# Aman-4-Real/MMTG

Measured on AMD Instinct MI355X. Metric: train tokens/sec, full MMTG config (GPT-2-base-zh decoder, 5x(img+text) 2048-d WenLan embs), higher is better.
Workload: dtype bf16; 1 GPU; Full MMTG train step: S=5 experience steps, T=15+221=236 decoder positions, GPT-2 12L/768/12H V=13317, dropout 0.1 on, MyLoss stage 3 + 0.2*KL, clip 1.0, AdamW; rows_per_gpu=64, global_rows=64, seq_len=236, parallelism=single GPU, no collective

## Files before the change

include/mmtg_hip.h:

```cpp
#ifndef MMTG_HIP_H
#define MMTG_HIP_H

#ifdef __cplusplus
extern "C" {
#endif

#define MMTG_ABI_VERSION 12

#define MMTG_API __attribute__((visibility("default")))

enum { MMTG_OK = 0, MMTG_ERR_BAD_ARG = -1, MMTG_ERR_HIP = -2, MMTG_ERR_UNSUPPORTED = -3 };
enum { MMTG_F32 = 0, MMTG_BF16 = 1 };

enum {
    MMTG_EPI_NONE = 0,
    MMTG_EPI_GELU = 1,
    MMTG_EPI_TANH = 2,
    MMTG_EPI_RESID = 3,
    MMTG_EPI_DGELU = 4,
    MMTG_EPI_DTANH = 5,
    MMTG_EPI_ATOMIC = 6,
    MMTG_EPI_ROWDOT = 7,
    MMTG_EPI_SPLIT = 8,
    MMTG_EPI_TANH_ADD = 9
};
#define MMTG_GEMM_NO_TR 1
#define MMTG_GEMM_REGSTAGE 2
#define MMTG_GEMM_SKINNY 4
#define MMTG_GEMM_NO_SKINNY 8
#define MMTG_GEMM_WIDE 16
#define MMTG_GEMM_NO_WIDE 32
#define MMTG_GEMM_PERSIST 64
#define MMTG_GEMM_NO_PERSIST 128
#define MMTG_GEMM_ROW_ORDER 256
#define MMTG_GEMM_OCC4 512
#define MMTG_GEMM_NO_OCC4 1024
#define MMTG_GEMM_NO_P8 8192
#define MMTG_GEMM_GELU_GRAD 32768
#define MMTG_GEMM_P8 16384
#define MMTG_GEMM_AUX2_BF16 131072
#define MMTG_GEMM_P8_288 65536
#define MMTG_GEMM_P256 4096
#define MMTG_GEMM_COL_BLOCK 2048

enum {
    MMTG_PROF_GEMM_BF16 = 0, MMTG_PROF_GEMM_F32, MMTG_PROF_ATTN_FWD, MMTG_PROF_ATTN_BWD,
    MMTG_PROF_LAYERNORM, MMTG_PROF_EMBED, MMTG_PROF_LOSS, MMTG_PROF_OPTIM, MMTG_PROF_ENCODER,
    MMTG_PROF_DECODE, MMTG_PROF_MISC, MMTG_PROF_NCAT
};

MMTG_API int mmtg_abi_version(void);
MMTG_API const char* mmtg_build_flags(void);
MMTG_API const char* mmtg_last_error(void);

MMTG_API int mmtg_prof_enable(int on);
MMTG_API int mmtg_prof_read(int* launches, double* ms, double* flops, double* bytes);

MMTG_API int mmtg_gemm(int dtype, int transA, int transB, int M, int N, int K,
              const void* A, long lda, const void* B, long ldb, void* C, long ldc,
              const float* bias, int epi, const void* aux, long ldaux, void* aux2,
              int out_f32, float alpha, int splits, unsigned drop_thresh, unsigned drop_seed,
              int flags, void* stream);

MMTG_API int mmtg_gemm_x3(int M, int N, int K, const void* A, long lda, long planeA, const void* B, long ldb, long planeB,
                 float* C, long ldc, void* planes, long ldp, long plane_out, const float* bias, int epi,
                 const float* aux, long ldaux, void* aux2, unsigned drop_thresh, unsigned drop_seed, int flags, void* stream);
MMTG_API int mmtg_split_planes(const float* src, long lds, int rows, int cols, void* planes, long ldp, long plane, void* stream);
MMTG_API int mmtg_layernorm_fwd_x3(const float* x, void* planes, long ldp, long plane, const float* gamma, const float* beta,
                          float* mean, float* rstd, int rows, int cols, float eps, void* x_bf16, void* stream);

MMTG_API int mmtg_gemm_gather(int mode, int M, int N, int K, const void* A, long lda, const void* B, long ldb, void* C, long ldc,
                     const float* bias, int epi, const int* rows, int table_rows, const void* aux, long ldaux, const int* aux_rows,
                     int splits, void* stream);

MMTG_API int mmtg_gemm_trace(void* buf, int max_wgs);
MMTG_API int mmtg_gemm_cu_budget(int cus);
MMTG_API int mmtg_debug_occupy(int workgroups, int lds_bytes, double usec, void* stream);

MMTG_API int mmtg_splitk_finish(int dtype, const float* part, int splits, int M, int N, long ldp, const float* bias,
                       int epi, const void* aux, long ldaux, void* out, long ldo,
                       const float* ln_gamma, const float* ln_beta, void* ln_out, float eps, void* stream);

MMTG_API long mmtg_colsum_ws(int M, int N);
MMTG_API int mmtg_colsum(int dtype, const void* X, long ldx, int M, int N, float* out, float* ws, long ws_floats, void* stream);
typedef struct { const float* X; float* out; long ldx; int M; int N; } mmtg_colsum_item;
MMTG_API int mmtg_colsum_batch(const mmtg_colsum_item* items, int n, void* stream);

MMTG_API int mmtg_layernorm_fwd(int dtype, const void* x, void* y, const float* gamma, const float* beta,
                       float* mean, float* rstd, int rows, int cols, float eps, void* stream);
MMTG_API long mmtg_layernorm_bwd_ws(int rows, int cols);
MMTG_API int mmtg_layernorm_bwd(int dtype, const void* dy, const void* x, const float* gamma,
                       const float* mean, const float* rstd, const void* dres, void* dx,
                       float* dgamma, float* dbeta, int rows, int cols,
                       void* dx_masked, unsigned drop_thresh, unsigned drop_seed, float* dcolsum,
                       float* ws, long ws_floats, void* stream);
MMTG_API int mmtg_layernorm_bwd_partial(int dtype, const void* dy, const void* x, const float* gamma,
                       const float* mean, const float* rstd, const void* dres, void* dx, int rows, int cols,
                       void* dx_masked, unsigned drop_thresh, unsigned drop_seed, int want_colsum,
                       float* ws, long ws_floats, int* partial_rows, void* stream);
MMTG_API int mmtg_layernorm_bwd_x3(const float* dy, const float* x, const float* gamma, const float* mean, const float* rstd,
                          const float* dres, float* dx, float* dgamma, float* dbeta, int rows, int cols,
                          void* dx_planes, long plane, unsigned drop_thresh, unsigned drop_seed, float* dcolsum,
                          float* ws, long ws_floats, void* stream);
MMTG_API int mmtg_layernorm_bwd_x3_partial(const float* dy, const float* x, const float* gamma, const float* mean, const float* rstd,
                          const float* dres, float* dx, int rows, int cols, void* dx_planes, long plane,
                          unsigned drop_thresh, unsigned drop_seed, int want_colsum,
                          float* ws, long ws_floats, int* partial_rows, void* stream);

MMTG_API int mmtg_attn_fwd(int dtype, const void* qkv, const int* keep, void* out, float* lse,
                  int B, int T, int nH, int dh, unsigned drop_thresh, unsigned drop_seed, void* stream);
MMTG_API int mmtg_attn_fwd_x3(const void* qkv_planes, long qplane, const int* keep, float* out, void* out_planes, long plane, float* lse,
                     int B, int T, int nH, int dh, unsigned drop_thresh, unsigned drop_seed, void* stream);
MMTG_API int mmtg_attn_bwd_x3(const void* qkv_planes, long qplane, const int* keep, const float* out, const void* dout_planes, long doplane,
                     const float* lse, float* delta,
                     int delta_ready, float* dq32, long dq32_floats, void* dqkv_planes, long dplane, float* dbias, float* dbias_ws,
                     long dbias_ws_floats, int B, int T, int nH, int dh, unsigned drop_thresh, unsigned drop_seed, void* stream);
MMTG_API int mmtg_attn_trace(void* buf);
#define MMTG_ATTN_ELEM_MASK 1
#define MMTG_ATTN_DBIAS_ROWS 2
MMTG_API int mmtg_attn_bwd_dbias_rows(int dtype, int B, int T);
MMTG_API int mmtg_attn_bwd(int dtype, const void* qkv, const int* keep, const void* out, const void* dout,
                  const float* lse, float* delta, int delta_ready, float* dq32, void* dqkv, float* dbias, float* dbias_ws,
                  int B, int T, int nH, int dh, unsigned drop_thresh, unsigned drop_seed, int flags, void* stream);

MMTG_API int mmtg_embed_condition(int dtype, const void* table, const long long* topic_ids,
                         const long long* targets, const void* c, void* x,
                         int B, int P, int L, int S, int E, int two_sents, int V, void* stream);
MMTG_API int mmtg_segment_sum(int dtype, const void* g, void* out, int B, int P, int L, int S, int H,
                     int two_sents, void* stream);
MMTG_API int mmtg_embed_add(int dtype, const void* g, const void* wpe, const void* wte, const long long* type_ids,
                   void* h, int M, int T, int D, unsigned drop_thresh, unsigned drop_seed, void* stream);
MMTG_API long mmtg_embed_add_bwd_ws(int M, int D, int ntypes);
MMTG_API int mmtg_embed_add_bwd(int dtype, void* dh, const long long* type_ids, float* dwpe, float* dwte,
                       int M, int T, int D, int ntypes, unsigned drop_thresh, unsigned drop_seed, float* ws, long ws_floats,
                       void* stream);
MMTG_API int mmtg_dropout_apply(int dtype, const void* x, void* y, long n, int N, unsigned drop_thresh,
                       unsigned drop_seed, void* stream);

MMTG_API int mmtg_loss_fwd(int logits_dtype, const void* logits, long ldl, int V, const long long* topic_ids,
                  const long long* targets, const long long* ratings, int stage, int label_zero,
                  int B, int P, int L, float batch_den, float* nll, float* lse, float* sample_ce,
                  float* coef, float* scalars, void* stream);
MMTG_API int mmtg_loss_bwd(int dtype, int logits_dtype, const void* logits, long ldl, int V, const long long* topic_ids,
                  const long long* targets, const float* lse, const float* coef, float gscale, float lm_coef,
                  int B, int P, int L, void* dlogits, long ldd, int Vpad, void* stream);
MMTG_API int mmtg_loss_bwd_x3(const float* logits, long ldl, int V, const long long* topic_ids, const long long* targets, const float* lse,
                     const float* coef, float gscale, float lm_coef, int B, int P, int L, void* planes, long ldd, long plane,
                     int Vpad, void* stream);

MMTG_API int mmtg_gru_cell_fwd(int dtype, const void* gi, long ld_gi, const void* gh, long ld_gh, const void* h_prev, long ld_hp,
                      void* h, long ld_h, float* save, int B, int H, void* stream);
MMTG_API int mmtg_gru_cell_bwd(int dtype, const float* dh, const float* save, const void* h_prev, long ld_hp,
                      void* dgi, long ld_dgi, void* dgh, float* dh_prev, int B, int H, void* stream);
MMTG_API int mmtg_gru_cell_bwd_fused(int dtype, const void* rows, long ld_rows, const float* carry, const float* part, int splits,
                            const float* save, const void* h_prev, long ld_hp, void* dgi, long ld_dgi, void* dgh,
                            float* dh_prev, int B, int H, void* stream);
#define MMTG_RNN_RELU 0
#define MMTG_RNN_LSTM 1
MMTG_API int mmtg_rnn_cell_fwd(int dtype, int kind, const void* gi, long ld_gi, const void* gh, long ld_gh, const float* c_prev,
                      void* h, long ld_h, float* c, float* save, int B, int H, void* stream);
MMTG_API int mmtg_rnn_cell_bwd(int dtype, int kind, const void* rows, long ld_rows, const float* part, const float* save,
                      const float* c_prev, const void* h, long ld_h, float* dc, int dc_in, void* da, long ld_da,
                      int B, int H, void* stream);
MMTG_API int mmtg_alpha_attn_fwd(int dtype, const void* qkv, const float* prior, void* ctx, float* probs,
                        float* kl, int B, int S, int H, int heads, void* stream);
MMTG_API int mmtg_alpha_attn_bwd(int dtype, const void* qkv, const float* prior, const float* probs,
                        const void* dctx, float dkl, void* dqkv, int B, int S, int H, int heads,
                        void* stream);
MMTG_API int mmtg_beta_fuse_fwd(int dtype, const void* topic, const void* img, const void* txt,
                       const float* att_w, const float* att_b, void* o, float* a,
                       int B, int S, int H, void* stream);
MMTG_API long mmtg_beta_fuse_bwd_ws(int B, int S, int H);
// ... 110 lines not shown
```

mmtg_amd/csrc/attention.hip:

```cpp
#include <stdlib.h>

#include "attn_common.h"

namespace {

#ifndef ATTN_FWD_WAVES
#define ATTN_FWD_WAVES 4
#endif
template <typename T>
__global__ __launch_bounds__(256, ATTN_FWD_WAVES) void attn_fwd_kernel(const T* __restrict__ qkv, const int* __restrict__ keep,
        T* __restrict__ out, float* __restrict__ lse, int Tn, int nH,
        uint32_t drop_thresh, uint32_t drop_seed, float inv_keep) {
    typedef typename Vec16<T>::type V;
    typedef AT<T> A;
    __shared__ __attribute__((aligned(16))) char sK[64 * A::ROWB];
    __shared__ __attribute__((aligned(16))) char sV[64 * A::ROWB];
    __shared__ int sKeep[64];

    const int tid = threadIdx.x, lane = tid & 63, wave = tid >> 6, g = lane >> 4, l15 = lane & 15;
    const int qb = gridDim.x - 1 - blockIdx.x, h = blockIdx.y, b = blockIdx.z;
    const int D = nH * DH;
    const long ld = 3L * D;
    const T* base = qkv + (long)b * Tn * ld + h * DH;
    const int qi = qb * 64 + wave * 16 + l15;
// ... 422 lines not shown
}
template <int MT = 256>
__device__ __forceinline__ void dma_issue_scalars(void* dst, const void* src, int stride, int nvalid, int wave, int lane) {
    const __amdgpu_buffer_rsrc_t r = __builtin_amdgcn_make_buffer_rsrc(const_cast<void*>(src), 0, (int)(((long)(nvalid - 1) * stride + 1) * 4), 0x00020000);
    const int ws = wave % (MT / 64), i = 64 * ws + lane;
    __builtin_amdgcn_raw_ptr_buffer_load_lds(r, LDS_PTR(void, (char*)dst + 256 * ws), 4, i * stride * 4, 0, 0, 0);
}
template <int NW = 8, int MT = 256>
__device__ __forceinline__ void dma_wait_chunk(int c) {
    if (c >= 3) asm volatile("s_waitcnt vmcnt(0)" ::: "memory");
    else if ((MT / 32) / NW == 1) asm volatile("s_waitcnt vmcnt(2)" ::: "memory");
    else asm volatile("s_waitcnt vmcnt(4)" ::: "memory");
}
__device__ __forceinline__ void raw_barrier() { asm volatile("s_waitcnt lgkmcnt(0)\n\ts_barrier" ::: "memory"); }

constexpr int MASK_BITS = 12;
template <int NTHR = 512, int MT = 256>
__device__ __forceinline__ void gen_keep_mask(uint32_t* sMask, uint32_t bh, int Tn, uint32_t seed, uint32_t keepq, int tid) {
    const int nband = (Tn + 31) >> 5, total = 16 * nband * (nband + 1);
#pragma unroll 1
    for (int i = tid; i < total; i += NTHR) {
        int k = 0;
        while (16 * (k + 1) * (k + 2) <= i) ++k;
        const int j = i - 16 * k * (k + 1), row = 32 * k + j / (k + 1), w = j % (k + 1);
        if (keepq > 4096u) {
            const uint32_t base = (bh * (uint32_t)Tn + (uint32_t)row) * (uint32_t)Tn + 32u * (uint32_t)w;
            uint32_t bits = 0;
#pragma unroll 8
            for (int bit = 0; bit < 32; ++bit) bits |= (hash_u32(seed, base + (uint32_t)bit) >= keepq ? 1u : 0u) << bit;
            sMask[mask_row_base<MT>(row) + w] = bits;
            continue;
        }
        uint32_t x = hash_u32(seed, (bh * (uint32_t)Tn + (uint32_t)row) * (uint32_t)(MT / 32) + (uint32_t)w) | 1u;
        uint32_t acc = 0;
#pragma unroll
        for (int bit = 0; bit < MASK_BITS; ++bit) {
            x ^= x << 13; x ^= x >> 17; x ^= x << 5;
            acc = ((keepq >> bit) & 1u) ? (acc | x) : (acc & x);
        }
        sMask[mask_row_base<MT>(row) + w] = acc;
    }
}
__device__ __forceinline__ float mask_keep(float p, uint32_t w, int pos) {
    const int m = __builtin_amdgcn_sbfe(w, pos, 1);
    return __builtin_bit_cast(float, __builtin_bit_cast(int, p) & m);
}

__device__ __forceinline__ float mask_keep_u(float p, uint32_t w, int pos) {
    int m;
    asm("v_bfe_i32 %0, %1, %2, 1" : "=v"(m) : "v"(w), "s"(pos));
    return __builtin_bit_cast(float, __builtin_bit_cast(int, p) & m);
}

struct FwdTile {
    f32x4 o[4];
    float m, l;
};

__device__ __forceinline__ float max3f(float a, float b, float c) {
    float d;
    asm("v_max3_f32 %0, %1, %2, %3" : "=v"(d) : "v"(a), "v"(b), "v"(c));
    return d;
}

template <bool DROP, int MT = 256, bool DIAG = true>
__device__ __forceinline__ void fwd_small_chunk(FwdTile& st, const char* sK, const char* sV, const float* sBias, const uint32_t* sMask,
                                                const bf16x8 (&qf)[2], int t, int j0, int lane) {
    const int g = lane >> 4, l15 = lane & 15;
    const int qi = 16 * t + l15, qlast = 16 * t + 15;
    f32x4 s_acc[4];
    float mloc = -INFINITY;
#pragma unroll
    for (int kt = 0; kt < 4; ++kt) {
        s_acc[kt] = f32x4{0.f, 0.f, 0.f, 0.f};
        if (!DIAG || j0 + 16 * kt <= qlast) {
#pragma unroll
            for (int ks = 0; ks < 2; ++ks) mma16(ld_row(sK, j0 + kt * 16 + l15, ks, g), qf[ks], s_acc[kt]);
            const int k0 = j0 + kt * 16 + 4 * g;
            const f32x4 kb = *reinterpret_cast<const f32x4*>(sBias + k0);
            if (DIAG && j0 + 16 * kt + 15 > 16 * t) {
#pragma unroll
                for (int r = 0; r < 4; ++r) s_acc[kt][r] = (k0 + r <= qi) ? s_acc[kt][r] * LOG2E + kb[r] : -INFINITY;
            } else {
#pragma unroll
                for (int r = 0; r < 4; ++r) s_acc[kt][r] = s_acc[kt][r] * LOG2E + kb[r];
            }
            mloc = max3f(max3f(mloc, s_acc[kt][0], s_acc[kt][1]), s_acc[kt][2], s_acc[kt][3]);
        }
    }
    mloc = fmaxf(mloc, __shfl_xor(mloc, 16, 64));
    mloc = fmaxf(mloc, __shfl_xor(mloc, 32, 64));
    const float m_new = fmaxf(st.m, mloc);
    const float m_use = (m_new == -INFINITY) ? 0.f : m_new;
    const float alpha = __builtin_amdgcn_exp2f(st.m - m_use);
    float rs = 0.f;
    uint32_t w0 = 0, w1 = 0;
    if constexpr (DROP) {
        if constexpr (MT == 256) {
            const u32x2 w = *reinterpret_cast<const u32x2*>(sMask + qi * 8 + (j0 >> 5));
            w0 = w[0] >> (4 * g);
            w1 = w[1] >> (4 * g);
        } else {
            const uint32_t* wp = sMask + mask_row_base<MT>(qi) + (j0 >> 5);
            w0 = wp[0] >> (4 * g);
            w1 = wp[1] >> (4 * g);
        }
    }
#pragma unroll
    for (int kt = 0; kt < 4; ++kt) {
        if (!DIAG || j0 + 16 * kt <= qlast) {
#pragma unroll
            for (int r = 0; r < 4; ++r) {
                float p = __builtin_amdgcn_exp2f(s_acc[kt][r] - m_use);
                rs += p;
                if constexpr (DROP) p = mask_keep_u(p, kt < 2 ? w0 : w1, 16 * (kt & 1) + r);
                s_acc[kt][r] = p;
            }
        }
    }
    rs += __shfl_xor(rs, 16, 64);
    rs += __shfl_xor(rs, 32, 64);
    st.l = st.l * alpha + rs;
    st.m = m_new;
#pragma unroll
    for (int dt = 0; dt < 4; ++dt) {
        st.o[dt][0] *= alpha; st.o[dt][1] *= alpha; st.o[dt][2] *= alpha; st.o[dt][3] *= alpha;
    }
#pragma unroll
    for (int s2 = 0; s2 < 2; ++s2) {
        if (!DIAG || j0 + 32 * s2 <= qlast) {
            const bf16x8 pb = acc_as_operand(s_acc[2 * s2], s_acc[2 * s2 + 1], bf16());
#pragma unroll
            for (int dt = 0; dt < 4; ++dt)
                mma16(ld_ks(sV, j0 + 32 * s2 + 4 * g, j0 + 32 * s2 + 16 + 4 * g, dt * 16, lane, bf16()), pb, st.o[dt]);
        }
    }
}
template <bool DROP, int MT = 256>
__device__ __forceinline__ void fwd_small_chunk_any(FwdTile& st, const char* sK, const char* sV, const float* sBias, const uint32_t* sMask,
                                                    const bf16x8 (&qf)[2], int t, int j0, int lane) {
    if (j0 + 63 <= 16 * t) fwd_small_chunk<DROP, MT, false>(st, sK, sV, sBias, sMask, qf, t, j0, lane);
    else fwd_small_chunk<DROP, MT, true>(st, sK, sV, sBias, sMask, qf, t, j0, lane);
}

__device__ __forceinline__ void fwd_small_store(const FwdTile& st, int t, int lane, int b, int h, int Tn, int nH, float inv_keep,
                                                bf16* __restrict__ out, float* __restrict__ lse) {
    const int g = lane >> 4, l15 = lane & 15, qi = 16 * t + l15, D = nH * DH;
    if (qi < Tn) {
        const float inv = st.l > 0.f ? inv_keep / st.l : 0.f;
        bf16* dst = out + ((long)b * Tn + qi) * D + h * DH;
#pragma unroll
        for (int dt = 0; dt < 4; ++dt) {
            bf16x4 o = {(bf16)(st.o[dt][0] * inv), (bf16)(st.o[dt][1] * inv), (bf16)(st.o[dt][2] * inv), (bf16)(st.o[dt][3] * inv)};
            *reinterpret_cast<bf16x4*>(dst + dt * 16 + 4 * g) = o;
        }
        if (g == 0) lse[((long)b * nH + h) * Tn + qi] = st.l > 0.f ? st.m * (1.0f / LOG2E) + logf(st.l) : -INFINITY;
    }
}

template <bool DROP, int MT = 256>
__global__ __launch_bounds__(2 * MT, 4) void attn_fwd_small_kernel(const bf16* __restrict__ qkv, const int* __restrict__ keep,
        bf16* __restrict__ out, float* __restrict__ lse, int Tn, int nH,
        uint32_t keep16, uint32_t drop_seed, float inv_keep, unsigned long long* __restrict__ trace) {
    extern __shared__ __attribute__((aligned(16))) char smem[];
    unsigned long long ts[6] = {0, 0, 0, 0, 0, 0};
    ts[0] = __builtin_amdgcn_s_memrealtime();
    constexpr int NW = MT / 32, CROWS = MT / 4;
    const int nchunk = (Tn + CROWS - 1) / CROWS, rows_pad = nchunk * CROWS;
    char* sK = smem;
    char* sV = sK + rows_pad * 128;
    int* sKeep = reinterpret_cast<int*>(sV + rows_pad * 128);
    float* sBias = reinterpret_cast<float*>(sKeep + MT);
    uint32_t* sMask = reinterpret_cast<uint32_t*>(sBias + MT + MT);
    const int tid = threadIdx.x, lane = tid & 63, g = lane >> 4, l15 = lane & 15;
    const int wave = __builtin_amdgcn_readfirstlane(tid >> 6);
    const int h = blockIdx.x % nH, b = blockIdx.x / nH;
    const int D = nH * DH;
    const long ld = 3L * D;
    const bf16* base = qkv + (long)b * Tn * ld + h * DH;
    const int ntile = (Tn + 15) >> 4, npair = (ntile + 1) >> 1;
    const int tA = wave, tB = ntile - 1 - wave;
    const bool work = wave < npair;
    bf16x8 qfA[2], qfB[2];
#pragma unroll
    for (int ks = 0; ks < 2; ++ks) {
        qfA[ks] = zero16<bf16>();
        qfB[ks] = zero16<bf16>();
        if (work) {
            const int qa = 16 * tA + l15, qb = 16 * tB + l15;
            if (qa < Tn) qfA[ks] = *reinterpret_cast<const bf16x8*>(base + (long)qa * ld + ks * 32 + g * 8);
            if (qb < Tn) qfB[ks] = *reinterpret_cast<const bf16x8*>(base + (long)qb * ld + ks * 32 + g * 8);
        }
    }
    const __amdgpu_buffer_rsrc_t rk = rows_rsrc(base + D, ld, Tn), rv = rows_rsrc(base + 2 * D, ld, Tn);
    dma_issue_scalars<MT>(sKeep, keep + (long)b * Tn, 1, Tn, wave, lane);
    dma_issue_chunk<NW, MT>(sK, rk, ld, sV, rv, ld, 0, nchunk, wave, lane);
    dma_issue_chunk<NW, MT>(sK, rk, ld, sV, rv, ld, 1, nchunk, wave, lane);
    if (trace) ts[1] = __builtin_amdgcn_s_memrealtime();
    if constexpr (DROP) gen_keep_mask<2 * MT, MT>(sMask, (uint32_t)(b * nH + h), Tn, drop_seed, keep16, tid);
#pragma unroll
    for (int ks = 0; ks < 2; ++ks)
#pragma unroll
        for (int e = 0; e < 8; ++e) {
            qfA[ks][e] = (bf16)((float)qfA[ks][e] * 0.125f);
            qfB[ks][e] = (bf16)((float)qfB[ks][e] * 0.125f);
        }
    FwdTile st;
#pragma unroll
    for (int i = 0; i < 4; ++i) st.o[i] = f32x4{0.f, 0.f, 0.f, 0.f};
    st.m = -INFINITY;
    st.l = 0.f;
#pragma unroll 1
    for (int jb = 0; jb < nchunk; ++jb) {
        dma_wait_chunk<NW, MT>(jb);
        raw_barrier();
        if (jb < 2) dma_issue_chunk<NW, MT>(sK, rk, ld, sV, rv, ld, jb + 2, nchunk, wave, lane);
        if (jb == 0) {
            if (tid < MT) sBias[tid] = sKeep[tid] != 0 ? 0.f : -INFINITY;
            raw_barrier();
            if (trace) ts[2] = __builtin_amdgcn_s_memrealtime();
        }
#pragma unroll 1
        for (int j0 = jb * CROWS; j0 < (jb + 1) * CROWS; j0 += 64)
            if (work && j0 <= 16 * tB + 15) fwd_small_chunk_any<DROP, MT>(st, sK, sV, sBias, sMask, qfB, tB, j0, lane);
    }
    if (trace) ts[3] = __builtin_amdgcn_s_memrealtime();
    if (work) fwd_small_store(st, tB, lane, b, h, Tn, nH, inv_keep, out, lse);
    if (trace) ts[4] = __builtin_amdgcn_s_memrealtime();
    if (work && tA != tB) {
#pragma unroll
        for (int i = 0; i < 4; ++i) st.o[i] = f32x4{0.f, 0.f, 0.f, 0.f};
        st.m = -INFINITY;
        st.l = 0.f;
#pragma unroll 1
        for (int j0 = 0; j0 <= 16 * tA + 15; j0 += 64) fwd_small_chunk_any<DROP, MT>(st, sK, sV, sBias, sMask, qfA, tA, j0, lane);
        fwd_small_store(st, tA, lane, b, h, Tn, nH, inv_keep, out, lse);
    }
    if (trace && lane == 0) {
        ts[5] = __builtin_amdgcn_s_memrealtime();
        unsigned long long* r = trace + ((long)blockIdx.x * NW + wave) * 8;
        r[0] = ts[0]; r[1] = ts[1]; r[2] = ts[2]; r[3] = ts[3]; r[4] = ts[4]; r[5] = ts[5];
        r[6] = __builtin_amdgcn_s_getreg((4 << 11) | 20);
        r[7] = 1;
    }
}

struct BwdKeys {
// ... 305 lines not shown
#pragma unroll
    for (int dt = 0; dt < 4; ++dt) {
        const bf16x8 ao = ld_ks(sO, q0 + 4 * g, q0 + 16 + 4 * g, dt * 16, lane, bf16());
        const bf16x8 aq = ld_ks(sQ, q0 + 4 * g, q0 + 16 + 4 * g, dt * 16, lane, bf16());
#pragma unroll
        for (int j = 0; j < 2; ++j) {
            mma16(ao, pb[j], st[j].dv[dt]);
            mma16(aq, db[j], st[j].dk[dt]);
        }
    }
}
__device__ __forceinline__ void bwd_small_keys2_store(const BwdKeys (&st)[2], int u, int lane, int b, int h, int Tn, int nH, float inv_keep,
                                                      const int* sKeep, int mt_mask, bf16* __restrict__ dqkv, bool bias, float& ck, float& cv) {
    const int g = lane >> 4, l15 = lane & 15, D = nH * DH;
    const long ld = 3L * D;
    f32x4 fk[4], fv[4];
#pragma unroll
    for (int dt = 0; dt < 4; ++dt) fk[dt] = fv[dt] = f32x4{0.f, 0.f, 0.f, 0.f};
#pragma unroll
    for (int j = 0; j < 2; ++j) {
        const int key = 32 * u + 16 * j + l15;
        const bool kin = key < Tn, kpok = sKeep[key & mt_mask] != 0;
        const float kz = kpok ? 1.f : 0.f, vz = kpok ? inv_keep : 0.f;
        bf16x4 kk[4], vv[4];
#pragma unroll
        for (int dt = 0; dt < 4; ++dt) {
            kk[dt] = bf16x4{(bf16)(st[j].dk[dt][0] * kz), (bf16)(st[j].dk[dt][1] * kz), (bf16)(st[j].dk[dt][2] * kz), (bf16)(st[j].dk[dt][3] * kz)};
            vv[dt] = bf16x4{(bf16)(st[j].dv[dt][0] * vz), (bf16)(st[j].dv[dt][1] * vz), (bf16)(st[j].dv[dt][2] * vz), (bf16)(st[j].dv[dt][3] * vz)};
        }
        if (kin) {
            bf16* dst = dqkv + ((long)b * Tn + key) * ld + h * DH;
#pragma unroll
            for (int dt = 0; dt < 4; ++dt) {
                *reinterpret_cast<bf16x4*>(dst + D + dt * 16 + 4 * g) = kk[dt];
                *reinterpret_cast<bf16x4*>(dst + 2 * D + dt * 16 + 4 * g) = vv[dt];
            }
        }
        if (bias) {
#pragma unroll
            for (int dt = 0; dt < 4; ++dt)
#pragma unroll
                for (int r = 0; r < 4; ++r) {
                    fk[dt][r] += kin ? (float)kk[dt][r] : 0.f;
                    fv[dt][r] += kin ? (float)vv[dt][r] : 0.f;
                }
        }
    }
    if (bias) {
        ck += bias_fold16(fk, l15);
        cv += bias_fold16(fv, l15);
    }
}

template <bool DROP, int MT = 256>
__global__ __launch_bounds__(MT, (MT == 256 ? 2 : 1)) void attn_bwd_small_kv2_kernel(const bf16* __restrict__ qkv, const int* __restrict__ keep,
        const bf16* __restrict__ d_out, const float* __restrict__ lse, const float* __restrict__ delta,
        bf16* __restrict__ dqkv, float* __restrict__ dbias, int bias_rows, int Tn, int nH,
        uint32_t keep16, uint32_t drop_seed, float inv_keep, unsigned long long* __restrict__ trace) {
    extern __shared__ __attribute__((aligned(16))) char smem[];
    unsigned long long ts[6] = {0, 0, 0, 0, 0, 0};
    ts[0] = __builtin_amdgcn_s_memrealtime();
    constexpr int NW = MT / 64, CROWS = MT / 4;
    const int nchunk = (Tn + CROWS - 1) / CROWS, rows_pad = nchunk * CROWS;
    char* sQ = smem;
    char* sO = sQ + rows_pad * 128;
    float* sLse = reinterpret_cast<float*>(sO + rows_pad * 128);
    float* sDel = sLse + MT;
    int* sKeep = reinterpret_cast<int*>(sDel + MT);
    uint32_t* sMask = reinterpret_cast<uint32_t*>(sKeep + 2 * MT);
    const int tid = threadIdx.x, lane = tid & 63, g = lane >> 4, l15 = lane & 15;
    const int wave = __builtin_amdgcn_readfirstlane(tid >> 6);
    const int h = blockIdx.x % nH, b = blockIdx.x / nH;
    const int D = nH * DH;
    const long ld = 3L * D;
    const bf16* base = qkv + (long)b * Tn * ld + h * DH;
    const bf16* dob = d_out + (long)b * Tn * D + h * DH;
    const int nunit = (Tn + 31) >> 5, nupair = (nunit + 1) >> 1;
    const int uA = wave, uB = nunit - 1 - wave;
    const bool work = wave < nupair;
    bf16x8 kf[2][2], vf[2][2];
    auto load_frags = [&](int u) {
#pragma unroll
        for (int j = 0; j < 2; ++j) {
            const int key = 32 * u + 16 * j + l15;
#pragma unroll
            for (int ks = 0; ks < 2; ++ks) {
                kf[j][ks] = vf[j][ks] = zero16<bf16>();
                if (key < Tn) {
                    kf[j][ks] = *reinterpret_cast<const bf16x8*>(base + (long)key * ld + D + ks * 32 + g * 8);
                    vf[j][ks] = *reinterpret_cast<const bf16x8*>(base + (long)key * ld + 2 * D + ks * 32 + g * 8);
                }
            }
        }
    };
    if (work) load_frags(uA);
    else {
#pragma unroll
        for (int j = 0; j < 2; ++j) kf[j][0] = kf[j][1] = vf[j][0] = vf[j][1] = zero16<bf16>();
    }
    const __amdgpu_buffer_rsrc_t rq = rows_rsrc(base, ld, Tn), ro = rows_rsrc(dob, D, Tn);
    dma_issue_scalars<MT>(sKeep, keep + (long)b * Tn, 1, Tn, wave, lane);
    dma_issue_scalars<MT>(sLse, lse + ((long)b * nH + h) * Tn, 1, Tn, wave, lane);
    dma_issue_scalars<MT>(sDel, delta + (long)b * Tn * nH + h, nH, Tn, wave, lane);
    dma_issue_chunk<NW, MT>(sQ, rq, ld, sO, ro, D, 0, nchunk, wave, lane);
    dma_issue_chunk<NW, MT>(sQ, rq, ld, sO, ro, D, 1, nchunk, wave, lane);
    if (trace) ts[1] = __builtin_amdgcn_s_memrealtime();
    if constexpr (DROP) gen_keep_mask<64 * NW, MT>(sMask, (uint32_t)(b * nH + h), Tn, drop_seed, keep16, tid);
    asm volatile("" :: "v"(kf[0][0]), "v"(kf[0][1]), "v"(vf[0][0]), "v"(vf[0][1]), "v"(kf[1][0]), "v"(kf[1][1]), "v"(vf[1][0]), "v"(vf[1][1]));
    BwdKeys st[2];
#pragma unroll
    for (int j = 0; j < 2; ++j)
#pragma unroll
        for (int i = 0; i < 4; ++i) st[j].dk[i] = st[j].dv[i] = f32x4{0.f, 0.f, 0.f, 0.f};
    float ck = 0.f, cv = 0.f;
    const float ik_scale = inv_keep * 0.125f;
#pragma unroll 1
    for (int c = 0; c < nchunk; ++c) {
        dma_wait_chunk<NW, MT>(c);
        raw_barrier();
        if (c < 2) dma_issue_chunk<NW, MT>(sQ, rq, ld, sO, ro, D, c + 2, nchunk, wave, lane);
        if (c == 0) {
            for (int i = tid; i < MT; i += 64 * NW) { sLse[i] *= LOG2E; sDel[i] *= 0.125f; }
            raw_barrier();
            if (trace) ts[2] = __builtin_amdgcn_s_memrealtime();
        }
#pragma unroll 1
        for (int qb = c * (CROWS / 32); qb < (c + 1) * (CROWS / 32) && qb < nunit; ++qb)
            if (work && qb >= uA) {
                if (qb == uA) bwd_small_keys2_block<DROP, MT, true>(st, sQ, sO, sLse, sDel, sMask, kf, vf, uA, 32 * qb, lane, ik_scale);
                else bwd_small_keys2_block<DROP, MT, false>(st, sQ, sO, sLse, sDel, sMask, kf, vf, uA, 32 * qb, lane, ik_scale);
            }
    }
    if (trace) ts[3] = __builtin_amdgcn_s_memrealtime();
    if (work) {
        if (uB != uA) load_frags(uB);
        bwd_small_keys2_store(st, uA, lane, b, h, Tn, nH, inv_keep, sKeep, MT - 1, dqkv, dbias != nullptr, ck, cv);
        if (uB != uA) {
#pragma unroll
            for (int j = 0; j < 2; ++j)
#pragma unroll
                for (int i = 0; i < 4; ++i) st[j].dk[i] = st[j].dv[i] = f32x4{0.f, 0.f, 0.f, 0.f};
            bwd_small_keys2_block<DROP, MT, true>(st, sQ, sO, sLse, sDel, sMask, kf, vf, uB, 32 * uB, lane, ik_scale);
#pragma unroll 1
// ... 39 lines not shown
    uint32_t wq = 0;
    if constexpr (DROP) wq = sMask[mask_row_base<MT>(qi) + (j0 >> 5)] >> (4 * g);
#pragma unroll
    for (int kt = 0; kt < 2; ++kt) {
        dsT[kt] = f32x4{0.f, 0.f, 0.f, 0.f};
        if (!DIAG || j0 + 16 * kt <= qlast) {
            f32x4 s_acc = {0.f, 0.f, 0.f, 0.f}, dp_acc = {0.f, 0.f, 0.f, 0.f};
#pragma unroll
            for (int ks = 0; ks < 2; ++ks) {
                mma16(ld_row(sK, j0 + kt * 16 + l15, ks, g), qf[ks], s_acc);
                mma16(ld_row(sV, j0 + kt * 16 + l15, ks, g), of[ks], dp_acc);
            }
            const int k0 = j0 + kt * 16 + 4 * g;
            const f32x4 kb = *reinterpret_cast<const f32x4*>(sBias + k0);
#pragma unroll
            for (int r = 0; r < 4; ++r) {
                float x = s_acc[r] * c1 - lse2_q + kb[r];
                if constexpr (DIAG) x = k0 + r <= qi ? x : -INFINITY;
                const float p = __builtin_amdgcn_exp2f(x);
                float dp = dp_acc[r];
                if constexpr (DROP) dp = mask_keep_u(dp, wq, 16 * kt + r);
                dsT[kt][r] = p * (dp * ik_scale - dels_q);
            }
        }
    }
    const bf16x8 db = acc_as_operand(dsT[0], dsT[1], bf16());
#pragma unroll
    for (int dt = 0; dt < 4; ++dt)
        mma16(ld_ks(sK, j0 + 4 * g, j0 + 16 + 4 * g, dt * 16, lane, bf16()), db, dq[dt]);
}
__device__ __forceinline__ void bwd_small_queries_store(const f32x4 (&dq)[4], int t, int lane, int b, int h, int Tn, int nH,
                                                        bf16* __restrict__ dqkv, bool bias, float& cq) {
    const int g = lane >> 4, l15 = lane & 15, qi = 16 * t + l15, D = nH * DH;
    const long ld = 3L * D;
    const bool qok = qi < Tn;
    if (qok) {
        bf16* dst = dqkv + ((long)b * Tn + qi) * ld + h * DH;
#pragma unroll
        for (int dt = 0; dt < 4; ++dt) {
            bf16x4 qq = {(bf16)dq[dt][0], (bf16)dq[dt][1], (bf16)dq[dt][2], (bf16)dq[dt][3]};
            *reinterpret_cast<bf16x4*>(dst + dt * 16 + 4 * g) = qq;
        }
    }
    if (bias) {
        f32x4 fq[4];
#pragma unroll
        for (int dt = 0; dt < 4; ++dt)
#pragma unroll
            for (int r = 0; r < 4; ++r) fq[dt][r] = qok ? (float)(bf16)dq[dt][r] : 0.f;
        cq += bias_fold16(fq, l15);
    }
}

template <bool DROP, int MT = 256>
__global__ __launch_bounds__(2 * MT, 4) void attn_bwd_small_q_kernel(const bf16* __restrict__ qkv, const int* __restrict__ keep,
        const bf16* __restrict__ d_out, const float* __restrict__ lse, const float* __restrict__ delta,
        bf16* __restrict__ dqkv, float* __restrict__ dbias, int bias_rows, int Tn, int nH,
        uint32_t keep16, uint32_t drop_seed, float inv_keep, unsigned long long* __restrict__ trace) {
    extern __shared__ __attribute__((aligned(16))) char smem[];
    unsigned long long ts[6] = {0, 0, 0, 0, 0, 0};
    ts[0] = __builtin_amdgcn_s_memrealtime();
    constexpr int NW = MT / 32, CROWS = MT / 4;
    const int nchunk = (Tn + CROWS - 1) / CROWS, rows_pad = nchunk * CROWS;
    char* sK = smem;
    char* sV = sK + rows_pad * 128;
    int* sKeep = reinterpret_cast<int*>(sV + rows_pad * 128);
    float* sBias = reinterpret_cast<float*>(sKeep);
    float* sLse = sBias + MT;
    float* sDel = sLse + MT;
    uint32_t* sMask = reinterpret_cast<uint32_t*>(sDel + 2 * MT);
    const int tid = threadIdx.x, lane = tid & 63, g = lane >> 4, l15 = lane & 15;
    const int wave = __builtin_amdgcn_readfirstlane(tid >> 6);
    const int h = blockIdx.x % nH, b = blockIdx.x / nH;
    const int D = nH * DH;
    const long ld = 3L * D;
    const bf16* base = qkv + (long)b * Tn * ld + h * DH;
    const bf16* dob = d_out + (long)b * Tn * D + h * DH;
    const int ntile = (Tn + 15) >> 4, npair = (ntile + 1) >> 1;
    const int tA = wave, tB = ntile - 1 - wave;
    const bool work = wave < npair;
    const __amdgpu_buffer_rsrc_t rk = rows_rsrc(base + D, ld, Tn), rv = rows_rsrc(base + 2 * D, ld, Tn);
    dma_issue_scalars<MT>(sKeep, keep + (long)b * Tn, 1, Tn, wave, lane);
    dma_issue_scalars<MT>(sLse, lse + ((long)b * nH + h) * Tn, 1, Tn, wave, lane);
    dma_issue_scalars<MT>(sDel, delta + (long)b * Tn * nH + h, nH, Tn, wave, lane);
    dma_issue_chunk<NW, MT>(sK, rk, ld, sV, rv, ld, 0, nchunk, wave, lane);
    const int qa = 16 * tA + l15, qb_ = 16 * tB + l15;
    bf16x8 qfB[2], ofB[2];
    {
        const int qc = work ? (qb_ < Tn ? qb_ : Tn - 1) : 0;
#pragma unroll
        for (int ks = 0; ks < 2; ++ks) {
            qfB[ks] = *reinterpret_cast<const bf16x8*>(base + (long)qc * ld + ks * 32 + g * 8);
            ofB[ks] = *reinterpret_cast<const bf16x8*>(dob + (long)qc * D + ks * 32 + g * 8);
        }
    }
    dma_issue_chunk<NW, MT>(sK, rk, ld, sV, rv, ld, 1, nchunk, wave, lane);
    if (trace) ts[1] = __builtin_amdgcn_s_memrealtime();
    if constexpr (DROP) gen_keep_mask<2 * MT, MT>(sMask, (uint32_t)(b * nH + h), Tn, drop_seed, keep16, tid);
    asm volatile("" :: "v"(qfB[0]), "v"(qfB[1]), "v"(ofB[0]), "v"(ofB[1]));
    if (!(work && qb_ < Tn)) { qfB[0] = qfB[1] = ofB[0] = ofB[1] = zero16<bf16>(); }
    float lseB = 0.f, delB = 0.f;
    f32x4 dq[4];
#pragma unroll
    for (int i = 0; i < 4; ++i) dq[i] = f32x4{0.f, 0.f, 0.f, 0.f};
    const float ik_scale = inv_keep * 0.125f;
    bf16x8 qfA[2], ofA[2];
#pragma unroll 1
    for (int c = 0; c < nchunk; ++c) {
        dma_wait_chunk<NW, MT>(c);
        raw_barrier();
        if (c < 2) dma_issue_chunk<NW, MT>(sK, rk, ld, sV, rv, ld, c + 2, nchunk, wave, lane);
        if (c == 0) {
            if (tid < MT) sBias[tid] = sKeep[tid] != 0 ? 0.f : -INFINITY;
            lseB = sLse[qb_ & (MT - 1)] * LOG2E;
            delB = sDel[qb_ & (MT - 1)] * 0.125f;
            raw_barrier();
            if (trace) ts[2] = __builtin_amdgcn_s_memrealtime();
        }
#pragma unroll 1
        for (int kb = c * (CROWS / 32); kb < (c + 1) * (CROWS / 32); ++kb)
            if (work && 32 * kb <= 16 * tB + 15) {
                if (32 * kb + 31 <= 16 * tB) bwd_small_queries_block<DROP, MT, false>(dq, sK, sV, sBias, sMask, qfB, ofB, lseB, delB, tB, 32 * kb, lane, ik_scale);
                else bwd_small_queries_block<DROP, MT, true>(dq, sK, sV, sBias, sMask, qfB, ofB, lseB, delB, tB, 32 * kb, lane, ik_scale);
            }
    }
    if (trace) ts[3] = __builtin_amdgcn_s_memrealtime();
    float cq = 0.f;
    if (work) {
        if (tA != tB) {
            const int qc = qa < Tn ? qa : Tn - 1;
#pragma unroll
            for (int ks = 0; ks < 2; ++ks) {
                qfA[ks] = *reinterpret_cast<const bf16x8*>(base + (long)qc * ld + ks * 32 + g * 8);
                ofA[ks] = *reinterpret_cast<const bf16x8*>(dob + (long)qc * D + ks * 32 + g * 8);
// ... 16 lines not shown
    if (trace) ts[4] = __builtin_amdgcn_s_memrealtime();
    if (dbias) {
        __syncthreads();
        float* sBw = reinterpret_cast<float*>(smem);
        sBw[wave * DH + (l15 >> 2) * 16 + 4 * g + (l15 & 3)] = cq;
        __syncthreads();
        if (tid < DH) {
            float sm = 0.f;
#pragma unroll
            for (int w = 0; w < NW; ++w) sm += sBw[w * DH + tid];
            const int col = h * DH + tid;
            if (bias_rows) dbias[(long)b * 3 * D + col] = sm;
            else atomicAdd(dbias + col, sm);
        }
    }
    if (trace && lane == 0) {
        ts[5] = __builtin_amdgcn_s_memrealtime();
        unsigned long long* r = trace + ((long)(gridDim.x + blockIdx.x) * 16 + wave) * 8;
        r[0] = ts[0]; r[1] = ts[1]; r[2] = ts[2]; r[3] = ts[3]; r[4] = ts[4]; r[5] = ts[5];
        r[6] = __builtin_amdgcn_s_getreg((4 << 11) | 20);
        r[7] = 1;
    }
}

template <int MT = 256> inline size_t small_smem(int T) {
    const int cr = MT / 4, rp = ((T + cr - 1) / cr) * cr;
    return (size_t)rp * 256 + 4 * MT * 4 + (size_t)mask_words<MT>() * 4;
}
inline unsigned small_keep16(unsigned thresh32) { return 4096u - ((thresh32 + 0x80000u) >> 20); }
inline float small_inv_keep(unsigned keepq) { return (float)(4096.0 / (double)keepq); }


template <typename T> size_t bwd_smem_bytes() {
    typedef AT<T> A;
    const int KB = 4 * A::KPW;
    return (size_t)3 * KB * A::ROWB + 4 * 32 * A::ROWB + 32 * KB * sizeof(T) + 64 * sizeof(float) + KB * sizeof(int);
}

inline float inv_keep_of(unsigned thresh) {
    return thresh ? (float)(4294967296.0 / (4294967296.0 - (double)thresh)) : 1.0f;
}

}

static unsigned long long* g_attn_trace = nullptr;
extern "C" int mmtg_attn_trace(void* buf) {
    g_attn_trace = reinterpret_cast<unsigned long long*>(buf);
    return MMTG_OK;
}

static bool attn_route_tiled() { static const bool v = getenv("MMTG_ATTN_TILED") != nullptr; return v; }
static bool attn_route_no512() { static const bool v = getenv("MMTG_ATTN_NO512") != nullptr; return v; }

extern "C" int mmtg_attn_fwd(int dtype, const void* qkv, const int* keep, void* out, float* lse,
                             int B, int T, int nH, int dh, unsigned drop_thresh, unsigned drop_seed, void* stream) {
    MMTG_REQUIRE(dh == DH, "attn_fwd: head dim %d unsupported (built for 64)", dh);
    MMTG_REQUIRE(B > 0 && T > 0 && nH > 0, "attn_fwd: bad sizes");
    MMTG_REQUIRE(qkv && keep && out && lse, "attn_fwd: null pointer");
    MMTG_REQUIRE(MMTG_ALIGNED16(qkv) && MMTG_ALIGNED16(out), "attn_fwd: 16-byte alignment");
    hipStream_t s = (hipStream_t)stream;
    const double esz = dtype == MMTG_F32 ? 4 : 2;
    ProfScope prof(MMTG_PROF_ATTN_FWD, s, 2.0 * B * nH * (double)T * T * dh, esz * 4.0 * B * T * nH * dh);
    dim3 grid(cdiv(T, 64), nH, B), block(256);
    const float ik = inv_keep_of(drop_thresh);
    const bool legacy = attn_route_tiled(), no512 = attn_route_no512();
    if (dtype == MMTG_BF16 && T <= (no512 ? 256 : SM_MAXT) && !legacy) {
        static bool attr_set = false;
        if (!attr_set) {
            if (hipFuncSetAttribute((const void*)attn_fwd_small_kernel<false, 256>, hipFuncAttributeMaxDynamicSharedMemorySize, (int)small_smem<256>(256)) != hipSuccess ||
                hipFuncSetAttribute((const void*)attn_fwd_small_kernel<true, 256>, hipFuncAttributeMaxDynamicSharedMemorySize, (int)small_smem<256>(256)) != hipSuccess ||
                hipFuncSetAttribute((const void*)attn_fwd_small_kernel<false, 512>, hipFuncAttributeMaxDynamicSharedMemorySize, (int)small_smem<512>(512)) != hipSuccess ||
                hipFuncSetAttribute((const void*)attn_fwd_small_kernel<true, 512>, hipFuncAttributeMaxDynamicSharedMemorySize, (int)small_smem<512>(512)) != hipSuccess)
                MMTG_FAIL(MMTG_ERR_HIP, "attn_fwd: cannot raise dynamic LDS");
            attr_set = true;
        }
        const unsigned k16 = small_keep16(drop_thresh);
        const bool drop = k16 < 4096u;
        const unsigned kq = drop ? k16 : 0u;
        const float ikq = drop ? small_inv_keep(k16) : 1.0f;
#define FWD_SMALL(DROP_, MT_) hipLaunchKernelGGL((attn_fwd_small_kernel<DROP_, MT_>), dim3(B * nH), dim3(2 * MT_), small_smem<MT_>(T), s, \
                                                 (const bf16*)qkv, keep, (bf16*)out, lse, T, nH, kq, drop_seed, ikq, g_attn_trace)
        if (T <= 256) { if (drop) FWD_SMALL(true, 256); else FWD_SMALL(false, 256); }
        else { if (drop) FWD_SMALL(true, 512); else FWD_SMALL(false, 512); }
#undef FWD_SMALL
        MMTG_LAUNCH_CHECK("attn_fwd");
        return MMTG_OK;
    }
    if (dtype == MMTG_F32)
        hipLaunchKernelGGL(attn_fwd_kernel<float>, grid, block, 0, s, (const float*)qkv, keep, (float*)out, lse, T, nH, drop_thresh, drop_seed, ik);
    else if (dtype == MMTG_BF16)
        hipLaunchKernelGGL(attn_fwd_kernel<bf16>, grid, block, 0, s, (const bf16*)qkv, keep, (bf16*)out, lse, T, nH, drop_thresh, drop_seed, ik);
    else MMTG_FAIL(MMTG_ERR_BAD_ARG, "attn_fwd: bad dtype");
    MMTG_LAUNCH_CHECK("attn_fwd");
    return MMTG_OK;
}

extern "C" int mmtg_colsum(int dtype, const void* X, long ldx, int M, int N, float* out, float* ws, long ws_floats, void* stream);

extern "C" int mmtg_attn_bwd_dbias_rows(int dtype, int B, int T) {
    return (dtype == MMTG_BF16 && T <= (attn_route_no512() ? 256 : SM_MAXT) && !attn_route_tiled()) ? B : 0;
}

extern "C" int mmtg_attn_bwd(int dtype, const void* qkv, const int* keep, const void* out, const void* dout,
                             const float* lse, float* delta, int delta_ready, float* dq32, void* dqkv, float* dbias, float* dbias_ws,
                             int B, int T, int nH, int dh, unsigned drop_thresh, unsigned drop_seed, int flags, void* stream) {
    MMTG_REQUIRE(dh == DH, "attn_bwd: head dim %d unsupported (built for 64)", dh);
    MMTG_REQUIRE(B > 0 && T > 0 && nH > 0, "attn_bwd: bad sizes");
    MMTG_REQUIRE(qkv && keep && out && dout && lse && delta && dq32 && dqkv, "attn_bwd: null pointer");
    MMTG_REQUIRE(MMTG_ALIGNED16(qkv) && MMTG_ALIGNED16(dout) && MMTG_ALIGNED16(dqkv), "attn_bwd: 16-byte alignment");
    hipStream_t s = (hipStream_t)stream;
    const double esz = dtype == MMTG_F32 ? 4 : 2;
    ProfScope prof(MMTG_PROF_ATTN_BWD, s, 5.0 * B * nH * (double)T * T * dh, esz * 8.0 * B * T * nH * dh);
    const long rows = (long)B * T;
    const int D = nH * dh;
    const float ik = inv_keep_of(drop_thresh);
    float* const bias_dst = dbias && dbias_ws ? dbias_ws : dbias;
    const int bias_rows = dbias && dbias_ws ? 1 : 0;
    static bool attr_set[2] = {false, false};
    bool small_path = false;
    static const int ablate = getenv("MMTG_ATTN_ABLATE") ? atoi(getenv("MMTG_ATTN_ABLATE")) : 0;
    if (dtype == MMTG_F32) {
        const int KB = 4 * AT<float>::KPW;
        const int nkb = cdiv(T, KB);
        const size_t shm = bwd_smem_bytes<float>();
        if (!attr_set[0]) {
            if (hipFuncSetAttribute((const void*)attn_bwd_kernel<float, 4>, hipFuncAttributeMaxDynamicSharedMemorySize, (int)shm) != hipSuccess)
                MMTG_FAIL(MMTG_ERR_HIP, "attn_bwd: cannot raise dynamic LDS to %zu", shm);
            attr_set[0] = true;
        }
        if (!delta_ready) hipLaunchKernelGGL(attn_delta_kernel<float>, dim3(cdiv(rows * nH, 4)), dim3(256), 0, s, (const float*)out, (const float*)dout, delta, T, nH, rows);
        if (nkb > 1) { if (hipMemsetAsync(dq32, 0, rows * D * sizeof(float), s) != hipSuccess) MMTG_FAIL(MMTG_ERR_HIP, "attn_bwd: memset failed"); }
        hipLaunchKernelGGL((attn_bwd_kernel<float, 4>), dim3(nkb, nH, B), dim3(256), shm, s, (const float*)qkv, keep, (const float*)dout, lse, delta, dq32, (float*)dqkv, bias_dst, bias_rows, T, nH, nkb == 1, drop_thresh, drop_seed, ik, ablate);
        if (nkb > 1) hipLaunchKernelGGL(attn_dq_finish_kernel<float>, dim3(2048), dim3(256), 0, s, dq32, (float*)dqkv, rows, D);
    } else if (dtype == MMTG_BF16 && T <= (attn_route_no512() ? 256 : SM_MAXT) && !attn_route_tiled()) {
        small_path = true;
        static bool attr_small = false;
        if (!attr_small) {
            const int shm2 = (int)small_smem<256>(256), shm5 = (int)small_smem<512>(512);
            bool ok = true;
#define SET_LDS(K_, B_) ok = ok && hipFuncSetAttribute((const void*)K_, hipFuncAttributeMaxDynamicSharedMemorySize, B_) == hipSuccess
            SET_LDS((attn_bwd_small_kv_kernel<false, 8, 256>), shm2); SET_LDS((attn_bwd_small_kv_kernel<true, 8, 256>), shm2);
            SET_LDS((attn_bwd_small_kv_kernel<false, 4, 256>), shm2); SET_LDS((attn_bwd_small_kv_kernel<true, 4, 256>), shm2);
            SET_LDS((attn_bwd_small_q_kernel<false, 256>), shm2); SET_LDS((attn_bwd_small_q_kernel<true, 256>), shm2);
            SET_LDS((attn_bwd_small_kv_kernel<false, 16, 512>), shm5); SET_LDS((attn_bwd_small_kv_kernel<true, 16, 512>), shm5);
            SET_LDS((attn_bwd_small_kv_kernel<false, 8, 512>), shm5); SET_LDS((attn_bwd_small_kv_kernel<true, 8, 512>), shm5);
            SET_LDS((attn_bwd_small_q_kernel<false, 512>), shm5); SET_LDS((attn_bwd_small_q_kernel<true, 512>), shm5);
            SET_LDS((attn_bwd_small_kv2_kernel<false, 256>), shm2); SET_LDS((attn_bwd_small_kv2_kernel<true, 256>), shm2);
            SET_LDS((attn_bwd_small_kv2_kernel<false, 512>), shm5); SET_LDS((attn_bwd_small_kv2_kernel<true, 512>), shm5);
#undef SET_LDS
            if (!ok) MMTG_FAIL(MMTG_ERR_HIP, "attn_bwd: cannot raise dynamic LDS");
            attr_small = true;
        }
        if (!delta_ready) hipLaunchKernelGGL(attn_delta_kernel<bf16>, dim3(cdiv(rows * nH, 4)), dim3(256), 0, s, (const bf16*)out, (const bf16*)dout, delta, T, nH, rows);
        const unsigned th16 = small_keep16(drop_thresh);
        const bool elem = (flags & MMTG_ATTN_ELEM_MASK) && drop_thresh > 4096u;
        const bool drop = elem || th16 < 4096u;
        const unsigned kq = elem ? drop_thresh : drop ? th16 : 0u;
        const float ik16 = elem ? ik : drop ? small_inv_keep(th16) : 1.0f;
        static const int kv_nw = getenv("MMTG_ATTN_KV_NW") ? atoi(getenv("MMTG_ATTN_KV_NW")) : 0;
#define KV_SMALL(DROP_, NW_, MT_) hipLaunchKernelGGL((attn_bwd_small_kv_kernel<DROP_, NW_, MT_>), dim3(B * nH), dim3(64 * NW_), small_smem<MT_>(T), s, \
                                   (const bf16*)qkv, keep, (const bf16*)dout, lse, delta, (bf16*)dqkv, bias_dst, bias_rows, T, nH, kq, drop_seed, ik16, g_attn_trace)
#define Q_SMALL(DROP_, MT_) hipLaunchKernelGGL((attn_bwd_small_q_kernel<DROP_, MT_>), dim3(B * nH), dim3(2 * MT_), small_smem<MT_>(T), sq, \
                                   (const bf16*)qkv, keep, (const bf16*)dout, lse, delta, (bf16*)dqkv, bias_dst, bias_rows, T, nH, kq, drop_seed, ik16, g_attn_trace)
        static const bool kv2 = !(getenv("MMTG_ATTN_KV2") && atoi(getenv("MMTG_ATTN_KV2")) == 0);
#define KV2_SMALL(DROP_, MT_) hipLaunchKernelGGL((attn_bwd_small_kv2_kernel<DROP_, MT_>), dim3(B * nH), dim3(MT_), small_smem<MT_>(T), s, \
                                   (const bf16*)qkv, keep, (const bf16*)dout, lse, delta, (bf16*)dqkv, bias_dst, bias_rows, T, nH, kq, drop_seed, ik16, g_attn_trace)
        static const bool fork = getenv("MMTG_ATTN_BWD_FORK") && atoi(getenv("MMTG_ATTN_BWD_FORK")) == 1;
        static hipStream_t s2 = nullptr;
        static hipEvent_t ev_fork = nullptr, ev_join = nullptr;
        if (fork && !s2) {
            if (hipStreamCreateWithFlags(&s2, hipStreamNonBlocking) != hipSuccess || hipEventCreateWithFlags(&ev_fork, hipEventDisableTiming) != hipSuccess ||
                hipEventCreateWithFlags(&ev_join, hipEventDisableTiming) != hipSuccess)
                MMTG_FAIL(MMTG_ERR_HIP, "attn_bwd: cannot create the side stream");
        }
        hipStream_t sq = s;
        if (fork && kv2 && !kv_nw) {
            sq = s2;
            if (hipEventRecord(ev_fork, s) != hipSuccess || hipStreamWaitEvent(s2, ev_fork, 0) != hipSuccess) MMTG_FAIL(MMTG_ERR_HIP, "attn_bwd: fork failed");
        }
        if (kv2 && !kv_nw) {
            if (T <= 256) { if (drop) KV2_SMALL(true, 256); else KV2_SMALL(false, 256); }
            else { if (drop) KV2_SMALL(true, 512); else KV2_SMALL(false, 512); }
            if (T <= 256) { if (drop) Q_SMALL(true, 256); else Q_SMALL(false, 256); }
            else { if (drop) Q_SMALL(true, 512); else Q_SMALL(false, 512); }
            if (sq != s) {
                if (hipEventRecord(ev_join, s2) != hipSuccess || hipStreamWaitEvent(s, ev_join, 0) != hipSuccess) MMTG_FAIL(MMTG_ERR_HIP, "attn_bwd: join failed");
            }
        } else if (T <= 256) {
            const bool half = kv_nw ? kv_nw == 4 : drop;
            if (drop) { if (half) KV_SMALL(true, 4, 256); else KV_SMALL(true, 8, 256); Q_SMALL(true, 256); }
            else { if (half) KV_SMALL(false, 4, 256); else KV_SMALL(false, 8, 256); Q_SMALL(false, 256); }
        } else {
            const bool half = kv_nw ? kv_nw == 8 : drop;
            if (drop) { if (half) KV_SMALL(true, 8, 512); else KV_SMALL(true, 16, 512); Q_SMALL(true, 512); }
            else { if (half) KV_SMALL(false, 8, 512); else KV_SMALL(false, 16, 512); Q_SMALL(false, 512); }
        }
#undef KV_SMALL
#undef KV2_SMALL
#undef Q_SMALL
    } else if (dtype == MMTG_BF16) {
        const int KB = 4 * AT<bf16>::KPW;
        const int nkb = cdiv(T, KB);
        const size_t shm = bwd_smem_bytes<bf16>();
        if (!attr_set[1]) {
            if (hipFuncSetAttribute((const void*)attn_bwd_kernel<bf16, 8>, hipFuncAttributeMaxDynamicSharedMemorySize, (int)shm) != hipSuccess)
                MMTG_FAIL(MMTG_ERR_HIP, "attn_bwd: cannot raise dynamic LDS to %zu", shm);
            attr_set[1] = true;
        }
        if (!delta_ready) hipLaunchKernelGGL(attn_delta_kernel<bf16>, dim3(cdiv(rows * nH, 4)), dim3(256), 0, s, (const bf16*)out, (const bf16*)dout, delta, T, nH, rows);
        if (nkb > 1) { if (hipMemsetAsync(dq32, 0, rows * D * sizeof(float), s) != hipSuccess) MMTG_FAIL(MMTG_ERR_HIP, "attn_bwd: memset failed"); }
        hipLaunchKernelGGL((attn_bwd_kernel<bf16, 8>), dim3(nkb, nH, B), dim3(512), shm, s, (const bf16*)qkv, keep, (const bf16*)dout, lse, delta, dq32, (bf16*)dqkv, bias_dst, bias_rows, T, nH, nkb == 1, drop_thresh, drop_seed, ik, ablate);
        if (nkb > 1) hipLaunchKernelGGL(attn_dq_finish_kernel<bf16>, dim3(2048), dim3(256), 0, s, dq32, (bf16*)dqkv, rows, D);
    } else MMTG_FAIL(MMTG_ERR_BAD_ARG, "attn_bwd: bad dtype");
    MMTG_LAUNCH_CHECK("attn_bwd");
    const int nkb_ = small_path ? 1 : cdiv(T, dtype == MMTG_F32 ? 4 * AT<float>::KPW : 4 * AT<bf16>::KPW);
    if (bias_rows && !((flags & MMTG_ATTN_DBIAS_ROWS) && small_path)) {
        int rc = mmtg_colsum(MMTG_F32, dbias_ws, 3L * D, B * nkb_, 3 * D, dbias, nullptr, 0, stream);
        if (rc) return rc;
    }
    if (dbias && nkb_ > 1)
        return mmtg_colsum(dtype, dqkv, 3L * D, (int)rows, D, dbias, dbias_ws ? dbias_ws + (long)B * nkb_ * 3 * D : nullptr, dbias_ws ? 44L * 3 * D : 0, stream);
    return MMTG_OK;
}
```

mmtg_amd/csrc/gemm.hip:

```cpp
#include "gemm_common.h"
#include <stdlib.h>

namespace {

template <typename T, bool AKS, bool BKS, bool USE_TR>
__global__ __launch_bounds__(NTHR, 2) void gemm_kernel(GemmArgs p) {
    typedef typename Vec16<T>::type V;
    __shared__ __attribute__((aligned(16))) char smem[4 * TILE_BYTES];
    const int tid = threadIdx.x, lane = tid & 63, wave = tid >> 6;
    const int g = lane >> 4, l15 = lane & 15;
    const int wm = wave >> 1, wn = wave & 1;
    int m0, n0;
    int split;
    tile_origin(p, blockIdx.x, gridDim.x, m0, n0, split);
    const int kbeg = split * p.kper;
    const int kend = min(p.K, kbeg + p.kper);
    const int nk = (kend - kbeg + GT<T>::BK - 1) / GT<T>::BK;
    const T* A = reinterpret_cast<const T*>(p.A);
    const T* B = reinterpret_cast<const T*>(p.B);

    f32x4 acc[4][4];
#pragma unroll
    for (int i = 0; i < 4; ++i)
#pragma unroll
// ... 574 lines not shown
    constexpr int NW = TBM / 32;
    const size_t shm = 2 * (TBM + 128) * 128 + NW * epi_scratch_bytes<4, 4>();
    static_assert(TBM == 256 || 2 * (128 + 128) * 128 + 4 * epi_scratch_bytes<4, 4>() <= 80 * 1024, "two workgroups per CU");
    if (!attr_done) {
        int rc = set_lds(gemm_pp_kernel<AKS, BKS, TBM>, shm, 64 * NW, TBM == 256 ? "persistent 256x128" : "persistent 128x128");
        if (rc) return rc;
        attr_done = true;
    }
    GemmArgs b = a;
    b.tiles_n = cdiv(a.N, 128);
    b.ntiles = cdiv(a.M, TBM) * b.tiles_n;
    b.nitems = b.ntiles * splits;
    if (TBM == 256 && !(AKS && BKS) && splits == 1 && !(a.dbg_flags & 1)) b.cbw = column_block(a, TBM, 128, num_cus());
    const int slots = ((TBM == 256 ? 1 : 2) * num_cus()) & ~7;
    dim3 grid(b.nitems < slots ? b.nitems : slots), block(64 * NW);
    hipLaunchKernelGGL((gemm_pp_kernel<AKS, BKS, TBM>), grid, block, shm, stream, b);
    return MMTG_OK;
}

__device__ __forceinline__ void p8_issue(__amdgpu_buffer_rsrc_t r, char* d0, char* d1, int v0, int v1, int soff) {
    soff = __builtin_amdgcn_readfirstlane(soff);
    __builtin_amdgcn_raw_ptr_buffer_load_lds(r, LDS_PTR(void, d0), 16, v0, soff, 0, 0);
    __builtin_amdgcn_raw_ptr_buffer_load_lds(r, LDS_PTR(void, d1), 16, v1, soff, 0, 0);
}
__device__ __forceinline__ void p8_issue1(__amdgpu_buffer_rsrc_t r, char* d0, int v0, int soff) {
    soff = __builtin_amdgcn_readfirstlane(soff);
    __builtin_amdgcn_raw_ptr_buffer_load_lds(r, LDS_PTR(void, d0), 16, v0, soff, 0, 0);
}

template <int AH, int BH, int NA, int TMW, int FAN>
__device__ __forceinline__ void p8_mfma(const bf16x8 (&fa)[FAN][2], const bf16x8 (&fb)[2][2], f32x4 (&acc)[TMW][4], const bool prio = true) {
    if (prio) __builtin_amdgcn_s_setprio(1);
#pragma unroll
    for (int kk = 0; kk < 2; ++kk)
#pragma unroll
        for (int i = 0; i < NA; ++i)
#pragma unroll
            for (int j = 0; j < 2; ++j) mma16(fb[j][kk], fa[i][kk], acc[4 * AH + i][2 * BH + j]);
    if (prio) __builtin_amdgcn_s_setprio(0);
}

__device__ __forceinline__ bf16x8 p8_ld(const char* q) { return *reinterpret_cast<const bf16x8*>(q); }

#define P8_SYNC_IN()  do { asm volatile("s_barrier\n\ts_waitcnt lgkmcnt(0)" ::: "memory"); __builtin_amdgcn_sched_barrier(0); } while (0)
#define P8_SYNC_OUT() do { __builtin_amdgcn_sched_barrier(0); asm volatile("s_barrier" ::: "memory"); } while (0)

template <int GRPCH>
__device__ __forceinline__ int p8_ks_voff(long ld, int col0, int ncols, int h, int blk, int lane) {
    const int k = blk * 4 + (lane >> 4), pc = lane & 15, c = pc ^ ks_swz(k);
    const int col = (c / GRPCH) * (2 * GRPCH * 8) + h * (GRPCH * 8) + (c % GRPCH) * 8;
    return (col0 + col < ncols) ? (int)(((long)k * ld + col) * 2) : OOB;
}

template <int TBM, bool KS = false, bool X3 = false>
__global__ __launch_bounds__(512, 1) void gemm_p8_kernel(GemmArgs p) {
    typedef typename std::conditional<X3, float, bf16>::type TE;
    static_assert(!(X3 && (KS || TBM == 288)), "x3: K-contiguous operands, 256- or 192-row tiles");
    static_assert(TBM == 256 || ((TBM == 192 || TBM == 288) && !KS), "row tiles of 256 or (K-contiguous operands) 192 / 288");
    constexpr int WTM = TBM / 2, TMW = WTM / 16, NA1 = TMW - 4;
    constexpr int NBG = TBM / 16;
    constexpr int TA = TBM * 128, STAGE = TA + 256 * 128;
    extern __shared__ __attribute__((aligned(16))) char smem[];
    const int tid = threadIdx.x, lane = tid & 63;
    const int wave = __builtin_amdgcn_readfirstlane(tid >> 6);
    const int g = lane >> 4, l15 = lane & 15;
    const int wr = wave >> 2, wc = wave & 3;
    asm volatile("" :: "s"(p.A), "s"(p.B), "s"(p.M), "s"(p.N), "s"(p.K), "s"(p.lda), "s"(p.ldb), "s"(p.ntiles), "s"(p.tiles_n),
                 "s"(p.tiles_m_fast), "s"(p.cbw), "s"(p.trace), "s"(p.dbg_flags), "s"(p.bytesA), "s"(p.bytesB), "s"(p.kper));
    const bool tr = p.trace != nullptr;
    unsigned long long ts0 = 0, ts1 = 0, ts2 = 0, tc1 = 0, tc2 = 0;
    ts0 = __builtin_amdgcn_s_memrealtime();
    int m0, n0, split;
    tile_origin(p, blockIdx.x, gridDim.x, m0, n0, split, TBM, 256);
    const int kbeg = KS ? split * p.kper : 0;
    const int nk1 = max(0, (KS ? min(p.K, kbeg + p.kper) : p.K) - kbeg) >> 6;
    const int nk = X3 ? 3 * nk1 : nk1;

    const __amdgpu_buffer_rsrc_t ra = __builtin_amdgcn_make_buffer_rsrc(const_cast<void*>(p.A), 0, p.bytesA, 0x00020000);
    const __amdgpu_buffer_rsrc_t rb = __builtin_amdgcn_make_buffer_rsrc(const_cast<void*>(p.B), 0, p.bytesB, 0x00020000);
    const int sa0 = (int)((KS ? (long)kbeg * p.lda + m0 : (long)m0 * p.lda) * 2), sb0 = (int)((KS ? (long)kbeg * p.ldb + n0 : (long)n0 * p.ldb) * 2);
    const int stepa = KS ? (int)(64 * p.lda * 2) : 128, stepb = KS ? (int)(64 * p.ldb * 2) : 128;
    int lA00, lA01, lA10, lA11, lB00, lB01, lB10, lB11, vA00, vA01, vA10, vA11, vB00, vB01, vB10, vB11;
    int lA12 = 0, vA12 = OOB;
    if constexpr (!KS) {
        const int bA0 = wave, bA1 = bA0 + NBG;
        const int bA2 = TBM != 192 ? 8 + wave : (wave >> 2) * NBG + 8 + (wave & 3), bA3 = NBG + 8 + wave;
        const int bA4 = wave < 2 ? 16 + wave : NBG + 16 + ((wave - 2) & 1);
        lA12 = bA4 * 1024;
        vA12 = (TBM == 288 && wave < 4) ? dma_voff<false, TBM>(p.lda, m0, p.M, 64, bA4, lane) : OOB;
        const int bB = 8 * (wave >> 2) + (wave & 3);
        lA00 = bA0 * 1024; lA01 = bA1 * 1024; lA10 = bA2 * 1024; lA11 = bA3 * 1024;
        lB00 = TA + bB * 1024; lB01 = TA + (bB + 16) * 1024; lB10 = TA + (bB + 4) * 1024; lB11 = TA + (bB + 20) * 1024;
        vA00 = dma_voff<false, TBM>(p.lda, m0, p.M, 64, bA0, lane); vA01 = dma_voff<false, TBM>(p.lda, m0, p.M, 64, bA1, lane);
        vA10 = dma_voff<false, TBM>(p.lda, m0, p.M, 64, bA2, lane);
        vA11 = TBM != 192 ? dma_voff<false, TBM>(p.lda, m0, p.M, 64, bA3, lane) : OOB;
        vB00 = dma_voff<false, 256>(p.ldb, n0, p.N, 64, bB, lane); vB01 = dma_voff<false, 256>(p.ldb, n0, p.N, 64, bB + 16, lane);
        vB10 = dma_voff<false, 256>(p.ldb, n0, p.N, 64, bB + 4, lane); vB11 = dma_voff<false, 256>(p.ldb, n0, p.N, 64, bB + 20, lane);
    } else {
        lA00 = wave * 1024; lA01 = (wave + 8) * 1024; lA10 = 16384 + lA00; lA11 = 16384 + lA01;
        lB00 = TA + lA00; lB01 = TA + lA01; lB10 = TA + lA10; lB11 = TA + lA11;
        vA00 = p8_ks_voff<8>(p.lda, m0, p.M, 0, wave, lane); vA01 = p8_ks_voff<8>(p.lda, m0, p.M, 0, wave + 8, lane);
        vA10 = p8_ks_voff<8>(p.lda, m0, p.M, 1, wave, lane); vA11 = p8_ks_voff<8>(p.lda, m0, p.M, 1, wave + 8, lane);
        vB00 = p8_ks_voff<4>(p.ldb, n0, p.N, 0, wave, lane); vB01 = p8_ks_voff<4>(p.ldb, n0, p.N, 0, wave + 8, lane);
        vB10 = p8_ks_voff<4>(p.ldb, n0, p.N, 1, wave, lane); vB11 = p8_ks_voff<4>(p.ldb, n0, p.N, 1, wave + 8, lane);
    }
#define P8_PASS(t) (((t) >= nk1 ? 1 : 0) + ((t) >= 2 * nk1 ? 1 : 0))
#define P8_SA(t) (X3 ? sa0 + ((t) - P8_PASS(t) * nk1) * stepa + (P8_PASS(t) == 1 ? p.planeA : 0) : sa0 + (t) * stepa)
// ... 54 lines not shown
#ifdef MMTG_P8_PHASE_TRACE
    unsigned pst[20];
#pragma unroll
    for (int i_ = 0; i_ < 20; ++i_) pst[i_] = 0;
#define P8_STAMP(kt_, i_) do { if (tr && (kt_) == 8 && blockIdx.x == 0) pst[i_] = (unsigned)__builtin_amdgcn_s_memtime(); } while (0)
#else
#define P8_STAMP(kt_, i_) do { } while (0)
#endif
#define P8_TILE(ST, kt)                                                                                    \
    do {                                                                                                   \
        P8_STAMP(kt, 0);                                                                                   \
        P8_RD_B(ST, 0, fb0);                                                                               \
        __builtin_amdgcn_sched_barrier(0);                                                                 \
        P8_RD_A(ST, 0, 4);                                                                                 \
        P8_A1((kt) + 1);                                                                                   \
         \
        if constexpr (!KS) asm volatile("s_waitcnt lgkmcnt(8)" ::: "memory");                               \
        else asm volatile("s_waitcnt lgkmcnt(15)" ::: "memory");                                           \
        P8_STAMP(kt, 1);                                                                                   \
        P8_SYNC_IN(); P8_STAMP(kt, 2); p8_mfma<0, 0, 4, TMW>(fa, fb0, acc, mprio); P8_STAMP(kt, 3); P8_SYNC_OUT(); P8_STAMP(kt, 4);  \
        P8_RD_B(ST, 1, fb1);                                                                               \
        P8_B0((kt) + 2);                                                                                   \
        P8_STAMP(kt, 5);                                                                                   \
        P8_SYNC_IN(); P8_STAMP(kt, 6); p8_mfma<0, 1, 4, TMW>(fa, fb1, acc, mprio); P8_STAMP(kt, 7); P8_SYNC_OUT(); P8_STAMP(kt, 8);  \
        P8_RD_A(ST, 1, NA1);                                                                               \
        P8_A0((kt) + 2);                                                                                   \
        P8_STAMP(kt, 9);                                                                                   \
        P8_SYNC_IN(); P8_STAMP(kt, 10); p8_mfma<1, 1, NA1, TMW>(fa, fb1, acc, mprio); P8_STAMP(kt, 11); P8_SYNC_OUT(); P8_STAMP(kt, 12); \
        P8_B1((kt) + 2);                                                                                   \
        wait_vmcnt<6>();                                                      \
        P8_STAMP(kt, 13);                                                                                  \
        P8_SYNC_IN(); P8_STAMP(kt, 14); p8_mfma<1, 0, NA1, TMW>(fa, fb0, acc, mprio); P8_STAMP(kt, 15); P8_SYNC_OUT(); P8_STAMP(kt, 16); \
    } while (0)
    for (int kt = 0; kt < nk; kt += 2) {
        P8_TILE(0, kt);
        P8_TILE(1, kt + 1);
    }
#undef P8_TILE
#undef P8_STAMP
#undef P8_RD_A
#undef P8_RD_B
#undef P8_A0
#undef P8_A1
#undef P8_B0
#undef P8_B1
#undef P8_SA
#undef P8_SB
#undef P8_PASS
    wait_vmcnt<0>();
    if (tr) { ts2 = __builtin_amdgcn_s_memrealtime(); tc2 = __builtin_amdgcn_s_memtime(); }
    if (wr == 0) asm volatile("s_barrier" ::: "memory");
    asm volatile("s_barrier" ::: "memory");
    if constexpr (KS) p.C = reinterpret_cast<char*>(p.C) + (long)split * p.split_stride;
    gemm_epilogue<TE, false, TMW, 4, (TBM == 256 ? 2 : TBM == 288 ? -1 : -2), X3>(p, acc, m0 + wr * WTM, n0 + wc * 64, g, l15, smem + wave * epi_scratch_bytes<TMW, 4>(), lane);
#ifdef MMTG_P8_PHASE_TRACE
    if (tr && blockIdx.x == 0 && lane == 0 && (int)(gridDim.x + 4 * wave + 4) <= p.trace_n) {
        unsigned long long* r = p.trace + 6 * (size_t)(gridDim.x + 4 * wave);
#pragma unroll
        for (int i_ = 0; i_ < 20; ++i_) r[i_] = pst[i_];
    }
#endif
    if (tr && wave == 0 && (int)blockIdx.x < p.trace_n) {
        wait_vmcnt<0>();
        const unsigned long long ts3 = __builtin_amdgcn_s_memrealtime();
        if (lane == 0) {
            unsigned long long* r = p.trace + 6 * (size_t)blockIdx.x;
            r[0] = ts0; r[1] = ts1; r[2] = ts2; r[3] = ts3; r[4] = (unsigned long long)nk | ((tc2 - tc1) << 20);
            r[5] = ((unsigned long long)__builtin_amdgcn_s_getreg((3 << 11) | 20) << 32) | __builtin_amdgcn_s_getreg((31 << 11) | 4);
        }
    }
}

template <int TBM>
__global__ __launch_bounds__(512, 1) void gemm_p8p_kernel(GemmArgs p) {
    typedef bf16 T;
    static_assert(TBM == 256 || TBM == 192, "row tiles of 256 or 192");
    constexpr int WTM = TBM / 2, TMW = WTM / 16, NA1 = TMW - 4;
    constexpr int NBG = TBM / 16;
    constexpr int TA = TBM * 128, STAGE = TA + 256 * 128;
    extern __shared__ __attribute__((aligned(16))) char smem[];
    const int tid = threadIdx.x, lane = tid & 63;
    const int wave = __builtin_amdgcn_readfirstlane(tid >> 6);
    const int g = lane >> 4, l15 = lane & 15, l8 = lane >> 3;
    const int wr = wave >> 2, wc = wave & 3;
    const int nk = p.K >> 6;
    const __amdgpu_buffer_rsrc_t ra = __builtin_amdgcn_make_buffer_rsrc(const_cast<void*>(p.A), 0, p.bytesA, 0x00020000);
    const __amdgpu_buffer_rsrc_t rb = __builtin_amdgcn_make_buffer_rsrc(const_cast<void*>(p.B), 0, p.bytesB, 0x00020000);
    const int bA0 = wave, bA1 = bA0 + NBG;
    const int bA2 = TBM == 256 ? 8 + wave : (wave >> 2) * NBG + 8 + (wave & 3), bA3 = NBG + 8 + wave;
    const int bB0 = 8 * (wave >> 2) + (wave & 3), bB1 = bB0 + 16, bB2 = bB0 + 4, bB3 = bB0 + 20;
    const int c8 = ((lane & 7) ^ l8) * 16;
    const int vrA = (int)((long)l8 * p.lda * 2) + c8, vrB = (int)((long)l8 * p.ldb * 2) + c8;
    const int vA00 = vrA + (int)((long)bA0 * 8 * p.lda * 2), vA01 = vrA + (int)((long)bA1 * 8 * p.lda * 2);
    const int vA10 = vrA + (int)((long)bA2 * 8 * p.lda * 2), vA11 = vrA + (int)((long)bA3 * 8 * p.lda * 2);
    const int vB00 = vrB + (int)((long)bB0 * 8 * p.ldb * 2), vB01 = vrB + (int)((long)bB1 * 8 * p.ldb * 2);
    const int vB10 = vrB + (int)((long)bB2 * 8 * p.ldb * 2), vB11 = vrB + (int)((long)bB3 * 8 * p.ldb * 2);

    int item = blockIdx.x, m0, n0, split, m0n = 0, n0n = 0;
    tile_origin(p, item, p.nitems, m0, n0, split, TBM, 256);
    bool has_next = false;
#define P8P_SEL(t)                                                                                          \
    const bool cur_ = (t) < nk;                                                                             \
    const bool live_ = cur_ || has_next;                                                                    \
    const int tt_ = cur_ ? (t) : (t) - nk;                                                                  \
    const int mm_ = cur_ ? m0 : m0n, nn_ = cur_ ? n0 : n0n;                                                 \
    const int sa_ = (int)(((long)mm_ * p.lda + (long)tt_ * 64) * 2), sb_ = (int)(((long)nn_ * p.ldb + (long)tt_ * 64) * 2); \
    const int la_ = live_ ? p.M - mm_ : 0, lb_ = live_ ? p.N - nn_ : 0;                                     \
// ... 50 lines not shown
        P8P_A0((kt) + 2);                                                                                  \
        P8_SYNC_IN(); p8_mfma<1, 1, NA1, TMW>(fa, fb1, acc); P8_SYNC_OUT();                                 \
        P8P_B1((kt) + 2);                                                                                  \
        wait_vmcnt<6>();                                                                                   \
        P8_SYNC_IN(); p8_mfma<1, 0, NA1, TMW>(fa, fb0, acc); P8_SYNC_OUT();                                 \
    } while (0)
    for (;;) {
        const int nxt = item + (int)gridDim.x;
        has_next = nxt < p.nitems;
        if (has_next) tile_origin(p, nxt, p.nitems, m0n, n0n, split, TBM, 256);
        for (int kt = 0; kt < nk; kt += 2) {
            P8P_TILE(0, kt);
            P8P_TILE(1, kt + 1);
        }
        gemm_epilogue<T, false, TMW, 4, (TBM == 256 ? 2 : -2)>(p, acc, m0 + wr * WTM, n0 + wc * 64, g, l15,
                                                               smem + 2 * STAGE + wave * epi_scratch_bytes<TMW, 4>(), lane);
        if (!has_next) break;
        for (int i = 0; i < TMW; ++i)
            for (int j = 0; j < 4; ++j) acc[i][j] = f32x4{0.f, 0.f, 0.f, 0.f};
        item = nxt; m0 = m0n; n0 = n0n;
    }
#undef P8P_TILE
#undef P8_RD_A
#undef P8_RD_B
#undef P8P_A0
#undef P8P_A1
#undef P8P_B0
#undef P8P_B1
#undef P8P_SEL
    if (wr == 0) asm volatile("s_barrier" ::: "memory");
}

template <int TBM>
int launch_p8p(const GemmArgs& a, hipStream_t stream) {
    static bool attr_done = false;
    const size_t shm = 2 * (TBM + 256) * 128 + 8 * epi_scratch_bytes<TBM / 32, 4>();
    if (!attr_done) {
        int rc = set_lds(gemm_p8p_kernel<TBM>, shm, 512, TBM == 256 ? "persistent eight-phase 256x256" : "persistent eight-phase 192x256");
        if (rc) return rc;
        attr_done = true;
    }
    GemmArgs b = a;
    b.tiles_n = cdiv(a.N, 256);
    b.ntiles = cdiv(a.M, TBM) * b.tiles_n;
    b.nitems = b.ntiles;
    b.tiles_m_fast = 0;
    b.cbw = 0;
    if (!(a.dbg_flags & 1)) b.cbw = column_block(a, TBM, 256, num_cus());
    const int grid = b.nitems < num_cus() ? b.nitems : num_cus();
    hipLaunchKernelGGL(gemm_p8p_kernel<TBM>, dim3(grid), dim3(512), shm, stream, b);
    return MMTG_OK;
}

template <int TBM, bool KS = false, bool X3 = false>
int launch_p8(const GemmArgs& a, int splits, hipStream_t stream) {
    static bool attr_done = false;
    const size_t shm = 2 * (TBM + 256) * 128;
    if (!attr_done) {
        int rc = set_lds(gemm_p8_kernel<TBM, KS, X3>, shm, 512, KS ? "eight-phase 256x256 K-strided" : TBM == 256 ? "eight-phase 256x256" : TBM == 288 ? "eight-phase 288x256" : "eight-phase 192x256");
        if (rc) return rc;
        attr_done = true;
    }
    GemmArgs b = a;
    b.tiles_n = cdiv(a.N, 256);
    b.ntiles = cdiv(a.M, TBM) * b.tiles_n;
    b.nitems = b.ntiles * splits;
    b.tiles_m_fast = KS && b.tiles_n > cdiv(a.M, TBM) && !(a.dbg_flags & 1);
    b.cbw = 0;
    if (!KS && !(a.dbg_flags & 1)) b.cbw = column_block(a, TBM, 256, num_cus());
    hipLaunchKernelGGL((gemm_p8_kernel<TBM, KS, X3>), dim3(b.nitems), dim3(512), shm, stream, b);
    return MMTG_OK;
}

template <bool AKS, bool BKS, bool SLAB = false>
int launch_occ4(const GemmArgs& a, int splits, hipStream_t stream) {
    static bool attr_done = false;
    constexpr int TBM = 128;
    const size_t shm = (TBM + 128) * 128;
    if (!attr_done) {
        int rc = set_lds(gemm_occ4_kernel<AKS, BKS, SLAB>, shm, 256, "single-stage 128x128, 4 per CU");
        if (rc) return rc;
        attr_done = true;
    }
    GemmArgs b = a;
    b.tiles_n = cdiv(a.N, 128);
    b.ntiles = cdiv(a.M, TBM) * b.tiles_n;
    b.nitems = b.ntiles * splits;
    b.tiles_m_fast = AKS && BKS && b.tiles_n > cdiv(a.M, TBM);
    if (!(AKS && BKS) && splits == 1 && !(a.dbg_flags & 1)) b.cbw = column_block(a, TBM, 128, 3 * num_cus());
    hipLaunchKernelGGL((gemm_occ4_kernel<AKS, BKS, SLAB>), dim3(b.nitems), dim3(256), shm, stream, b);
    return MMTG_OK;
}

int launch_dma(const GemmArgs& a, int transA, int transB, int splits, int skinny, int wide, int persist, hipStream_t stream) {
    if (a.dbg_flags & 2) {
        if (!transA && transB) return launch_occ4<false, false>(a, splits, stream);
        if (!transA && !transB) return launch_occ4<false, true>(a, splits, stream);
        if (a.epi == MMTG_EPI_SPLIT) return launch_occ4<true, true, true>(a, splits, stream);
        return launch_occ4<true, true>(a, splits, stream);
    }
    if (persist && !wide && !skinny && (a.dbg_flags & 32)) {
        if (!transA && transB) return launch_pp<false, false, 256>(a, splits, stream);
        if (!transA && !transB) return launch_pp<false, true, 256>(a, splits, stream);
    }
    if (persist && !wide && !skinny) {
        if (!transA && transB) return launch_pp<false, false>(a, splits, stream);
        if (!transA && !transB) return launch_pp<false, true>(a, splits, stream);
        return launch_pp<true, true>(a, splits, stream);
    }
    if (wide) {
        if (!transA && transB) return launch_dma_cfg<false, false, 192, 128, 3, 2, 2>(a, splits, stream);
        if (!transA && !transB) return launch_dma_cfg<false, true, 192, 128, 3, 2, 2>(a, splits, stream);
    }
    if (!transA && transB && !skinny && (a.dbg_flags & 64)) {
        return launch_dma_cfg<false, false, 256, 256, 2, 2, 2>(a, splits, stream);
    }
    if (!transA && transB) {
        if (skinny) {
            const char* e = getenv("MMTG_SKINNY_CFG");
            const int cfg = e ? atoi(e) : 1;
            switch (cfg) {
                case 1: return launch_dma_cfg<false, false, 64, 64, 2, 2, 4>(a, splits, stream);
                case 2: return launch_dma_cfg<false, false, 128, 64, 2, 2, 4>(a, splits, stream);
// ... 72 lines not shown
        const long bytesA = ((long)(K - 1) * lda + M) * 2, bytesB = ((long)(table_rows - 1) * ldb + N) * 2;
        MMTG_REQUIRE(bytesA < 0x7FFFFF00L && bytesB < 0x7FFFFF00L, "gemm_gather: operands must stay below 2 GiB");
        a.bytesA = (int)bytesA; a.bytesB = (int)bytesB;
        a.out_f32 = 1;
        a.kper = cdiv(cdiv(K, splits), 64) * 64;
        a.split_stride = (long)M * ldc * 4;
        a.tiles_n = cdiv(N, 128);
        a.ntiles = cdiv(M, 128) * a.tiles_n;
        a.nitems = a.ntiles * splits;
        a.tiles_m_fast = a.tiles_n > cdiv(M, 128);
        ProfScope prof(MMTG_PROF_GEMM_BF16, s, 2.0 * M * N * (double)K, 2.0 * ((double)M * K + (double)N * K) + 4.0 * (double)M * N);
        static bool attr_done = false;
        const size_t shm = (128 + 128) * 128;
        if (!attr_done) {
            int rc = set_lds(gemm_occ4_kernel<true, true, true, true>, shm, 256, "gather weight gradient");
            if (rc) return rc;
            attr_done = true;
        }
        hipLaunchKernelGGL((gemm_occ4_kernel<true, true, true, true>), dim3(a.nitems), dim3(256), shm, s, a);
    }
    MMTG_LAUNCH_CHECK("gemm_gather");
    return MMTG_OK;
}

extern "C" int mmtg_gemm(int dtype, int transA, int transB, int M, int N, int K,
                         const void* A, long lda, const void* B, long ldb, void* C, long ldc,
                         const float* bias, int epi, const void* aux, long ldaux, void* aux2,
                         int out_f32, float alpha, int splits, unsigned drop_thresh, unsigned drop_seed,
                         int flags, void* stream) {
    MMTG_REQUIRE(dtype == MMTG_F32 || dtype == MMTG_BF16, "gemm: bad dtype %d", dtype);
    MMTG_REQUIRE(M > 0 && N > 0 && K > 0, "gemm: empty problem %d %d %d", M, N, K);
    MMTG_REQUIRE(A && B && C, "gemm: null operand");
    MMTG_REQUIRE(!(transA && transB), "gemm: layout transA=1,transB=1 is not built");
    const int epc = dtype == MMTG_F32 ? 4 : 8;
    MMTG_REQUIRE(MMTG_ALIGNED16(A) && MMTG_ALIGNED16(B) && MMTG_ALIGNED16(C), "gemm: operands must be 16-byte aligned");
    MMTG_REQUIRE(lda % epc == 0 && ldb % epc == 0, "gemm: lda/ldb must be multiples of %d elements", epc);
    MMTG_REQUIRE((transA ? M : K) % epc == 0, "gemm: contiguous extent of A (%d) must be a multiple of %d", transA ? M : K, epc);
    MMTG_REQUIRE((transB ? K : N) % epc == 0, "gemm: contiguous extent of B (%d) must be a multiple of %d", transB ? K : N, epc);
    const bool wgrad = transA && !transB;
    MMTG_REQUIRE(epi != MMTG_EPI_ATOMIC || wgrad, "gemm: the atomic epilogue belongs to the transA=1,transB=0 (weight-gradient) layout");
    MMTG_REQUIRE(!wgrad || epi == MMTG_EPI_ATOMIC || epi == MMTG_EPI_SPLIT,
                 "gemm: the weight-gradient layout has the atomic and the split (slab) epilogues only");
    if (epi != MMTG_EPI_ATOMIC) {
        MMTG_REQUIRE(N % 8 == 0 && ldc % 8 == 0, "gemm: N and ldc must be multiples of 8 (N=%d ldc=%ld)", N, ldc);
        MMTG_REQUIRE(!bias || MMTG_ALIGNED16(bias), "gemm: bias must be 16-byte aligned");
        MMTG_REQUIRE(splits <= 1 || epi == MMTG_EPI_SPLIT, "gemm: split-K needs the atomic or the split epilogue");
        if (epi == MMTG_EPI_SPLIT)
            MMTG_REQUIRE(out_f32 && !bias && (dtype == MMTG_BF16 ? !(flags & (MMTG_GEMM_REGSTAGE | MMTG_GEMM_NO_TR | MMTG_GEMM_PERSIST)) : true),
                         "gemm: the split epilogue stores raw fp32 partial products (out_f32, no bias) from the bf16 LDS-DMA kernels "
                         "or the fp32 kernel");
    } else {
        MMTG_REQUIRE(!bias, "gemm: atomic epilogue takes no bias");
    }
    if (epi == MMTG_EPI_ROWDOT)
        MMTG_REQUIRE(aux2 && !bias && N % 64 == 0 && dtype == MMTG_BF16 && !transA && M > 256 && !(flags & (MMTG_GEMM_REGSTAGE | MMTG_GEMM_NO_TR | MMTG_GEMM_SKINNY)),
                     "gemm: ROWDOT epilogue needs aux2 (f32 [M, N/64]), no bias, N %% 64 == 0, the bf16 128x128 LDS-DMA configuration");
    if (epi == MMTG_EPI_RESID || epi == MMTG_EPI_DGELU || epi == MMTG_EPI_DTANH || epi == MMTG_EPI_ROWDOT)
        MMTG_REQUIRE(aux && ldaux % 8 == 0 && MMTG_ALIGNED16(aux), "gemm: epilogue %d needs a 16-byte aligned aux operand with ldaux %% 8 == 0", epi);
    if (epi == MMTG_EPI_GELU) MMTG_REQUIRE(aux2 && MMTG_ALIGNED16(aux2), "gemm: GELU epilogue needs a 16-byte aligned aux2 for the pre-activation");
    GemmArgs a;
    memset(&a, 0, sizeof(a));
    a.A = A; a.B = B; a.C = C; a.bias = bias; a.aux = aux; a.aux2 = aux2;
    a.M = M; a.N = N; a.K = K; a.lda = lda; a.ldb = ldb; a.ldc = ldc; a.ldaux = ldaux;
    a.epi = epi; a.out_f32 = out_f32; a.use_tr = !(flags & MMTG_GEMM_NO_TR);
    a.trace = g_trace; a.trace_n = g_trace_n;
    a.gelu_grad = (flags & MMTG_GEMM_GELU_GRAD) ? 1 : 0;
    a.dbg_flags = ((flags & MMTG_GEMM_ROW_ORDER) ? 1 : 0) | ((flags & MMTG_GEMM_COL_BLOCK) ? 16 : 0) | ((flags & MMTG_GEMM_P256) ? 32 : 0);
    static const int p8_noprio = getenv("MMTG_P8_NOPRIO") ? atoi(getenv("MMTG_P8_NOPRIO")) : 0;
    if (p8_noprio) a.dbg_flags |= 128;
    a.tiles_n = cdiv(N, BN); a.alpha = alpha;
    const long esz = dtype == MMTG_F32 ? 4 : 2;
    const long bytesA = ((long)((transA ? K : M) - 1) * lda + (transA ? M : K)) * esz;
    const long bytesB = ((long)((transB ? N : K) - 1) * ldb + (transB ? K : N)) * esz;
    const bool small = bytesA < 0x7FFFFF00L && bytesB < 0x7FFFFF00L;
    MMTG_REQUIRE(!(wgrad && epi == MMTG_EPI_SPLIT) || small, "gemm: the weight-gradient slab epilogue needs operands below 2 GiB");
    a.bytesA = (int)(small ? bytesA : 0); a.bytesB = (int)(small ? bytesB : 0);
    const int bk = dtype == MMTG_F32 ? 32 : 64;
    if (splits < 1) splits = 1;
    int kper = cdiv(cdiv(K, splits), bk) * bk;
    if (epi != MMTG_EPI_SPLIT) splits = cdiv(K, kper);
    a.kper = kper;
    a.split_stride = epi == MMTG_EPI_SPLIT ? (long)M * ldc * 4 : 0;
    a.drop_thresh = drop_thresh; a.drop_seed = drop_seed;
    a.drop_inv_keep = drop_thresh ? (float)(4294967296.0 / (4294967296.0 - (double)drop_thresh)) : 1.0f;
    hipStream_t s = (hipStream_t)stream;
    const double esz_ = dtype == MMTG_F32 ? 4 : 2;
    double alg_bytes = esz_ * ((double)M * K + (double)N * K) + (double)M * N * (out_f32 ? 4 : esz_);
    if (epi == MMTG_EPI_RESID || epi == MMTG_EPI_DGELU || epi == MMTG_EPI_DTANH || epi == MMTG_EPI_ROWDOT) alg_bytes += esz_ * (double)M * N;
    if (epi == MMTG_EPI_GELU) alg_bytes += esz_ * (double)M * N;
    ProfScope prof(dtype == MMTG_F32 ? MMTG_PROF_GEMM_F32 : MMTG_PROF_GEMM_BF16, s, 2.0 * M * N * (double)K, alg_bytes);
    a.ntiles = cdiv(M, BM) * cdiv(N, BN);
    a.nitems = a.ntiles * splits;
    MMTG_REQUIRE((long)cdiv(M, BM) * cdiv(N, BN) * splits < (1L << 20), "gemm: %ld work items exceed the tile-order arithmetic's 2^20", (long)cdiv(M, BM) * cdiv(N, BN) * splits);
    dim3 grid(a.nitems);
    const int skinny = (flags & MMTG_GEMM_SKINNY) || (!transA && transB && M <= 256 && !(flags & MMTG_GEMM_NO_SKINNY));
    int rc;
    if (dtype == MMTG_F32) rc = launch_regstage<float>(a, transA, transB, grid, s);
    else if ((flags & (MMTG_GEMM_REGSTAGE | MMTG_GEMM_NO_TR)) || !small) rc = launch_regstage<bf16>(a, transA, transB, grid, s);
    else {
        bool wide = (flags & MMTG_GEMM_WIDE) != 0;
        static const int wide_rule = getenv("MMTG_GEMM_WIDE_RULE") ? atoi(getenv("MMTG_GEMM_WIDE_RULE")) : 1;
        if (!wide && !(flags & MMTG_GEMM_NO_WIDE) && !transA && !skinny && M >= 1024 && wide_rule) {
            const long t128 = (long)cdiv(M, 128) * cdiv(N, 128), t192 = (long)cdiv(M, 192) * cdiv(N, 128);
            wide = (t128 > 512 && t192 <= 512) || (wide_rule >= 2 && N >= 4096);
        }
        if (epi == MMTG_EPI_DGELU && aux2) {
            MMTG_REQUIRE(!(flags & MMTG_GEMM_WIDE), "gemm: DGELU with column sums (aux2) has no 192x128 configuration");
            wide = false;
        }
        bool persist = (flags & (MMTG_GEMM_PERSIST | MMTG_GEMM_P256)) != 0;
        static const int p256_rule = getenv("MMTG_GEMM_P256_RULE") ? atoi(getenv("MMTG_GEMM_P256_RULE")) : 0;
        if (p256_rule && !persist && !transA && !skinny && !(flags & (MMTG_GEMM_WIDE | MMTG_GEMM_OCC4 | MMTG_GEMM_NO_PERSIST)) && M >= 4096 && N <= 1024 &&
            K >= (p256_rule >= 2 ? 512 : 2048) && epi != MMTG_EPI_SPLIT && epi != MMTG_EPI_ROWDOT && epi != MMTG_EPI_DGELU) {
            persist = true;
            wide = false;
            a.dbg_flags |= 32;
        }
        static const bool env_no_occ4 = getenv("MMTG_GEMM_NO_OCC4") != nullptr;
        if (!(flags & MMTG_GEMM_NO_OCC4) && !env_no_occ4 && !persist && !skinny && !(flags & MMTG_GEMM_WIDE)) {
            const long t128 = (long)cdiv(M, 128) * cdiv(N, 128);
            if (transA || (flags & MMTG_GEMM_OCC4) || (!wide && t128 > 2L * num_cus())) a.dbg_flags |= 2;
        }
        if (wgrad && epi == MMTG_EPI_SPLIT) a.dbg_flags |= 2;
        static const int big = getenv("MMTG_GEMM_BIG") ? atoi(getenv("MMTG_GEMM_BIG")) : 0;
        static const int p8 = getenv("MMTG_GEMM_P8") ? atoi(getenv("MMTG_GEMM_P8")) : 1;
        static const int p8_rows_env = getenv("MMTG_GEMM_P8_ROWS") ? atoi(getenv("MMTG_GEMM_P8_ROWS")) : 0;
        const bool nt_big = !transA && transB && !skinny && !wgrad && M >= 1024 && N >= 256 && splits == 1 && epi != MMTG_EPI_SPLIT &&
                            epi != MMTG_EPI_ATOMIC && !(flags & (MMTG_GEMM_WIDE | MMTG_GEMM_OCC4 | MMTG_GEMM_P256 | MMTG_GEMM_NO_P8)) &&
                            (!(flags & MMTG_GEMM_PERSIST) || (flags & MMTG_GEMM_P8));
        if (big == 1 && nt_big && epi != MMTG_EPI_ROWDOT && !(epi == MMTG_EPI_DGELU && aux2)) {
            wide = false; persist = false; a.dbg_flags &= ~(2 | 32); a.dbg_flags |= 64;
        } else if (p8 && nt_big && K % 128 == 0 && (epi != MMTG_EPI_DGELU || p8 >= 2 || (flags & MMTG_GEMM_P8))) {
            const long t256 = (long)cdiv(M, 256) * cdiv(N, 256), t192 = (long)cdiv(M, 192) * cdiv(N, 256), t288 = (long)cdiv(M, 288) * cdiv(N, 256);
            const long ncu = p8_cus();
            static const int p8_288 = getenv("MMTG_GEMM_P8_288") ? atoi(getenv("MMTG_GEMM_P8_288")) : 1;
            const double nkt = (double)K / 64.0;
            auto cost = [&](long tiles, double r) { const double tk = 1.41 * r / 256.0; return (double)cdiv(tiles, ncu) * (5.6 + nkt * (tk < 1.15 ? 1.15 : tk)); };
            const double c192 = cost(t192, 192), c256 = cost(t256, 256), c288 = cost(t288, 288);
            int rows = c192 < 0.97 * c256 ? 192 : 256;
            if (p8_288 && c288 < 0.95 * (rows == 192 ? c192 : c256)) rows = 288;
            if (flags & MMTG_GEMM_P8_288) rows = 288;
            if (p8_rows_env) rows = p8_rows_env;
            if (epi == MMTG_EPI_DGELU && aux2) rows = 256;
            static const int p8_persist = getenv("MMTG_GEMM_P8_PERSIST") ? atoi(getenv("MMTG_GEMM_P8_PERSIST")) : 0;
            const bool want_persist = p8_persist || ((flags & MMTG_GEMM_P8) && (flags & MMTG_GEMM_PERSIST));
            if (want_persist && rows == 288) rows = 256;
            const long tiles = rows == 192 ? t192 : rows == 288 ? t288 : t256;
            if (want_persist && tiles > num_cus() && num_cus() % 8 == 0) rc = rows == 192 ? launch_p8p<192>(a, s) : launch_p8p<256>(a, s);
            else rc = rows == 192 ? launch_p8<192>(a, 1, s) : rows == 288 ? launch_p8<288>(a, 1, s) : launch_p8<256>(a, 1, s);
            if (rc) return rc;
            MMTG_LAUNCH_CHECK("gemm");
            return MMTG_OK;
        }
        static const int p8t = getenv("MMTG_GEMM_P8T") ? atoi(getenv("MMTG_GEMM_P8T")) : 0;
        if ((p8t || (flags & MMTG_GEMM_P8)) && wgrad && epi == MMTG_EPI_SPLIT && K % 128 == 0 && M >= 256 && N >= 256 && !(flags & (MMTG_GEMM_NO_P8 | MMTG_GEMM_PERSIST))) {
            a.kper = cdiv(cdiv(K, splits), 128) * 128;
            rc = launch_p8<256, true>(a, splits, s);
            if (rc) return rc;
            MMTG_LAUNCH_CHECK("gemm");
            return MMTG_OK;
        }
        rc = launch_dma(a, transA, transB, splits, skinny && !transA && transB, wide, persist, s);
    }
    if (rc) return rc;
    MMTG_LAUNCH_CHECK("gemm");
    return MMTG_OK;
}

extern "C" int mmtg_gemm_x3(int M, int N, int K, const void* A, long lda, long planeA, const void* B, long ldb, long planeB,
                            float* C, long ldc, void* planes, long ldp, long plane_out, const float* bias, int epi,
                            const float* aux, long ldaux, void* aux2, unsigned drop_thresh, unsigned drop_seed, int flags, void* stream) {
    MMTG_REQUIRE(M > 0 && N > 0 && K > 0 && A && B, "gemm_x3: empty problem or null operand");
    MMTG_REQUIRE(C || planes, "gemm_x3: needs an fp32 output, a plane-pair output, or both");
    MMTG_REQUIRE(K % 128 == 0 && N % 8 == 0 && lda % 8 == 0 && ldb % 8 == 0, "gemm_x3: K %% 128 == 0, N, lda, ldb %% 8 == 0 (K=%d N=%d)", K, N);
    MMTG_REQUIRE(MMTG_ALIGNED16(A) && MMTG_ALIGNED16(B) && MMTG_ALIGNED16(C) && MMTG_ALIGNED16(planes) && planeA % 8 == 0 && planeB % 8 == 0,
                 "gemm_x3: operands and plane distances must be 16-byte aligned");
    MMTG_REQUIRE(!C || ldc % 8 == 0, "gemm_x3: ldc %% 8 == 0");
    MMTG_REQUIRE(!planes || (ldp % 8 == 0 && plane_out % 8 == 0 && plane_out >= (long)(M - 1) * ldp + N), "gemm_x3: plane output: ldp, plane distance %% 8 == 0, planes disjoint");
    MMTG_REQUIRE(planeA >= (long)(M - 1) * lda + K && planeB >= (long)(N - 1) * ldb + K, "gemm_x3: an operand's lo plane must lie behind its hi plane");
    MMTG_REQUIRE(epi == MMTG_EPI_NONE || epi == MMTG_EPI_GELU || epi == MMTG_EPI_TANH || epi == MMTG_EPI_RESID || epi == MMTG_EPI_DGELU ||
                 epi == MMTG_EPI_DTANH || epi == MMTG_EPI_ROWDOT, "gemm_x3: epilogue %d is not built for the split-precision product", epi);
    if (epi == MMTG_EPI_RESID || epi == MMTG_EPI_DGELU || epi == MMTG_EPI_DTANH || epi == MMTG_EPI_ROWDOT)
        MMTG_REQUIRE(aux && ldaux % 8 == 0 && MMTG_ALIGNED16(aux), "gemm_x3: epilogue %d needs a 16-byte aligned fp32 aux with ldaux %% 8 == 0", epi);
    if (epi == MMTG_EPI_GELU) MMTG_REQUIRE(aux2 && MMTG_ALIGNED16(aux2) && ldc % 8 == 0 && ldc >= N, "gemm_x3: GELU needs aux2 (fp32 pre-activation, ld = ldc)");
    if (epi == MMTG_EPI_ROWDOT) MMTG_REQUIRE(aux2 && !bias && N % 64 == 0, "gemm_x3: ROWDOT needs aux2 (f32 [M, N/64]), no bias, N %% 64 == 0");
    MMTG_REQUIRE(!bias || MMTG_ALIGNED16(bias), "gemm_x3: bias must be 16-byte aligned");
    const long bytesA = (planeA + (long)(M - 1) * lda + K) * 2, bytesB = (planeB + (long)(N - 1) * ldb + K) * 2;
    MMTG_REQUIRE(bytesA < 0x7FFFFF00L && bytesB < 0x7FFFFF00L, "gemm_x3: an operand's plane pair must stay below 2 GiB");
    GemmArgs a;
    memset(&a, 0, sizeof(a));
    a.A = A; a.B = B; a.C = C; a.bias = bias; a.aux = aux; a.aux2 = aux2;
    a.M = M; a.N = N; a.K = K; a.lda = lda; a.ldb = ldb; a.ldc = ldc; a.ldaux = ldaux;
    a.epi = epi; a.out_f32 = 1; a.use_tr = 1; a.alpha = 1.0f;
    a.trace = g_trace; a.trace_n = g_trace_n;
    a.gelu_grad = (flags & MMTG_GEMM_GELU_GRAD) ? 1 : 0;
    a.dbg_flags = (flags & MMTG_GEMM_ROW_ORDER) ? 1 : 0;
    a.bytesA = (int)bytesA; a.bytesB = (int)bytesB;
    a.planeA = (int)(planeA * 2); a.planeB = (int)(planeB * 2);
    a.planes = planes; a.ldp = ldp; a.plane_out = plane_out;
    a.aux2_bf16 = (flags & MMTG_GEMM_AUX2_BF16) ? 1 : 0;
    a.x3 = 1;
// ... 23 lines not shown
```

mmtg_amd/csrc/gemm_common.h:

```cpp
#pragma once
#include "mma.h"
#include <type_traits>

namespace {

enum { BM = 128, BN = 128, TILE_BYTES = 16384, NTHR = 256 };
constexpr int DG_NP = 32;

struct GemmArgs {
    const void* A; const void* B; void* C;
    const float* bias;
    const void* aux;
    void* aux2;
    int M, N, K;
    long lda, ldb, ldc, ldaux;
    int epi;
    int out_f32;
    int use_tr;
    int tiles_n;
    int tiles_m_fast;
    int cbw;
    int ntiles;
    int kper;
    long split_stride;
// ... 196 lines not shown
template <typename T, bool AKS, bool BKS, bool std_orient, bool use_tr>
__device__ __forceinline__ void compute_tile(const char* tA, const char* tB, f32x4 (&acc)[4][4],
                                             int wm, int wn, int lane,
                                             const int (&oa)[4], const int (&ob)[4]) {
    typedef typename Vec16<T>::type V;
    const int g = lane >> 4, l15 = lane & 15;
    constexpr bool hoist = sizeof(T) == 2;
#pragma unroll
    for (int kk = 0; kk < 2; ++kk) {
        V fa[4], fb[4];
#pragma unroll
        for (int i = 0; i < 4; ++i) {
            if constexpr (!AKS) fa[i] = ld_frag_kc<T>(tA, wm * 64 + i * 16 + l15, kk, g);
            else if constexpr (hoist && use_tr) fa[i] = tr_read_pair(tA, oa[i] + kk * 8192, oa[i] + kk * 8192 + 1024);
            else fa[i] = ld_frag_ks(tA, wm * 64 + i * 16, kk, lane, 0, T());
            if constexpr (!BKS) fb[i] = ld_frag_kc<T>(tB, wn * 64 + i * 16 + l15, kk, g);
            else if constexpr (hoist && use_tr) fb[i] = tr_read_pair(tB, ob[i] + kk * 8192, ob[i] + kk * 8192 + 1024);
            else fb[i] = ld_frag_ks(tB, wn * 64 + i * 16, kk, lane, 0, T());
        }
        if (std_orient) {
#pragma unroll
            for (int i = 0; i < 4; ++i)
#pragma unroll
                for (int j = 0; j < 4; ++j) mma16(fa[i], fb[j], acc[i][j]);
        } else {
#pragma unroll
            for (int i = 0; i < 4; ++i)
#pragma unroll
                for (int j = 0; j < 4; ++j) mma16(fb[j], fa[i], acc[i][j]);
        }
    }
}

template <typename T> __device__ __forceinline__ void load8(const T* p, float (&v)[8]);
template <> __device__ __forceinline__ void load8<float>(const float* p, float (&v)[8]) {
    f32x4 a = *reinterpret_cast<const f32x4*>(p), b = *reinterpret_cast<const f32x4*>(p + 4);
#pragma unroll
    for (int e = 0; e < 4; ++e) { v[e] = a[e]; v[4 + e] = b[e]; }
}
template <> __device__ __forceinline__ void load8<bf16>(const bf16* p, float (&v)[8]) {
    bf16x8 a = *reinterpret_cast<const bf16x8*>(p);
#pragma unroll
    for (int e = 0; e < 8; ++e) v[e] = (float)a[e];
}
template <typename TO> __device__ __forceinline__ void store8(TO* p, const float (&v)[8]);
template <> __device__ __forceinline__ void store8<float>(float* p, const float (&v)[8]) {
    *reinterpret_cast<f32x4*>(p) = f32x4{v[0], v[1], v[2], v[3]};
    *reinterpret_cast<f32x4*>(p + 4) = f32x4{v[4], v[5], v[6], v[7]};
}
template <> __device__ __forceinline__ void store8<bf16>(bf16* p, const float (&v)[8]) {
    bf16x8 o = {(bf16)v[0], (bf16)v[1], (bf16)v[2], (bf16)v[3], (bf16)v[4], (bf16)v[5], (bf16)v[6], (bf16)v[7]};
    *reinterpret_cast<bf16x8*>(p) = o;
}
template <typename T, int EPI, int TM, int TN, int PFD, bool X3 = false>
__device__ __forceinline__ void epi_tiles(const GemmArgs& p, f32x4 (&acc)[TM][TN], int mw0, int nw0, int g, int l15,
                                          char* lds, int lane) {
    constexpr int WTN = TN * 16;
    constexpr int NCH = WTN / 4;
    constexpr int LPR = WTN / 8;
    constexpr int RPI = 64 / LPR;
    constexpr int NQ = 16 / RPI;
    constexpr bool HAS_AUX = EPI == MMTG_EPI_RESID || EPI == MMTG_EPI_DGELU || EPI == MMTG_EPI_DTANH || EPI == MMTG_EPI_ROWDOT ||
                             EPI == MMTG_EPI_TANH_ADD;
    const T* aux = reinterpret_cast<const T*>(p.aux);
    typedef typename std::conditional<X3, bf16, T>::type TF;
    const int col = (lane % LPR) * 8, n = nw0 + col, r0 = lane / LPR;
    const bool nok = n < p.N;
    float b8[8];
#pragma unroll
    for (int e = 0; e < 8; ++e) b8[e] = 0.f;
    if (p.bias && nok) load8<float>(p.bias + n, b8);
    typedef typename Vec16<T>::type V;
    constexpr int VPA = 8 / Vec16<T>::N;
    constexpr int DEPTH = PFD < 0 ? -PFD : PFD;
    constexpr int RING = DEPTH + 1 < TM ? DEPTH + 1 : TM;
    V ax[HAS_AUX ? RING * NQ * VPA : 1];
#define EPI_LOAD_BAND(hb)                                                                                   \
    _Pragma("unroll") for (int q_ = 0; q_ < NQ; ++q_) {                                                     \
        const int m_ = mw0 + (hb) * 16 + q_ * RPI + r0;                                                     \
        const int mc_ = m_ < p.M ? m_ : p.M - 1;                                                            \
        const V* src_ = reinterpret_cast<const V*>(aux + (long)(p.aux_rows ? p.aux_rows[mc_] : mc_) * p.ldaux + (nok ? n : 0)); \
        _Pragma("unroll") for (int u_ = 0; u_ < VPA; ++u_) ax[(((hb) % RING) * NQ + q_) * VPA + u_] = src_[u_]; \
    }
    if constexpr (HAS_AUX) {
#pragma unroll
        for (int hb = 0; hb < RING - 1; ++hb) { EPI_LOAD_BAND(hb) }
    }
    constexpr bool COLSUM = EPI == MMTG_EPI_DGELU && PFD > 0;
    float cs[8] = {0.f, 0.f, 0.f, 0.f, 0.f, 0.f, 0.f, 0.f};
#pragma unroll
    for (int h = 0; h < TM; ++h) {
        if constexpr (HAS_AUX) {
            if (h + RING - 1 < TM) { EPI_LOAD_BAND(h + RING - 1) }
        }
#pragma unroll
        for (int j = 0; j < TN; ++j)
            *reinterpret_cast<f32x4*>(lds + l15 * (WTN * 4) + (((j * 4 + g) ^ (l15 & (NCH - 1))) << 4)) = acc[h][j];
#pragma unroll
        for (int q = 0; q < NQ; ++q) {
            const int row = q * RPI + r0;
            const int m = mw0 + h * 16 + row;
            float v[8];
            {
                const int c0 = 2 * (lane % LPR), sw = row & (NCH - 1);
                const f32x4 lo = *reinterpret_cast<const f32x4*>(lds + row * (WTN * 4) + ((c0 ^ sw) << 4));
                const f32x4 hi = *reinterpret_cast<const f32x4*>(lds + row * (WTN * 4) + (((c0 + 1) ^ sw) << 4));
#pragma unroll
// ... 12 lines not shown
                    for (int e = 0; e < 8; ++e) gd[e] = gelu_new_grad_t<TF>(v[e]);
                    if (X3 && p.aux2_bf16) store8<bf16>(reinterpret_cast<bf16*>(p.aux2) + (long)m * p.ldc + n, gd);
                    else store8<T>(reinterpret_cast<T*>(p.aux2) + (long)m * p.ldc + n, gd);
                } else if (X3 && p.aux2_bf16) {
                    store8<bf16>(reinterpret_cast<bf16*>(p.aux2) + (long)m * p.ldc + n, v);
                } else {
                    store8<T>(reinterpret_cast<T*>(p.aux2) + (long)m * p.ldc + n, v);
                }
#pragma unroll
                for (int e = 0; e < 8; ++e) v[e] = gelu_new_t<TF>(v[e]);
            } else if constexpr (EPI == MMTG_EPI_TANH) {
#pragma unroll
                for (int e = 0; e < 8; ++e) v[e] = tanh_t<TF>(v[e]);
            } else if constexpr (EPI == MMTG_EPI_TANH_ADD) {
#pragma unroll
                for (int e = 0; e < 8; ++e) v[e] = tanh_t<TF>(v[e] + a8[e]);
            } else if constexpr (EPI == MMTG_EPI_RESID) {
                if (p.drop_thresh) {
#pragma unroll
                    for (int e = 0; e < 8; ++e)
                        v[e] *= dropout_scale(p.drop_seed, (uint32_t)((long)m * p.N + n + e), p.drop_thresh, p.drop_inv_keep);
                }
#pragma unroll
                for (int e = 0; e < 8; ++e) v[e] += a8[e];
            } else if constexpr (EPI == MMTG_EPI_DGELU) {
#pragma unroll
                for (int e = 0; e < 8; ++e) {
                    v[e] *= p.gelu_grad ? a8[e] : gelu_new_grad_t<TF>(a8[e]);
                    if constexpr (COLSUM) cs[e] += (float)(T)v[e];
                }
            } else if constexpr (EPI == MMTG_EPI_DTANH) {
#pragma unroll
                for (int e = 0; e < 8; ++e) v[e] *= (1.0f - a8[e] * a8[e]);
            } else if constexpr (EPI == MMTG_EPI_ROWDOT) {
                static_assert(WTN == 64, "ROWDOT needs 64-column wave tiles (one attention head)");
                float dot = 0.f;
#pragma unroll
                for (int e = 0; e < 8; ++e) dot += (float)(T)v[e] * a8[e];
                dot += __shfl_xor(dot, 1, 64);
                dot += __shfl_xor(dot, 2, 64);
                dot += __shfl_xor(dot, 4, 64);
                if ((lane & 7) == 0) reinterpret_cast<float*>(p.aux2)[(long)m * (p.N >> 6) + (n >> 6)] = dot;
            }
            if constexpr (X3) {
                if (p.C) store8<float>(reinterpret_cast<float*>(p.C) + (long)m * p.ldc + n, v);
                if (p.planes) {
                    bf16x8 hi, lo;
#pragma unroll
                    for (int e = 0; e < 8; ++e) { hi[e] = (bf16)v[e]; lo[e] = (bf16)(v[e] - (float)hi[e]); }
                    bf16* dst = reinterpret_cast<bf16*>(p.planes) + (long)m * p.ldp + n;
                    *reinterpret_cast<bf16x8*>(dst) = hi;
                    *reinterpret_cast<bf16x8*>(dst + p.plane_out) = lo;
                }
            } else {
                if (p.out_f32) store8<float>(reinterpret_cast<float*>(p.C) + (long)m * p.ldc + n, v);
                else store8<T>(reinterpret_cast<T*>(p.C) + (long)m * p.ldc + n, v);
            }
        }
        if constexpr (COLSUM) {
            static_assert(!COLSUM || TM % 4 == 0, "column-sum bands are 64 rows: wave tiles of 64 or 128 rows");
            if (h % 4 == 3) {
                if (p.aux2) {
#pragma unroll
                    for (int e = 0; e < 8; ++e) {
#pragma unroll
                        for (int o = LPR; o < 64; o <<= 1) cs[e] += __shfl_xor(cs[e], o, 64);
                    }
                    if (lane < LPR && nok && mw0 + (h - 3) * 16 < p.M)
                        store8<float>(reinterpret_cast<float*>(p.aux2) + (long)((mw0 >> 6) + (h >> 2)) * p.N + n, cs);
                }
#pragma unroll
                for (int e = 0; e < 8; ++e) cs[e] = 0.f;
            }
        }
    }
}

#undef EPI_LOAD_BAND

template <int TM, int TN> constexpr int epi_scratch_bytes() { return 16 * (TN * 16) * 4; }

template <typename T, bool std_orient, int TM, int TN, int PFD = TM, bool X3 = false>
__device__ __forceinline__ void gemm_epilogue(const GemmArgs& p, f32x4 (&acc)[TM][TN], int mw0, int nw0, int g, int l15,
                                              char* lds, int lane) {
    if constexpr (std_orient) {
        float* C = reinterpret_cast<float*>(p.C);
        const bool slab = p.epi == MMTG_EPI_SPLIT;
#pragma unroll
        for (int i = 0; i < TM; ++i)
#pragma unroll
            for (int j = 0; j < TN; ++j) {
                const int n = nw0 + j * 16 + l15;
#pragma unroll
                for (int r = 0; r < 4; ++r) {
                    const int m = mw0 + i * 16 + 4 * g + r;
                    if (m < p.M && n < p.N) {
                        if (slab) C[(long)m * p.ldc + n] = acc[i][j][r];
                        else atomicAdd(C + (long)m * p.ldc + n, acc[i][j][r] * p.alpha);
                    }
                }
            }
    } else {
        switch (p.epi) {
            case MMTG_EPI_GELU: epi_tiles<T, MMTG_EPI_GELU, TM, TN, PFD, X3>(p, acc, mw0, nw0, g, l15, lds, lane); break;
            case MMTG_EPI_TANH: epi_tiles<T, MMTG_EPI_TANH, TM, TN, PFD, X3>(p, acc, mw0, nw0, g, l15, lds, lane); break;
            case MMTG_EPI_TANH_ADD: epi_tiles<T, MMTG_EPI_TANH_ADD, TM, TN, PFD, X3>(p, acc, mw0, nw0, g, l15, lds, lane); break;
            case MMTG_EPI_RESID: epi_tiles<T, MMTG_EPI_RESID, TM, TN, PFD, X3>(p, acc, mw0, nw0, g, l15, lds, lane); break;
            case MMTG_EPI_DGELU: epi_tiles<T, MMTG_EPI_DGELU, TM, TN, PFD, X3>(p, acc, mw0, nw0, g, l15, lds, lane); break;
            case MMTG_EPI_DTANH: epi_tiles<T, MMTG_EPI_DTANH, TM, TN, PFD, X3>(p, acc, mw0, nw0, g, l15, lds, lane); break;
            case MMTG_EPI_ROWDOT:
                if constexpr (TN == 4) epi_tiles<T, MMTG_EPI_ROWDOT, TM, TN, PFD, X3>(p, acc, mw0, nw0, g, l15, lds, lane);
                break;
            default: epi_tiles<T, MMTG_EPI_NONE, TM, TN, PFD, X3>(p, acc, mw0, nw0, g, l15, lds, lane); break;
        }
    }
}

}
```

mmtg_amd/engine.py:

```python
from __future__ import annotations

import contextlib
import math

import numpy as np
import torch

from . import hip
from .configs import rnn_param_shapes

ALIGN = 64


class ParamLayout:

    def __init__(self, model_cfgs, gpt2_cfg):
        S = model_cfgs["seq_len"]
        E = model_cfgs["topic"]["input_dim"]
        H = model_cfgs["topic"]["hidden_dim"]
        D = gpt2_cfg["n_embd"]
        V = gpt2_cfg["vocab_size"]
        NP = gpt2_cfg["n_positions"]
        L = gpt2_cfg["n_layer"]
        self.Vpad = (V + 127) // 128 * 128
# ... 112 lines not shown
        rows.append((v32 / v32.sum()).astype(np.float32))
    return np.stack(rows)


import os as _os


def _dist_rank():
    import torch.distributed as dist
    return dist.get_rank() if dist.is_available() and dist.is_initialized() else int(_os.environ.get("RANK", "0"))


_NO_OCC4 = bool(_os.environ.get("MMTG_GEMM_NO_OCC4"))
_WG_NUM = float(_os.environ.get("MMTG_WGRAD_NUM", "760"))
_WG_CAP = int(_os.environ.get("MMTG_WGRAD_CAP", "12"))
_NO_FEW_ROWS = bool(_os.environ.get("MMTG_NO_FEW_ROWS"))
_WGRAD_SLAB = not _os.environ.get("MMTG_WGRAD_ATOMIC")
_NO_GATHER = bool(_os.environ.get("MMTG_NO_GATHER"))
_PREFETCH = int(_os.environ.get("MMTG_PREFETCH", "0"))


def _wgrad_splits(M, N, K, occ4=False, slots=512, t_iter=1.1, t_fixed=6.0):
    tiles = ((M + 127) // 128) * ((N + 127) // 128)
    if occ4 and not _NO_OCC4:
        smax = max(1, K // 256)
        s = round(_WG_NUM / tiles) if tiles < 512 else round(2520.0 / tiles)
        return int(max(1, min(smax, s, _WG_CAP)))
    best, best_t = 1, None
    for s in range(1, 33):
        if s > 1 and K // s < 256:
            break
        rounds = -(-tiles * s // slots)
        t = rounds * (K / (64.0 * s) * t_iter + t_fixed) + tiles * s * 65536 / 1.3e6
        if best_t is None or t < best_t * 0.97:
            best, best_t = s, t
    return best


_LAZY_ZERO = _os.environ.get("MMTG_FULL_ZERO_GRAD") is None
_WTE_T = _os.environ.get("MMTG_NO_WTE_T") is None
_P8T = _os.environ.get("MMTG_GEMM_P8T", "0") != "0"
_WGRAD_GROUP = _os.environ.get("MMTG_WGRAD_GROUP", "1") != "0"
_WGRAD_GROUP_SPLITS = int(_os.environ.get("MMTG_WGRAD_GROUP_SPLITS", "0"))
_GELU_GRAD = _os.environ.get("MMTG_GELU_GRAD", "0") != "0"
_DEFER_SUMS = _os.environ.get("MMTG_DEFER_SUMS", "1") != "0"
_WGRAD_TAIL = int(_os.environ.get("MMTG_WGRAD_TAIL", "8"))
_TAIL_FORK_EARLY = _os.environ.get("MMTG_WGRAD_TAIL_FORK", "loop") == "loop"
_LMHEAD_GROUP = _os.environ.get("MMTG_LMHEAD_GROUP", "1") != "0"
_LMHEAD_GROUP_SPLITS = int(_os.environ.get("MMTG_LMHEAD_GROUP_SPLITS", "0"))
_WGRAD_STREAM = _os.environ.get("MMTG_WGRAD_STREAM", "0") != "0"
_ENC_STREAMS = _os.environ.get("MMTG_ENC_STREAMS", "0") != "0"
_HYBRID_ENC_BF16 = _os.environ.get("MMTG_HYBRID_ENC_BF16", "1") != "0"
_X3_WG_CFG = 6 if _os.environ.get("MMTG_WGRAD_X3_COMBINED", "1") != "0" else 2
_WGRAD_GROUP_CFG = int(_os.environ.get("MMTG_WGRAD_GROUP_CFG", "0"))


def _group_splits(tiles, K, slots=1024):
    if _WGRAD_GROUP_SPLITS > 0:
        return _WGRAD_GROUP_SPLITS
    return int(max(1, min(slots // max(1, tiles), K // 1024, 16)))


def _group_splits_x3(tiles, K):
    if _X3_WG_CFG != 6:
        return _group_splits(tiles, K)
    if _WGRAD_GROUP_SPLITS > 0:
        return _WGRAD_GROUP_SPLITS
    s = 512 // max(1, tiles)
    if s == 0:
        s = 2048 // tiles
    return int(max(1, min(s, K // 1024, 16)))


def _wgrad_splits_p8(M, N, K, cus=256):
    if not _P8T or K % 128 or M < 256 or N < 256:
        return None
    tiles = ((M + 255) // 256) * ((N + 255) // 256)
    if tiles > cus // 2:
        return None
    units = K // 128
    s0 = max(1, min(cus // tiles, units // 4))
    per = -(-units // s0)
    return -(-units // per)


def _round_capacity(n):
    if n <= 1024:
        return 1024
    k = 1 << (int(n - 1).bit_length() - 1)
    for q in (4, 5, 6, 7, 8):
        if k * q // 4 >= n:
            return k * q // 4
    return 2 * k


def mix_seed(seed, site):
    x = (seed ^ (0x9E3779B9 * (site + 1))) & 0xFFFFFFFF
    x = ((x ^ (x >> 16)) * 0x7FEB352D) & 0xFFFFFFFF
    x = ((x ^ (x >> 15)) * 0x846CA68B) & 0xFFFFFFFF
    return (x ^ (x >> 16)) & 0xFFFFFFFF


def initial_drop_seed(rank=0):
    return mix_seed(torch.initial_seed() & 0xFFFFFFFF, 0x5EED + 7919 * rank)


# ... 417 lines not shown
        else:
            type_ids, keep = self._infer_types_mask(batch, targets, per_row_infer)
        type_ids = type_ids.contiguous().view(-1)
        keep = (keep != 0).to(torch.int32).contiguous()
        h1 = self.buf("h1", (M, H))
        px3 = (self.x3 and E % 128 == 0 and H % 128 == 0 and D % 8 == 0 and "decoder.projector_layer2.weight" in self.wt_entries
               and _os.environ.get("MMTG_X3_PROJECTOR", "1") != "0")
        a["px3"] = px3
        gather = self.dtype == hip.BF16 and M > 256 and not _NO_GATHER
        if gather:
            ids32 = torch.cat([topic_ids, targets], 1).to(torch.int32).contiguous().view(-1)
            rowmap = self._rowmaps.get((B, T))
            if rowmap is None:
                lp = torch.arange(T, device=self.dev) - P
                seg = torch.div(lp, sh.two_sents, rounding_mode="floor")
                seg = torch.where((lp >= 0) & (seg < S), seg, torch.full_like(seg, -1))
                rowmap = torch.where(seg >= 0, torch.arange(B, device=self.dev)[:, None] * S + seg[None, :],
                                     torch.full((B, T), B * S, device=self.dev)).to(torch.int32).contiguous().view(-1)
                if len(self._rowmaps) > 256:
                    self._rowmaps.clear()
                self._rowmaps[(B, T)] = rowmap
            cW = self.buf("c_w1", (B * S + 1, H))
            self._fwd(c, "decoder.projector_layer1.weight", cW[:B * S], B * S, "linear")
            cW[B * S:].zero_()
            hip.gemm_gather(0, self.table, self.W("decoder.projector_layer1.weight"), h1, M, H, E, ids32, self.table.shape[0],
                            lda=E, ldb=E, bias=self.P("decoder.projector_layer1.bias"), epi=hip.EPI_TANH_ADD, aux=cW, ldaux=H,
                            aux_rows=rowmap)
            x = None
        else:
            ids32 = None
            x = self.buf("x_cond", (M, E))
            hip.embed_condition(self.table, topic_ids, targets, c, x, B, P, L, S, E, sh.two_sents, self.table.shape[0])
            if px3:
                xp = hip.split_planes(x, M, E, self.pbuf("x_cond_p", M, E))
                h1p = self.pbuf("h1_p", M, H)
                hip.gemm_x3(xp, self.Wx("decoder.projector_layer1.weight"), h1, M, H, E, planes=h1p,
                            bias=self.P("decoder.projector_layer1.bias"), epi=hip.EPI_TANH)
                a.update(xp=xp, h1p=h1p)
            else:
                self._fwd(x, "decoder.projector_layer1.weight", h1, M, "linear", bias=self.P("decoder.projector_layer1.bias"),
                          epi=hip.EPI_TANH)
        hcur = self.buf("resid_0", (M, D))
        if px3:
            hip.gemm_x3(a["h1p"], self.Wx("decoder.projector_layer2.weight"), hcur, M, D, H, bias=self.P("decoder.projector_layer2.bias"))
        else:
            self._fwd(h1, "decoder.projector_layer2.weight", hcur, M, "linear", bias=self.P("decoder.projector_layer2.bias"))
        pre = "decoder.gpt2.transformer."
        hip.embed_add(hcur, self.W(pre + "wpe.weight"), self.W(pre + "wte.weight"), type_ids, hcur, M, T, D,
                      drop_p=pe, drop_seed=seed)

        layers = []
        x3 = self.x3 and D % 128 == 0
        a["x3"] = x3
        for l in range(sh.L):
            p = f"{pre}h.{l}."
            s = (mix_seed(seed, 3 * l + 1), mix_seed(seed, 3 * l + 2), mix_seed(seed, 3 * l + 3))
            mu1 = self.buf(f"l{l}_mu1", (M,), torch.float32)
            rs1 = self.buf(f"l{l}_rs1", (M,), torch.float32)
            mu2 = self.buf(f"l{l}_mu2", (M,), torch.float32)
            rs2 = self.buf(f"l{l}_rs2", (M,), torch.float32)
            if x3:
                a1 = self.pbuf(f"l{l}_a", M, D)
                hyb = self.hybrid
                xb1 = self.buf(f"l{l}_xin_b", (M, D), torch.bfloat16) if hyb else None
                xb2 = self.buf(f"l{l}_xmid_b", (M, D), torch.bfloat16) if hyb else None
                hip.layernorm_fwd_x3(hcur, a1, self.P(p + "ln_1.weight"), self.P(p + "ln_1.bias"), mu1, rs1, M, D, sh.eps, xb=xb1)
                qkv = self.pbuf(f"l{l}_qkvp", M, 3 * D)
                self._fwd_x3(a1, p + "attn.c_attn.weight", None, M, bias=self.P(p + "attn.c_attn.bias"), planes=qkv, ldc=3 * D)
                if not need_logits and l == sh.L - 1:
                    layers.append((hcur, mu1, rs1, a1, qkv))
                    break
                ctx = self.buf(f"l{l}_ctx", (M, D))
                lse = self.buf(f"l{l}_lse", (B, sh.nH, T), torch.float32)
                ctxp = self.pbuf(f"l{l}_ctxp", M, D)
                hip.attn_fwd_x3(qkv, keep, ctx, ctxp, lse, B, T, sh.nH, D // sh.nH, drop_p=pa, drop_seed=s[0])
                xmid = self.buf(f"l{l}_xmid", (M, D))
                self._fwd_x3(ctxp, p + "attn.c_proj.weight", xmid, M, bias=self.P(p + "attn.c_proj.bias"),
                             epi=hip.EPI_RESID, aux=hcur, ldaux=D, drop_p=pr, drop_seed=s[1])
                m2 = self.pbuf(f"l{l}_m", M, D)
                hip.layernorm_fwd_x3(xmid, m2, self.P(p + "ln_2.weight"), self.P(p + "ln_2.bias"), mu2, rs2, M, D, sh.eps, xb=xb2)
                u = self.buf(f"l{l}_u_b" if hyb else f"l{l}_u", (M, 4 * D), torch.bfloat16 if hyb else None)
                gact = self.pbuf(f"l{l}_g", M, 4 * D)
                self._fwd_x3(m2, p + "mlp.c_fc.weight", None, M, bias=self.P(p + "mlp.c_fc.bias"), planes=gact, ldc=4 * D,
                             epi=hip.EPI_GELU, aux2=u, flags=hip.GEMM_AUX2_BF16 if hyb else 0)
                xout = self.buf(f"resid_{l + 1}", (M, D))
                self._fwd_x3(gact, p + "mlp.c_proj.weight", xout, M, bias=self.P(p + "mlp.c_proj.bias"),
                             epi=hip.EPI_RESID, aux=xmid, ldaux=D, drop_p=pr, drop_seed=s[2])
                layers.append((hcur, mu1, rs1, a1, qkv, ctx, lse, xmid, mu2, rs2, m2, u, gact, s, ctxp))
                if hyb:
                    a.setdefault("hyb_rows", []).append((xb1, xb2))
                hcur = xout
                continue
            a1 = self.buf(f"l{l}_a", (M, D))
            hip.layernorm_fwd(hcur, a1, self.P(p + "ln_1.weight"), self.P(p + "ln_1.bias"), mu1, rs1, M, D, sh.eps)
            qkv = self.buf(f"l{l}_qkv", (M, 3 * D))
            self._fwd(a1, p + "attn.c_attn.weight", qkv, M, "conv1d", bias=self.P(p + "attn.c_attn.bias"))
            if not need_logits and l == sh.L - 1:
                layers.append((hcur, mu1, rs1, a1, qkv))
                break
            ctx = self.buf(f"l{l}_ctx", (M, D))
            lse = self.buf(f"l{l}_lse", (B, sh.nH, T), torch.float32)
            hip.attn_fwd(qkv, keep, ctx, lse, B, T, sh.nH, D // sh.nH, drop_p=pa, drop_seed=s[0])
            xmid = self.buf(f"l{l}_xmid", (M, D))
            self._fwd(ctx, p + "attn.c_proj.weight", xmid, M, "conv1d", bias=self.P(p + "attn.c_proj.bias"),
                      epi=hip.EPI_RESID, aux=hcur, ldaux=D, drop_p=pr, drop_seed=s[1])
            m2 = self.buf(f"l{l}_m", (M, D))
            hip.layernorm_fwd(xmid, m2, self.P(p + "ln_2.weight"), self.P(p + "ln_2.bias"), mu2, rs2, M, D, sh.eps)
            u = self.buf(f"l{l}_u", (M, 4 * D))
            gact = self.buf(f"l{l}_g", (M, 4 * D))
            self._fwd(m2, p + "mlp.c_fc.weight", gact, M, "conv1d", bias=self.P(p + "mlp.c_fc.bias"),
                      epi=hip.EPI_GELU, aux2=u, flags=hip.GEMM_GELU_GRAD if _GELU_GRAD else 0)
            xout = self.buf(f"resid_{l + 1}", (M, D))
            self._fwd(gact, p + "mlp.c_proj.weight", xout, M, "conv1d", bias=self.P(p + "mlp.c_proj.bias"),
                      epi=hip.EPI_RESID, aux=xmid, ldaux=D, drop_p=pr, drop_seed=s[2])
            layers.append((hcur, mu1, rs1, a1, qkv, ctx, lse, xmid, mu2, rs2, m2, u, gact, s, None))
            hcur = xout
        if not need_logits:
            a.update(c=c, kl=kl, type_ids=type_ids, keep=keep, layers=layers, x_last=hcur, logits=None)
            self.act = a
            return a
        muf = self.buf("lnf_mu", (M,), torch.float32)
        rsf = self.buf("lnf_rs", (M,), torch.float32)
        Vp = self.layout.Vpad
        l32 = logits_f32 or self.dtype == hip.F32
        logits = self.buf("logits" if l32 else "logits_c", (M, Vp), torch.float32 if l32 else self.tdt)
        if x3:
            hf = self.pbuf("hf", M, D)
            if self.hybrid:
                a["x_last_b"] = self.buf("x_last_b", (M, D), torch.bfloat16)
            hip.layernorm_fwd_x3(hcur, hf, self.P(pre + "ln_f.weight"), self.P(pre + "ln_f.bias"), muf, rsf, M, D, sh.eps, xb=a.get("x_last_b"))
            hip.gemm_x3(hf, self.Wpx("wte", Vp, D), logits, M, Vp, D)
        else:
            hf = self.buf("hf", (M, D))
            hip.layernorm_fwd(hcur, hf, self.P(pre + "ln_f.weight"), self.P(pre + "ln_f.bias"), muf, rsf, M, D, sh.eps)
            hip.gemm(hf, self.Wp("wte"), logits, M, Vp, D, transB=True, ldb=D, out_f32=l32)
        a.update(xt=xt, t_raw=t_raw, t_ln=t_ln, st=st, enc=enc, alpha=alpha, kl=kl, o=o, ba=ba, c=c, x=x, ids32=ids32, h1=h1,
                 type_ids=type_ids, keep=keep, layers=layers, x_last=hcur, muf=muf, rsf=rsf, hf=hf, logits=logits)
        self.act = a
        return a

    def _infer_types_mask(self, batch, targets, per_row):
        sh = self.sh
        sent = sh.msl + 2
        n = targets.shape[1]
        Bn = targets.shape[0]
        src = targets if per_row else targets[:1].expand(Bn, n)
        tlist = list(range(1, sh.max_seq_length // sent + 1)) + [1]
        idx = torch.arange(n, device=self.dev)
        slot = torch.tensor([tlist[min(i // sent, len(tlist) - 1)] for i in range(n)], device=self.dev, dtype=torch.long)
        edge = ((idx + 1) % sent == 0) | ((idx + 1) % sent == 1)
        is_pad = src == 0
        types = torch.where(edge[None, :] | is_pad, torch.zeros_like(src), slot[None, :].expand(Bn, n))
        mask = (~is_pad).long()
        return (torch.cat([batch["tpw_type_ids"].to(self.dev).long(), types], 1),
                torch.cat([batch["tpw_attention_mask"].to(self.dev).long(), mask], 1))
# ... 111 lines not shown
            hip.layernorm_bwd_x3(dy, x, self.P(gamma_key), mean, rstd, dres, dx, self.G(gamma_key), self.G(g + "bias"), rows, cols, dx_planes,
                                 drop_p=drop_p, drop_seed=drop_seed, dcolsum=None if colsum_key is None else self.G(colsum_key), ws=lnws)

    def _ln_bwd(self, site, dy, x, gamma_key, mean, rstd, dres, dx, rows, cols, dx_masked=None, drop_p=0.0, drop_seed=0, colsum_key=None):
        g = gamma_key[:-len("weight")]
        if self._defer:
            ws = self.buf("ln_bwd_ws_" + site, (hip.lib().mmtg_layernorm_bwd_ws(rows, cols),), torch.float32)
            nb = hip.layernorm_bwd_partial(dy, x, self.P(gamma_key), mean, rstd, dres, dx, rows, cols, ws, dx_masked=dx_masked,
                                           drop_p=drop_p, drop_seed=drop_seed, want_colsum=colsum_key is not None)
            self._defer_sum(ws, 3 * cols, nb, cols, self.G(gamma_key))
            self._defer_sum(ws, 3 * cols, nb, cols, self.G(g + "bias"), offset=cols)
            if colsum_key is not None:
                self._defer_sum(ws, 3 * cols, nb, cols, self.G(colsum_key), offset=2 * cols)
        else:
            lnws = self.buf("ln_bwd_ws", (hip.lib().mmtg_layernorm_bwd_ws(rows, max(self.sh.D, self.sh.H)),), torch.float32)
            hip.layernorm_bwd(dy, x, self.P(gamma_key), mean, rstd, dres, dx, self.G(gamma_key), self.G(g + "bias"), rows, cols,
                              dx_masked=dx_masked, drop_p=drop_p, drop_seed=drop_seed,
                              dcolsum=None if colsum_key is None else self.G(colsum_key), ws=lnws)

    @contextlib.contextmanager
    def _as_bf16(self):
        saved = (self.dtype, self.tdt, self.x3, self.wc, self.wt, self.wte_t)
        self.dtype, self.tdt, self.x3 = hip.BF16, torch.bfloat16, False
        self.wc = self.wc2[0]
        self.wt = None if saved[4] is None else saved[4][0]
        self.wte_t = None if saved[5] is None else saved[5][0]
        try:
            yield
        finally:
            self.dtype, self.tdt, self.x3, self.wc, self.wt, self.wte_t = saved

    def _backward_hybrid(self, dlogits, dkl):
        a, sh = self.act, self.sh
        M, Vp = a["M"], self.layout.Vpad
        if isinstance(dlogits, hip.Planes):
            dlogits = dlogits.t[0]
        if dlogits.dtype != torch.bfloat16:
            dlb = self.buf("dlogits_b", (M, Vp), torch.bfloat16)
            hip.cast_f32_to(dlogits, dlb, M * Vp)
            dlogits = dlb
        hi = lambda pl: pl.t[0]
        layers = []
        for rec, (xb1, xb2) in zip(a["layers"], a["hyb_rows"]):
            (xin, mu1, rs1, a1, qkv, ctx, lse, xmid, mu2, rs2, m2, u, gact, s_, ctxp) = rec
            layers.append((xb1, mu1, rs1, hi(a1), hi(qkv), hi(ctxp), lse, xb2, mu2, rs2, hi(m2), u, hi(gact), s_, None))
        ab = dict(a)
        if a.get("px3"):
            h1b, xb = hi(a["h1p"]), hi(a["xp"])
        else:
            h1b = self.buf("h1_b", tuple(a["h1"].shape), torch.bfloat16)
            hip.cast_f32_to(a["h1"], h1b, a["h1"].numel())
            xb = self.buf("x_cond_b", tuple(a["x"].shape), torch.bfloat16)
            hip.cast_f32_to(a["x"], xb, a["x"].numel())
        ab.update(x3=False, px3=False, gelu_grad=False, elem_mask=True, layers=layers, x_last=a["x_last_b"], hf=hi(a["hf"]), h1=h1b, x=xb, ids32=None)
        try:
            with self._as_bf16():
                self.act = ab
                seg = self._backward_decoder(ab, dlogits)
        finally:
            self.act = a
        if _HYBRID_ENC_BF16:
            ae = self._encoder_record_bf16(a)
            with self._as_bf16():
                self._backward_encoder(ae, seg, dkl)
            return
        seg32 = self.buf("d_seg32", tuple(seg.shape), torch.float32)
        hip.cast_to_f32(seg, seg32, seg.numel())
        self._backward_encoder(a, seg32, dkl)

    def _encoder_record_bf16(self, a):
        def cast(t, name):
            b = self.buf("hyb_" + name, tuple(t.shape), torch.bfloat16)
            hip.cast_f32_to(t, b, t.numel())
            return b
        ae = dict(a)
        for k in ("o", "t_ln", "t_raw", "xt"):
            ae[k] = cast(a[k], k)
        ae["alpha"] = {mod: (cast(q, "aqkv_" + mod), cast(c, "actx_" + mod), p) for mod, (q, c, p) in a["alpha"].items()}
        enc = {}
        for ch, (layers, h_ln) in a["enc"].items():
            recs = []
            for l, rec in enumerate(layers):
                r = dict(rec)
                r["h"] = cast(rec["h"], "h_%s%d" % (ch, l))
                r["inp"] = recs[l - 1]["h"] if (l > 0 and rec["inp"] is layers[l - 1]["h"]) else cast(rec["inp"], "inp_%s%d" % (ch, l))
                recs.append(r)
            enc[ch] = (recs, cast(h_ln, "hln_" + ch))
        ae["enc"] = enc
        return ae

    def backward(self, dlogits, dkl=0.0):
        a = self.act
        self.ensure_grad()
        if self._lazy is not None and not self.wgrad_overwrite:
            self.grad.zero_()
            self._lazy = None
        if self.hybrid and a.get("x3"):
            self._backward_hybrid(dlogits, dkl)
        else:
            self._backward_encoder(a, self._backward_decoder(a, dlogits), dkl)
        if self._tail_side is not None:
            torch.cuda.current_stream().wait_stream(self._tail_side)
            self._tail_side = None
        self._lazy = None

    def _backward_decoder(self, a, dlogits):
        sh = self.sh
# ... 128 lines not shown
                    self._defer_sum(bws, 3 * D, nkv, 2 * D, self.G(p + "attn.c_attn.bias")[D:], offset=D)
                    self._defer_sum(bws, D, nq, D, self.G(p + "attn.c_attn.bias"), offset=nkv * 3 * D)
                self._dgrad_x3(dqkvp, p + "attn.c_attn.weight", da, M)
                keys = (p + "mlp.c_fc.weight", p + "mlp.c_proj.weight", p + "attn.c_proj.weight", p + "attn.c_attn.weight")
                probs = [(m2, dup, self.G(keys[0]), D, 4 * D), (gact, dyp, self.G(keys[1]), 4 * D, D),
                         (ctxp, dy2p, self.G(keys[2]), D, D), (a1, dqkvp, self.G(keys[3]), D, 3 * D)]
                if l < ntail:
                    self._tail_jobs.append((probs, M, gsplits, gws, gcnt, not self.wgrad_overwrite, _X3_WG_CFG))
                else:
                    hip.wgrad_group(probs, M, gsplits, gws, gcnt, accumulate=not self.wgrad_overwrite, config=_X3_WG_CFG)
                if self.wgrad_overwrite and self._ow_rec is not None:
                    self._ow_rec[1].extend((self.layout.entries[k][0], self.layout.entries[k][2]) for k in keys)
                if l > 0:
                    dyp = self.pbuf("d_masked_p" + xsfx(l - 1), M, D)
                    self._ln_bwd_x3("%d_1" % l, da, xin, p + "ln_1.weight", mu1, rs1, dx2, dx, M, D, dyp,
                                    drop_p=pr, drop_seed=a["layers"][l - 1][13][2], colsum_key=f"{pre}h.{l - 1}.mlp.c_proj.bias")
                else:
                    self._ln_bwd("0_1", da, xin, p + "ln_1.weight", mu1, rs1, dx2, dx, M, D)
                self._ready(p + "ln_1.bias")
                continue
            dy = dmask if pr > 0 else dx
            bands = self.buf("d_u_bands_%d" % l if self._defer else "d_u_bands", ((M + 63) // 64, 4 * D), torch.float32)
            self._prefetch(m2, gact)
            self._dgrad(dy, p + "mlp.c_proj.weight", du, M, "conv1d", epi=hip.EPI_DGELU, aux=u, ldaux=4 * D, aux2=bands,
                        flags=hip.GEMM_GELU_GRAD if a["gelu_grad"] else 0)
            if self._defer and bands.shape[0] <= 2048:
                self._defer_sum(bands, 4 * D, bands.shape[0], 4 * D, self.G(p + "mlp.c_fc.bias"))
            else:
                hip.colsum(bands, bands.shape[0], 4 * D, self.G(p + "mlp.c_fc.bias"))
            self._dgrad(du, p + "mlp.c_fc.weight", dm, M, "conv1d")
            dy_fc2 = dy
            if not group:
                self._wgrad(m2, du, p + "mlp.c_fc.weight", None, M, "conv1d")
                self._prefetch(xmid, ctx)
                self._wgrad(gact, dy, p + "mlp.c_proj.weight", None, M, "conv1d")
            self._ln_bwd("%d_2" % l, dm, xmid, p + "ln_2.weight", mu2, rs2, dx, dx2, M, D,
                         dx_masked=dmask_b, drop_p=pr, drop_seed=s[1], colsum_key=p + "attn.c_proj.bias")
            dy = dmask_b if pr > 0 else dx2
            fuse_delta = self.dtype == hip.BF16 and M > 256
            if fuse_delta:
                self._dgrad(dy, p + "attn.c_proj.weight", dctx, M, "conv1d", epi=hip.EPI_ROWDOT, aux=ctx, ldaux=D, aux2=delta)
            else:
                self._dgrad(dy, p + "attn.c_proj.weight", dctx, M, "conv1d")
            self._prefetch(qkv)
            if not group:
                self._wgrad(ctx, dy, p + "attn.c_proj.weight", None, M, "conv1d")
            exact = self.dtype == hip.F32 and not self.x3 and _WGRAD_SLAB
            brows = hip.attn_bwd_dbias_rows(self.dtype, B, T) if self._defer else 0
            brows = brows if 0 < brows <= 2048 else 0
            bws = None if exact else self.buf("attn_dbias_rows_%d" % l if brows else "attn_dbias_rows",
                                               (hip.attn_bwd_bias_rows(B, T, self.dtype), 3 * D), torch.float32)
            hip.attn_bwd(qkv, a["keep"], ctx, dctx, lse, delta, dq32, dqkv, B, T, sh.nH, D // sh.nH,
                         drop_p=pa, drop_seed=s[0], delta_ready=fuse_delta, dbias=None if exact else self.G(p + "attn.c_attn.bias"),
                         flags=(hip.ATTN_ELEM_MASK if a.get("elem_mask") else 0) | (hip.ATTN_DBIAS_ROWS if brows else 0), dbias_ws=bws)
            if brows:
                self._defer_sum(bws, 3 * D, brows, 3 * D, self.G(p + "attn.c_attn.bias"))
            if exact:
                hip.colsum(dqkv, M, 3 * D, self.G(p + "attn.c_attn.bias"))
            self._prefetch(a1, xin)
            self._dgrad(dqkv, p + "attn.c_attn.weight", da, M, "conv1d")
            if l > 0:
                self._prefetch(a["layers"][l - 1][11])
            if group:
                keys = (p + "mlp.c_fc.weight", p + "mlp.c_proj.weight", p + "attn.c_proj.weight", p + "attn.c_attn.weight")
                probs = [(m2, du, self.G(keys[0]), D, 4 * D), (gact, dy_fc2, self.G(keys[1]), 4 * D, D),
                         (ctx, dy, self.G(keys[2]), D, D), (a1, dqkv, self.G(keys[3]), D, 3 * D)]
                if stream_mode:
                    side.wait_stream(torch.cuda.current_stream())
                    with torch.cuda.stream(side):
                        hip.wgrad_group(probs, M, gsplits, gws, gcnt, accumulate=not self.wgrad_overwrite, config=gcfg)
                        wdone[l] = self._event(l)
                        wdone[l].record(side)
                elif l in tsets:
                    self._tail_jobs.append((probs, M, gsplits, gws, gcnt, not self.wgrad_overwrite, gcfg))
                else:
                    hip.wgrad_group(probs, M, gsplits, gws, gcnt, accumulate=not self.wgrad_overwrite, config=gcfg)
                if self.wgrad_overwrite and self._ow_rec is not None:
                    self._ow_rec[1].extend((self.layout.entries[k][0], self.layout.entries[k][2]) for k in keys)
            else:
                self._wgrad(a1, dqkv, p + "attn.c_attn.weight", None, M, "conv1d")
            if stream_mode and (l + 1) in wdone:
                torch.cuda.current_stream().wait_event(wdone.pop(l + 1))
                self._ready(f"{pre}h.{l + 1}.ln_1.bias")
            if l > 0:
                self._ln_bwd("%d_1" % l, da, xin, p + "ln_1.weight", mu1, rs1, dx2, dx, M, D,
                             dx_masked=(sets[(l - 1) & 1][1] if stream_mode else tsets[l - 1][1] if (l - 1) in tsets else dmask),
                             drop_p=pr, drop_seed=a["layers"][l - 1][13][2],
                             colsum_key=f"{pre}h.{l - 1}.mlp.c_proj.bias")
            else:
                self._ln_bwd("0_1", da, xin, p + "ln_1.weight", mu1, rs1, dx2, dx, M, D)
            if not stream_mode:
                self._ready(p + "ln_1.bias")
        if stream_mode:
            torch.cuda.current_stream().wait_stream(side)
            for l_ in sorted(wdone, reverse=True):
                self._ready(f"{pre}h.{l_}.ln_1.bias")
        elif _WGRAD_STREAM and pr > 0 and getattr(self, "_side", None) is not None:
            torch.cuda.current_stream().wait_stream(self._side)
        self._flush_sums()
        self._defer = False
        if _TAIL_FORK_EARLY:
            self._launch_tail_jobs()
        nty = min(32, sh.V)
        hip.embed_add_bwd(dx, a["type_ids"], self.G(pre + "wpe.weight"), self.G(pre + "wte.weight"), M, T, D,
                          nty, drop_p=pe, drop_seed=a["seed"],
                          ws=self.buf("embed_bwd_ws", (int(hip.lib().mmtg_embed_add_bwd_ws(M, D, nty)),), torch.float32))
        self._ready("wpe")
# ... 180 lines not shown
```

mmtg_amd/hip.py:

```python
from __future__ import annotations

import ctypes as C
import os

import torch

F32, BF16 = 0, 1
ABI_VERSION = 12
EPI_NONE, EPI_GELU, EPI_TANH, EPI_RESID, EPI_DGELU, EPI_DTANH, EPI_ATOMIC, EPI_ROWDOT = range(8)
GEMM_NO_TR, GEMM_REGSTAGE, GEMM_SKINNY, GEMM_NO_SKINNY, GEMM_WIDE, GEMM_NO_WIDE = 1, 2, 4, 8, 16, 32
GEMM_PERSIST, GEMM_NO_PERSIST, GEMM_ROW_ORDER, GEMM_OCC4, GEMM_NO_OCC4, GEMM_COL_BLOCK, GEMM_P256, GEMM_NO_P8, GEMM_P8 = 64, 128, 256, 512, 1024, 2048, 4096, 8192, 16384
GEMM_GELU_GRAD = 32768
GEMM_P8_288 = 65536
GEMM_AUX2_BF16 = 131072
PROF_CATS = ["gemm_bf16", "gemm_f32", "attn_fwd", "attn_bwd", "layernorm", "embed", "loss",
             "optim", "encoder", "decode", "misc"]

_LIB_PATH = os.path.join(os.path.dirname(os.path.abspath(__file__)), "libmmtg_hip.so")
_lib = None

_vp, _i, _l, _f, _u = C.c_void_p, C.c_int, C.c_long, C.c_float, C.c_uint

_SIGS = {
    "mmtg_abi_version": ([], _i),
    "mmtg_last_error": ([], C.c_char_p),
    "mmtg_build_flags": ([], C.c_char_p),
    "mmtg_prof_enable": ([_i], _i),
    "mmtg_prof_read": ([_vp, _vp, _vp, _vp], _i),
    "mmtg_gemm_trace": ([_vp, _i], _i),
    "mmtg_gemm_cu_budget": ([_i], _i),
    "mmtg_debug_occupy": ([_i, _i, C.c_double, _vp], _i),
    "mmtg_gemm": ([_i, _i, _i, _i, _i, _i, _vp, _l, _vp, _l, _vp, _l, _vp, _i, _vp, _l, _vp, _i, _f, _i, _u, _u, _i, _vp], _i),
    "mmtg_gemm_gather": ([_i, _i, _i, _i, _vp, _l, _vp, _l, _vp, _l, _vp, _i, _vp, _i, _vp, _l, _vp, _i, _vp], _i),
    "mmtg_splitk_finish": ([_i, _vp, _i, _i, _i, _l, _vp, _i, _vp, _l, _vp, _l, _vp, _vp, _vp, _f, _vp], _i),
    "mmtg_colsum": ([_i, _vp, _l, _i, _i, _vp, _vp, _l, _vp], _i),
    "mmtg_colsum_ws": ([_i, _i], _l),
    "mmtg_layernorm_fwd": ([_i, _vp, _vp, _vp, _vp, _vp, _vp, _i, _i, _f, _vp], _i),
    "mmtg_layernorm_bwd_ws": ([_i, _i], _l),
    "mmtg_layernorm_bwd": ([_i, _vp, _vp, _vp, _vp, _vp, _vp, _vp, _vp, _vp, _i, _i, _vp, _u, _u, _vp, _vp, _l, _vp], _i),
    "mmtg_layernorm_bwd_x3": ([_vp, _vp, _vp, _vp, _vp, _vp, _vp, _vp, _vp, _i, _i, _vp, _l, _u, _u, _vp, _vp, _l, _vp], _i),
    "mmtg_attn_fwd": ([_i, _vp, _vp, _vp, _vp, _i, _i, _i, _i, _u, _u, _vp], _i),
    "mmtg_attn_fwd_x3": ([_vp, _l, _vp, _vp, _vp, _l, _vp, _i, _i, _i, _i, _u, _u, _vp], _i),
    "mmtg_attn_bwd_x3": ([_vp, _l, _vp, _vp, _vp, _l, _vp, _vp, _i, _vp, _l, _vp, _l, _vp, _vp, _l, _i, _i, _i, _i, _u, _u, _vp], _i),
    "mmtg_attn_trace": ([_vp], _i),
    "mmtg_attn_bwd": ([_i, _vp, _vp, _vp, _vp, _vp, _vp, _i, _vp, _vp, _vp, _vp, _i, _i, _i, _i, _u, _u, _i, _vp], _i),
    "mmtg_embed_condition": ([_i, _vp, _vp, _vp, _vp, _vp, _i, _i, _i, _i, _i, _i, _i, _vp], _i),
    "mmtg_segment_sum": ([_i, _vp, _vp, _i, _i, _i, _i, _i, _i, _vp], _i),
    "mmtg_embed_add": ([_i, _vp, _vp, _vp, _vp, _vp, _i, _i, _i, _u, _u, _vp], _i),
    "mmtg_embed_add_bwd": ([_i, _vp, _vp, _vp, _vp, _i, _i, _i, _i, _u, _u, _vp, _l, _vp], _i),
    "mmtg_embed_add_bwd_ws": ([_i, _i, _i], _l),
    "mmtg_dropout_apply": ([_i, _vp, _vp, _l, _i, _u, _u, _vp], _i),
    "mmtg_loss_fwd": ([_i, _vp, _l, _i, _vp, _vp, _vp, _i, _i, _i, _i, _i, _f, _vp, _vp, _vp, _vp, _vp, _vp], _i),
    "mmtg_loss_bwd": ([_i, _i, _vp, _l, _i, _vp, _vp, _vp, _vp, _f, _f, _i, _i, _i, _vp, _l, _i, _vp], _i),
    "mmtg_loss_bwd_x3": ([_vp, _l, _i, _vp, _vp, _vp, _vp, _f, _f, _i, _i, _i, _vp, _l, _l, _i, _vp], _i),
    "mmtg_gru_cell_fwd": ([_i, _vp, _l, _vp, _l, _vp, _l, _vp, _l, _vp, _i, _i, _vp], _i),
    "mmtg_gru_cell_bwd_fused": ([_i, _vp, _l, _vp, _vp, _i, _vp, _vp, _l, _vp, _l, _vp, _vp, _i, _i, _vp], _i),
    "mmtg_rnn_cell_fwd": ([_i, _i, _vp, _l, _vp, _l, _vp, _vp, _l, _vp, _vp, _i, _i, _vp], _i),
    "mmtg_rnn_cell_bwd": ([_i, _i, _vp, _l, _vp, _vp, _vp, _vp, _l, _vp, _i, _vp, _l, _i, _i, _vp], _i),
    "mmtg_gru_cell_bwd": ([_i, _vp, _vp, _vp, _l, _vp, _l, _vp, _vp, _i, _i, _vp], _i),
    "mmtg_alpha_attn_fwd": ([_i, _vp, _vp, _vp, _vp, _vp, _i, _i, _i, _i, _vp], _i),
    "mmtg_alpha_attn_bwd": ([_i, _vp, _vp, _vp, _vp, _f, _vp, _i, _i, _i, _i, _vp], _i),
    "mmtg_beta_fuse_fwd": ([_i, _vp, _vp, _vp, _vp, _vp, _vp, _vp, _i, _i, _i, _vp], _i),
    "mmtg_beta_fuse_bwd": ([_i, _vp, _vp, _vp, _vp, _vp, _vp, _vp, _vp, _vp, _vp, _vp, _i, _i, _i, _vp, _l, _vp], _i),
    "mmtg_beta_fuse_bwd_ws": ([_i, _i, _i], _l),
    "mmtg_prefetch": ([_vp, _l, _i, _vp, _vp], _i),
    "mmtg_zero_ranges": ([_vp, _vp, _i, _vp], _i),
    "mmtg_sumsq": ([_vp, _l, _vp, _vp, _l, _vp], _i),
    "mmtg_sumsq_ws": ([_l], _l),
    "mmtg_adamw": ([_vp, _vp, _vp, _vp, _vp, _vp, _l, _f, _f, _f, _f, _f, _i, _vp, _f, _f, _vp, _vp], _i),
    "mmtg_gemm_x3": ([_i, _i, _i, _vp, _l, _l, _vp, _l, _l, _vp, _l, _vp, _l, _l, _vp, _i, _vp, _l, _vp, _u, _u, _i, _vp], _i),
    "mmtg_split_planes": ([_vp, _l, _i, _i, _vp, _l, _l, _vp], _i),
    "mmtg_layernorm_fwd_x3": ([_vp, _vp, _l, _l, _vp, _vp, _vp, _vp, _i, _i, _f, _vp, _vp], _i),
    "mmtg_cast_f32_to": ([_i, _vp, _vp, _l, _vp], _i),
    "mmtg_cast_pad_rows": ([_i, _vp, _l, _vp, _l, _i, _i, _vp], _i),
    "mmtg_cast_to_f32": ([_i, _vp, _vp, _l, _vp], _i),
    "mmtg_axpy_f32": ([_vp, _vp, _f, _l, _vp], _i),
    "mmtg_slab_sum": ([_vp, _i, _l, _vp, _i, _l, _vp], _i),
    "mmtg_wgrad_group": ([_i, _i, _vp, _i, _i, _vp, _l, _vp, _l, _i, _vp], _i),
    "mmtg_transpose_batch": ([_i, _vp, _vp, _vp, _i, _i, _i, _vp], _i),
    "mmtg_logits_process_argmax": ([_vp, _l, _i, _vp, _l, _vp, _f, _f, _vp, _i, _vp], _i),
    "mmtg_decode_embed": ([_i, _vp, _vp, _l, _vp, _vp, _vp, _vp, _vp, _vp, _vp, _l, _i, _i, _i, _i, _i, _i, _i, _i, _vp], _i),
    "mmtg_decode_embed_add": ([_i, _vp, _vp, _vp, _vp, _vp, _vp, _i, _i, _vp, _vp], _i),
    "mmtg_decode_gemm": ([_i, _i, _i, _i, _vp, _l, _vp, _l, _vp, _l, _vp, _vp, _vp, _i, _f, _i, _i, _vp, _l, _vp, _i, _vp, _l, _vp, _l,
                          _vp, _vp, _vp, _vp, _vp], _i),
    "mmtg_ln_fold_weights": ([_vp, _l, _vp, _vp, _vp, _vp, _vp, _vp, _i, _i, _vp], _i),
    "mmtg_decode_gemm_x3": ([_i, _i, _i, _i, _vp, _l, _l, _vp, _l, _l, _vp, _l, _vp, _l, _l, _vp, _vp, _vp, _i, _f, _i, _vp, _l, _vp, _i, _vp, _l,
                             _vp, _l, _vp, _vp, _vp, _vp, _vp], _i),
    "mmtg_ln_fold_weights_x3": ([_vp, _l, _l, _vp, _vp, _vp, _vp, _l, _l, _vp, _vp, _i, _i, _vp], _i),
    "mmtg_decode_attn_split_x3": ([_vp, _i, _vp, _vp, _vp, _vp, _l, _vp, _vp, _l, _i, _i, _i, _i, _vp], _i),
    "mmtg_decode_embed_x3": ([_vp, _vp, _l, _vp, _vp, _l, _vp, _vp, _vp, _vp, _vp, _l, _i, _i, _i, _i, _i, _i, _i, _i, _vp], _i),
    "mmtg_decode_attn": ([_i, _vp, _vp, _vp, _vp, _l, _vp, _vp, _i, _i, _i, _i, _vp], _i),
    "mmtg_decode_attn_split": ([_i, _vp, _i, _vp, _vp, _vp, _vp, _l, _vp, _vp, _i, _i, _i, _i, _vp], _i),
    "mmtg_logits_process_sample": ([_vp, _l, _i, _vp, _l, _vp, _f, _f, _i, _f, _vp, _vp, _vp, _i, _vp], _i),
    "mmtg_decode_sample": ([_vp, _l, _i, _vp, _l, _vp, _i, _i, _f, _f, _i, _f, _vp, _l, _i, _vp, _vp], _i),
# ... 264 lines not shown
        return
    key = tuple(items)
    arr = _colsum_batch_cache.get(key)
    if arr is None:
        if len(_colsum_batch_cache) > 64:
            _colsum_batch_cache.clear()
        arr = _colsum_batch_cache[key] = (ColsumItem * len(items))(*[ColsumItem(*it) for it in items])
    _check(lib().mmtg_colsum_batch(C.addressof(arr), len(items), _stream()), "colsum_batch")


def layernorm_fwd(x, y, gamma, beta, mean, rstd, rows, cols, eps=1e-5):
    _check(lib().mmtg_layernorm_fwd(dt(x), _p(x), _p(y), _p(gamma), _p(beta), _p(mean), _p(rstd), rows, cols,
                                    float(eps), _stream()), "layernorm_fwd")


_ln_ws = {}


def layernorm_bwd(dy, x, gamma, mean, rstd, dres, dx, dgamma, dbeta, rows, cols, dx_masked=None, drop_p=0.0,
                  drop_seed=0, dcolsum=None, ws=None):
    if ws is None:
        need = lib().mmtg_layernorm_bwd_ws(rows, cols)
        key = (x.device, need)
        ws = _ln_ws.get(key)
        if ws is None:
            ws = _ln_ws[key] = torch.empty(need, device=x.device, dtype=torch.float32)
    _check(lib().mmtg_layernorm_bwd(dt(x), _p(dy), _p(x), _p(gamma), _p(mean), _p(rstd), _p(dres), _p(dx),
                                    _p(dgamma), _p(dbeta), rows, cols, _p(dx_masked), drop_thresh(drop_p),
                                    drop_seed & 0xFFFFFFFF, _p(dcolsum), _p(ws), ws.numel(), _stream()), "layernorm_bwd")


def layernorm_bwd_partial(dy, x, gamma, mean, rstd, dres, dx, rows, cols, ws, dx_masked=None, drop_p=0.0, drop_seed=0, want_colsum=False):
    n = C.c_int(0)
    _check(lib().mmtg_layernorm_bwd_partial(dt(x), _p(dy), _p(x), _p(gamma), _p(mean), _p(rstd), _p(dres), _p(dx), rows, cols,
                                            _p(dx_masked), drop_thresh(drop_p), drop_seed & 0xFFFFFFFF, int(want_colsum),
                                            _p(ws), ws.numel(), C.addressof(n), _stream()), "layernorm_bwd_partial")
    return n.value


def layernorm_bwd_x3(dy, x, gamma, mean, rstd, dres, dx, dgamma, dbeta, rows, cols, dx_planes, drop_p=0.0, drop_seed=0, dcolsum=None, ws=None):
    _check(lib().mmtg_layernorm_bwd_x3(_p(dy), _p(x), _p(gamma), _p(mean), _p(rstd), _p(dres), _p(dx), _p(dgamma), _p(dbeta), rows, cols,
                                       _p(dx_planes.t), dx_planes.plane, drop_thresh(drop_p), drop_seed & 0xFFFFFFFF, _p(dcolsum),
                                       _p(ws), ws.numel(), _stream()), "layernorm_bwd_x3")


def layernorm_bwd_x3_partial(dy, x, gamma, mean, rstd, dres, dx, rows, cols, dx_planes, ws, drop_p=0.0, drop_seed=0, want_colsum=False):
    n = C.c_int(0)
    _check(lib().mmtg_layernorm_bwd_x3_partial(_p(dy), _p(x), _p(gamma), _p(mean), _p(rstd), _p(dres), _p(dx), rows, cols,
                                               _p(dx_planes.t), dx_planes.plane, drop_thresh(drop_p), drop_seed & 0xFFFFFFFF,
                                               int(want_colsum), _p(ws), ws.numel(), C.addressof(n), _stream()), "layernorm_bwd_x3_partial")
    return n.value


def attn_fwd(qkv, keep, out, lse, B, T, nH, dh, drop_p=0.0, drop_seed=0):
    _check(lib().mmtg_attn_fwd(dt(qkv), _p(qkv), _p(keep), _p(out), _p(lse), B, T, nH, dh,
                               drop_thresh(drop_p), drop_seed & 0xFFFFFFFF, _stream()), "attn_fwd")


def attn_fwd_x3(qkv_planes, keep, out, out_planes, lse, B, T, nH, dh, drop_p=0.0, drop_seed=0):
    if qkv_planes.ld != 3 * nH * dh:
        raise ValueError("attn_fwd_x3: the qkv plane pair must be dense ([B*T, 3D], ld = 3D)")
    _check(lib().mmtg_attn_fwd_x3(_p(qkv_planes.t), qkv_planes.plane, _p(keep), _p(out), 0 if out_planes is None else _p(out_planes.t),
                                  0 if out_planes is None else out_planes.plane, _p(lse), B, T, nH, dh,
                                  drop_thresh(drop_p), drop_seed & 0xFFFFFFFF, _stream()), "attn_fwd_x3")


def attn_bwd_x3_dq_floats(B, T, D):
    return (-(-T // 128)) * B * T * D


def attn_bwd_x3_ws(B, T, D):
    nkv, nq = B * (-(-T // 128)), -(-(B * T) // 16)
    return (nkv + nq) * 3 * D + (128 * 3 * D if nkv > 2048 else 0) + (128 * D if nq > 2048 else 0)


def attn_bwd_x3(qkv_planes, keep, out, dout_planes, lse, delta, dq32, dqkv_planes, B, T, nH, dh, drop_p=0.0, drop_seed=0, dbias=None,
                dbias_ws=None, delta_ready=False):
    if qkv_planes.ld != 3 * nH * dh or dout_planes.ld != nH * dh or dqkv_planes.ld != 3 * nH * dh:
        raise ValueError("attn_bwd_x3: the plane pairs must be dense (ld = columns)")
    _check(lib().mmtg_attn_bwd_x3(_p(qkv_planes.t), qkv_planes.plane, _p(keep), _p(out), _p(dout_planes.t), dout_planes.plane, _p(lse), _p(delta),
                                  int(delta_ready), _p(dq32), dq32.numel(), _p(dqkv_planes.t), dqkv_planes.plane,
                                  _p(dbias), _p(dbias_ws), 0 if dbias_ws is None else dbias_ws.numel(), B, T, nH, dh,
                                  drop_thresh(drop_p), drop_seed & 0xFFFFFFFF, _stream()), "attn_bwd_x3")


ATTN_ELEM_MASK = 1


def attn_bwd(qkv, keep, out, dout, lse, delta, dq32, dqkv, B, T, nH, dh, drop_p=0.0, drop_seed=0, delta_ready=False,
             dbias=None, dbias_ws=None, flags=0):
    _check(lib().mmtg_attn_bwd(dt(qkv), _p(qkv), _p(keep), _p(out), _p(dout), _p(lse), _p(delta), int(delta_ready), _p(dq32),
                               _p(dqkv), _p(dbias), _p(dbias_ws), B, T, nH, dh, drop_thresh(drop_p), drop_seed & 0xFFFFFFFF,
                               int(flags), _stream()), "attn_bwd")


def attn_trace(buf):
    _check(lib().mmtg_attn_trace(_p(buf)), "attn_trace")


ATTN_DBIAS_ROWS = 2


def attn_bwd_dbias_rows(dtype_code, B, T):
    return int(lib().mmtg_attn_bwd_dbias_rows(dtype_code, B, T))


def attn_bwd_bias_rows(B, T, dtype_code):
    return B * (-(-T // (128 if dtype_code == F32 else 256))) + 44


def embed_condition(table, topic_ids, targets, c, x, B, P, L, S, E, two_sents, V):
    _check(lib().mmtg_embed_condition(dt(table), _p(table), _p(topic_ids), _p(targets), _p(c), _p(x),
                                      B, P, L, S, E, two_sents, V, _stream()), "embed_condition")


def segment_sum(g, out, B, P, L, S, H, two_sents):
    _check(lib().mmtg_segment_sum(dt(g), _p(g), _p(out), B, P, L, S, H, two_sents, _stream()), "segment_sum")


def embed_add(g, wpe, wte, type_ids, h, M, T, D, drop_p=0.0, drop_seed=0):
    _check(lib().mmtg_embed_add(dt(g), _p(g), _p(wpe), _p(wte), _p(type_ids), _p(h), M, T, D,
                                drop_thresh(drop_p), drop_seed & 0xFFFFFFFF, _stream()), "embed_add")


_embed_ws = {}


def embed_add_bwd(dh, type_ids, dwpe, dwte, M, T, D, ntypes, drop_p=0.0, drop_seed=0, ws=None):
    need = int(lib().mmtg_embed_add_bwd_ws(M, D, ntypes))
    if ws is None or ws.numel() < need:
        key = (dh.device, need)
        ws = _embed_ws.get(key)
        if ws is None:
            ws = _embed_ws[key] = torch.empty(need, device=dh.device, dtype=torch.float32)
    _check(lib().mmtg_embed_add_bwd(dt(dh), _p(dh), _p(type_ids), _p(dwpe), _p(dwte), M, T, D, ntypes,
                                    drop_thresh(drop_p), drop_seed & 0xFFFFFFFF, _p(ws), ws.numel(), _stream()), "embed_add_bwd")


def dropout_apply(x, y, n, drop_p, drop_seed):
    _check(lib().mmtg_dropout_apply(dt(x), _p(x), _p(y), n, 0, drop_thresh(drop_p), drop_seed & 0xFFFFFFFF,
                                    _stream()), "dropout_apply")


def loss_fwd(logits, ldl, V, topic_ids, targets, ratings, stage, label_zero, B, P, L, batch_den,
             nll, lse, sample_ce, coef, scalars):
    _check(lib().mmtg_loss_fwd(dt(logits), _p(logits), ldl, V, _p(topic_ids), _p(targets), _p(ratings), stage,
                               int(label_zero), B, P, L, float(batch_den), _p(nll), _p(lse), _p(sample_ce),
                               _p(coef), _p(scalars), _stream()), "loss_fwd")


def loss_bwd(logits, ldl, V, topic_ids, targets, lse, coef, gscale, B, P, L, dlogits, ldd, Vpad, lm_coef=0.0):
    _check(lib().mmtg_loss_bwd(dt(dlogits), dt(logits), _p(logits), ldl, V, _p(topic_ids), _p(targets), _p(lse), _p(coef),
                               float(gscale), float(lm_coef), B, P, L, _p(dlogits), ldd, Vpad, _stream()), "loss_bwd")
# ... 277 lines not shown
```

Baseline: 1.058 million tokens/s.

## Store QKV GEMM output in head-panel layout for attention kernels

Adds a C_PANEL epilogue to the p8 GEMM that writes the QKV projection as contiguous 64-column head panels ([3*nH][M][64]) instead of row-major [M,3D]. The small bf16 attention forward and backward kernels gain a PQ template that reads Q/K/V from this panel layout with a 64-element row stride, so each head's loads are contiguous. It is enabled by default for bf16 at T<=256 when logits are needed, and it disables the backward side-stream fork on that path. The backward path also still reads qkv through the same panel buffer, and any other consumer of qkv assuming row-major layout would break.

```diff
diff --git a/include/mmtg_hip.h b/include/mmtg_hip.h
--- a/include/mmtg_hip.h
+++ b/include/mmtg_hip.h
@@ -42,6 +42,7 @@
 #define MMTG_GEMM_P8_288 65536
 #define MMTG_GEMM_P256 4096
 #define MMTG_GEMM_COL_BLOCK 2048
+#define MMTG_GEMM_C_PANEL 262144
 
 enum {
     MMTG_PROF_GEMM_BF16 = 0, MMTG_PROF_GEMM_F32, MMTG_PROF_ATTN_FWD, MMTG_PROF_ATTN_BWD,
@@ -109,6 +110,8 @@
 
 MMTG_API int mmtg_attn_fwd(int dtype, const void* qkv, const int* keep, void* out, float* lse,
                   int B, int T, int nH, int dh, unsigned drop_thresh, unsigned drop_seed, void* stream);
+MMTG_API int mmtg_attn_fwd_flags(int dtype, const void* qkv, const int* keep, void* out, float* lse,
+                  int B, int T, int nH, int dh, unsigned drop_thresh, unsigned drop_seed, int flags, void* stream);
 MMTG_API int mmtg_attn_fwd_x3(const void* qkv_planes, long qplane, const int* keep, float* out, void* out_planes, long plane, float* lse,
                      int B, int T, int nH, int dh, unsigned drop_thresh, unsigned drop_seed, void* stream);
 MMTG_API int mmtg_attn_bwd_x3(const void* qkv_planes, long qplane, const int* keep, const float* out, const void* dout_planes, long doplane,
@@ -118,6 +121,8 @@
 MMTG_API int mmtg_attn_trace(void* buf);
 #define MMTG_ATTN_ELEM_MASK 1
 #define MMTG_ATTN_DBIAS_ROWS 2
+#define MMTG_ATTN_QKV_PANEL 4
+MMTG_API int mmtg_attn_qkv_panel(int dtype, int T);
 MMTG_API int mmtg_attn_bwd_dbias_rows(int dtype, int B, int T);
 MMTG_API int mmtg_attn_bwd(int dtype, const void* qkv, const int* keep, const void* out, const void* dout,
                   const float* lse, float* delta, int delta_ready, float* dq32, void* dqkv, float* dbias, float* dbias_ws,
diff --git a/mmtg_amd/csrc/attention.hip b/mmtg_amd/csrc/attention.hip
--- a/mmtg_amd/csrc/attention.hip
+++ b/mmtg_amd/csrc/attention.hip
@@ -498,6 +498,11 @@
     return __builtin_bit_cast(float, __builtin_bit_cast(int, p) & m);
 }
 
+template <bool PQ> __device__ __forceinline__ const bf16* qkv_head(const bf16* qkv, int b, int h, int Tn, int nH, long ld) {
+    if constexpr (PQ) return qkv + ((long)h * (gridDim.x / nH) + b) * Tn * DH;
+    else return qkv + (long)b * Tn * ld + h * DH;
+}
+
 struct FwdTile {
     f32x4 o[4];
     float m, l;
@@ -604,7 +609,7 @@
     }
 }
 
-template <bool DROP, int MT = 256>
+template <bool DROP, int MT = 256, bool PQ = false>
 __global__ __launch_bounds__(2 * MT, 4) void attn_fwd_small_kernel(const bf16* __restrict__ qkv, const int* __restrict__ keep,
         bf16* __restrict__ out, float* __restrict__ lse, int Tn, int nH,
         uint32_t keep16, uint32_t drop_seed, float inv_keep, unsigned long long* __restrict__ trace) {
@@ -622,8 +627,9 @@
     const int wave = __builtin_amdgcn_readfirstlane(tid >> 6);
     const int h = blockIdx.x % nH, b = blockIdx.x / nH;
     const int D = nH * DH;
-    const long ld = 3L * D;
-    const bf16* base = qkv + (long)b * Tn * ld + h * DH;
+    const long ld = PQ ? (long)DH : 3L * D;
+    const long koff = PQ ? (long)gridDim.x * Tn * DH : (long)D;
+    const bf16* base = qkv_head<PQ>(qkv, b, h, Tn, nH, ld);
     const int ntile = (Tn + 15) >> 4, npair = (ntile + 1) >> 1;
     const int tA = wave, tB = ntile - 1 - wave;
     const bool work = wave < npair;
@@ -638,7 +644,7 @@
             if (qb < Tn) qfB[ks] = *reinterpret_cast<const bf16x8*>(base + (long)qb * ld + ks * 32 + g * 8);
         }
     }
-    const __amdgpu_buffer_rsrc_t rk = rows_rsrc(base + D, ld, Tn), rv = rows_rsrc(base + 2 * D, ld, Tn);
+    const __amdgpu_buffer_rsrc_t rk = rows_rsrc(base + koff, ld, Tn), rv = rows_rsrc(base + 2 * koff, ld, Tn);
     dma_issue_scalars<MT>(sKeep, keep + (long)b * Tn, 1, Tn, wave, lane);
     dma_issue_chunk<NW, MT>(sK, rk, ld, sV, rv, ld, 0, nchunk, wave, lane);
     dma_issue_chunk<NW, MT>(sK, rk, ld, sV, rv, ld, 1, nchunk, wave, lane);
@@ -1050,7 +1056,7 @@
     }
 }
 
-template <bool DROP, int MT = 256>
+template <bool DROP, int MT = 256, bool PQ = false>
 __global__ __launch_bounds__(MT, (MT == 256 ? 2 : 1)) void attn_bwd_small_kv2_kernel(const bf16* __restrict__ qkv, const int* __restrict__ keep,
         const bf16* __restrict__ d_out, const float* __restrict__ lse, const float* __restrict__ delta,
         bf16* __restrict__ dqkv, float* __restrict__ dbias, int bias_rows, int Tn, int nH,
@@ -1070,8 +1076,9 @@
     const int wave = __builtin_amdgcn_readfirstlane(tid >> 6);
     const int h = blockIdx.x % nH, b = blockIdx.x / nH;
     const int D = nH * DH;
-    const long ld = 3L * D;
-    const bf16* base = qkv + (long)b * Tn * ld + h * DH;
+    const long ld = PQ ? (long)DH : 3L * D;
+    const long koff = PQ ? (long)gridDim.x * Tn * DH : (long)D;
+    const bf16* base = qkv_head<PQ>(qkv, b, h, Tn, nH, ld);
     const bf16* dob = d_out + (long)b * Tn * D + h * DH;
     const int nunit = (Tn + 31) >> 5, nupair = (nunit + 1) >> 1;
     const int uA = wave, uB = nunit - 1 - wave;
@@ -1085,8 +1092,8 @@
             for (int ks = 0; ks < 2; ++ks) {
                 kf[j][ks] = vf[j][ks] = zero16<bf16>();
                 if (key < Tn) {
-                    kf[j][ks] = *reinterpret_cast<const bf16x8*>(base + (long)key * ld + D + ks * 32 + g * 8);
-                    vf[j][ks] = *reinterpret_cast<const bf16x8*>(base + (long)key * ld + 2 * D + ks * 32 + g * 8);
+                    kf[j][ks] = *reinterpret_cast<const bf16x8*>(base + (long)key * ld + koff + ks * 32 + g * 8);
+                    vf[j][ks] = *reinterpret_cast<const bf16x8*>(base + (long)key * ld + 2 * koff + ks * 32 + g * 8);
                 }
             }
         }
@@ -1232,7 +1239,7 @@
     }
 }
 
-template <bool DROP, int MT = 256>
+template <bool DROP, int MT = 256, bool PQ = false>
 __global__ __launch_bounds__(2 * MT, 4) void attn_bwd_small_q_kernel(const bf16* __restrict__ qkv, const int* __restrict__ keep,
         const bf16* __restrict__ d_out, const float* __restrict__ lse, const float* __restrict__ delta,
         bf16* __restrict__ dqkv, float* __restrict__ dbias, int bias_rows, int Tn, int nH,
@@ -1253,13 +1260,14 @@
     const int wave = __builtin_amdgcn_readfirstlane(tid >> 6);
     const int h = blockIdx.x % nH, b = blockIdx.x / nH;
     const int D = nH * DH;
-    const long ld = 3L * D;
-    const bf16* base = qkv + (long)b * Tn * ld + h * DH;
+    const long ld = PQ ? (long)DH : 3L * D;
+    const long koff = PQ ? (long)gridDim.x * Tn * DH : (long)D;
+    const bf16* base = qkv_head<PQ>(qkv, b, h, Tn, nH, ld);
     const bf16* dob = d_out + (long)b * Tn * D + h * DH;
     const int ntile = (Tn + 15) >> 4, npair = (ntile + 1) >> 1;
     const int tA = wave, tB = ntile - 1 - wave;
     const bool work = wave < npair;
-    const __amdgpu_buffer_rsrc_t rk = rows_rsrc(base + D, ld, Tn), rv = rows_rsrc(base + 2 * D, ld, Tn);
+    const __amdgpu_buffer_rsrc_t rk = rows_rsrc(base + koff, ld, Tn), rv = rows_rsrc(base + 2 * koff, ld, Tn);
     dma_issue_scalars<MT>(sKeep, keep + (long)b * Tn, 1, Tn, wave, lane);
     dma_issue_scalars<MT>(sLse, lse + ((long)b * nH + h) * Tn, 1, Tn, wave, lane);
     dma_issue_scalars<MT>(sDel, delta + (long)b * Tn * nH + h, nH, Tn, wave, lane);
@@ -1382,9 +1390,14 @@
 static bool attn_route_tiled() { static const bool v = getenv("MMTG_ATTN_TILED") != nullptr; return v; }
 static bool attn_route_no512() { static const bool v = getenv("MMTG_ATTN_NO512") != nullptr; return v; }
 
-extern "C" int mmtg_attn_fwd(int dtype, const void* qkv, const int* keep, void* out, float* lse,
-                             int B, int T, int nH, int dh, unsigned drop_thresh, unsigned drop_seed, void* stream) {
+static bool attn_panel_route(int dtype, int T) { return dtype == MMTG_BF16 && T <= 256 && !attn_route_tiled(); }
+extern "C" int mmtg_attn_qkv_panel(int dtype, int T) { return attn_panel_route(dtype, T) ? 1 : 0; }
+
+extern "C" int mmtg_attn_fwd_flags(int dtype, const void* qkv, const int* keep, void* out, float* lse,
+                                   int B, int T, int nH, int dh, unsigned drop_thresh, unsigned drop_seed, int flags, void* stream) {
     MMTG_REQUIRE(dh == DH, "attn_fwd: head dim %d unsupported (built for 64)", dh);
+    const bool panel = (flags & MMTG_ATTN_QKV_PANEL) != 0;
+    MMTG_REQUIRE(!panel || attn_panel_route(dtype, T), "attn_fwd: the head-panel qkv layout is built for the bf16 whole-head kernels at T <= 256 only");
     MMTG_REQUIRE(B > 0 && T > 0 && nH > 0, "attn_fwd: bad sizes");
     MMTG_REQUIRE(qkv && keep && out && lse, "attn_fwd: null pointer");
     MMTG_REQUIRE(MMTG_ALIGNED16(qkv) && MMTG_ALIGNED16(out), "attn_fwd: 16-byte alignment");
@@ -1399,6 +1412,8 @@
         if (!attr_set) {
             if (hipFuncSetAttribute((const void*)attn_fwd_small_kernel<false, 256>, hipFuncAttributeMaxDynamicSharedMemorySize, (int)small_smem<256>(256)) != hipSuccess ||
                 hipFuncSetAttribute((const void*)attn_fwd_small_kernel<true, 256>, hipFuncAttributeMaxDynamicSharedMemorySize, (int)small_smem<256>(256)) != hipSuccess ||
+                hipFuncSetAttribute((const void*)attn_fwd_small_kernel<false, 256, true>, hipFuncAttributeMaxDynamicSharedMemorySize, (int)small_smem<256>(256)) != hipSuccess ||
+                hipFuncSetAttribute((const void*)attn_fwd_small_kernel<true, 256, true>, hipFuncAttributeMaxDynamicSharedMemorySize, (int)small_smem<256>(256)) != hipSuccess ||
                 hipFuncSetAttribute((const void*)attn_fwd_small_kernel<false, 512>, hipFuncAttributeMaxDynamicSharedMemorySize, (int)small_smem<512>(512)) != hipSuccess ||
                 hipFuncSetAttribute((const void*)attn_fwd_small_kernel<true, 512>, hipFuncAttributeMaxDynamicSharedMemorySize, (int)small_smem<512>(512)) != hipSuccess)
                 MMTG_FAIL(MMTG_ERR_HIP, "attn_fwd: cannot raise dynamic LDS");
@@ -1408,10 +1423,11 @@
         const bool drop = k16 < 4096u;
         const unsigned kq = drop ? k16 : 0u;
         const float ikq = drop ? small_inv_keep(k16) : 1.0f;
-#define FWD_SMALL(DROP_, MT_) hipLaunchKernelGGL((attn_fwd_small_kernel<DROP_, MT_>), dim3(B * nH), dim3(2 * MT_), small_smem<MT_>(T), s, \
-                                                 (const bf16*)qkv, keep, (bf16*)out, lse, T, nH, kq, drop_seed, ikq, g_attn_trace)
-        if (T <= 256) { if (drop) FWD_SMALL(true, 256); else FWD_SMALL(false, 256); }
-        else { if (drop) FWD_SMALL(true, 512); else FWD_SMALL(false, 512); }
+#define FWD_SMALL(DROP_, MT_, PQ_) hipLaunchKernelGGL((attn_fwd_small_kernel<DROP_, MT_, PQ_>), dim3(B * nH), dim3(2 * MT_), small_smem<MT_>(T), s, \
+                                                      (const bf16*)qkv, keep, (bf16*)out, lse, T, nH, kq, drop_seed, ikq, g_attn_trace)
+        if (panel) { if (drop) FWD_SMALL(true, 256, true); else FWD_SMALL(false, 256, true); }
+        else if (T <= 256) { if (drop) FWD_SMALL(true, 256, false); else FWD_SMALL(false, 256, false); }
+        else { if (drop) FWD_SMALL(true, 512, false); else FWD_SMALL(false, 512, false); }
 #undef FWD_SMALL
         MMTG_LAUNCH_CHECK("attn_fwd");
         return MMTG_OK;
@@ -1425,6 +1441,11 @@
     return MMTG_OK;
 }
 
+extern "C" int mmtg_attn_fwd(int dtype, const void* qkv, const int* keep, void* out, float* lse,
+                             int B, int T, int nH, int dh, unsigned drop_thresh, unsigned drop_seed, void* stream) {
+    return mmtg_attn_fwd_flags(dtype, qkv, keep, out, lse, B, T, nH, dh, drop_thresh, drop_seed, 0, stream);
+}
+
 extern "C" int mmtg_colsum(int dtype, const void* X, long ldx, int M, int N, float* out, float* ws, long ws_floats, void* stream);
 
 extern "C" int mmtg_attn_bwd_dbias_rows(int dtype, int B, int T) {
@@ -1438,6 +1459,8 @@
     MMTG_REQUIRE(B > 0 && T > 0 && nH > 0, "attn_bwd: bad sizes");
     MMTG_REQUIRE(qkv && keep && out && dout && lse && delta && dq32 && dqkv, "attn_bwd: null pointer");
     MMTG_REQUIRE(MMTG_ALIGNED16(qkv) && MMTG_ALIGNED16(dout) && MMTG_ALIGNED16(dqkv), "attn_bwd: 16-byte alignment");
+    const bool panel = (flags & MMTG_ATTN_QKV_PANEL) != 0;
+    MMTG_REQUIRE(!panel || attn_panel_route(dtype, T), "attn_bwd: the head-panel qkv layout is built for the bf16 whole-head kernels at T <= 256 only");
     hipStream_t s = (hipStream_t)stream;
     const double esz = dtype == MMTG_F32 ? 4 : 2;
     ProfScope prof(MMTG_PROF_ATTN_BWD, s, 5.0 * B * nH * (double)T * T * dh, esz * 8.0 * B * T * nH * dh);
@@ -1477,6 +1500,8 @@
             SET_LDS((attn_bwd_small_q_kernel<false, 512>), shm5); SET_LDS((attn_bwd_small_q_kernel<true, 512>), shm5);
             SET_LDS((attn_bwd_small_kv2_kernel<false, 256>), shm2); SET_LDS((attn_bwd_small_kv2_kernel<true, 256>), shm2);
             SET_LDS((attn_bwd_small_kv2_kernel<false, 512>), shm5); SET_LDS((attn_bwd_small_kv2_kernel<true, 512>), shm5);
+            SET_LDS((attn_bwd_small_kv2_kernel<false, 256, true>), shm2); SET_LDS((attn_bwd_small_kv2_kernel<true, 256, true>), shm2);
+            SET_LDS((attn_bwd_small_q_kernel<false, 256, true>), shm2); SET_LDS((attn_bwd_small_q_kernel<true, 256, true>), shm2);
 #undef SET_LDS
             if (!ok) MMTG_FAIL(MMTG_ERR_HIP, "attn_bwd: cannot raise dynamic LDS");
             attr_small = true;
@@ -1490,10 +1515,10 @@
         static const int kv_nw = getenv("MMTG_ATTN_KV_NW") ? atoi(getenv("MMTG_ATTN_KV_NW")) : 0;
 #define KV_SMALL(DROP_, NW_, MT_) hipLaunchKernelGGL((attn_bwd_small_kv_kernel<DROP_, NW_, MT_>), dim3(B * nH), dim3(64 * NW_), small_smem<MT_>(T), s, \
                                    (const bf16*)qkv, keep, (const bf16*)dout, lse, delta, (bf16*)dqkv, bias_dst, bias_rows, T, nH, kq, drop_seed, ik16, g_attn_trace)
-#define Q_SMALL(DROP_, MT_) hipLaunchKernelGGL((attn_bwd_small_q_kernel<DROP_, MT_>), dim3(B * nH), dim3(2 * MT_), small_smem<MT_>(T), sq, \
+#define Q_SMALL(DROP_, MT_, ...) hipLaunchKernelGGL((attn_bwd_small_q_kernel<DROP_, MT_, ##__VA_ARGS__>), dim3(B * nH), dim3(2 * MT_), small_smem<MT_>(T), sq, \
                                    (const bf16*)qkv, keep, (const bf16*)dout, lse, delta, (bf16*)dqkv, bias_dst, bias_rows, T, nH, kq, drop_seed, ik16, g_attn_trace)
         static const bool kv2 = !(getenv("MMTG_ATTN_KV2") && atoi(getenv("MMTG_ATTN_KV2")) == 0);
-#define KV2_SMALL(DROP_, MT_) hipLaunchKernelGGL((attn_bwd_small_kv2_kernel<DROP_, MT_>), dim3(B * nH), dim3(MT_), small_smem<MT_>(T), s, \
+#define KV2_SMALL(DROP_, MT_, ...) hipLaunchKernelGGL((attn_bwd_small_kv2_kernel<DROP_, MT_, ##__VA_ARGS__>), dim3(B * nH), dim3(MT_), small_smem<MT_>(T), s, \
                                    (const bf16*)qkv, keep, (const bf16*)dout, lse, delta, (bf16*)dqkv, bias_dst, bias_rows, T, nH, kq, drop_seed, ik16, g_attn_trace)
         static const bool fork = getenv("MMTG_ATTN_BWD_FORK") && atoi(getenv("MMTG_ATTN_BWD_FORK")) == 1;
         static hipStream_t s2 = nullptr;
@@ -1504,11 +1529,14 @@
                 MMTG_FAIL(MMTG_ERR_HIP, "attn_bwd: cannot create the side stream");
         }
         hipStream_t sq = s;
-        if (fork && kv2 && !kv_nw) {
+        if (fork && kv2 && !kv_nw && !panel) {
             sq = s2;
             if (hipEventRecord(ev_fork, s) != hipSuccess || hipStreamWaitEvent(s2, ev_fork, 0) != hipSuccess) MMTG_FAIL(MMTG_ERR_HIP, "attn_bwd: fork failed");
         }
-        if (kv2 && !kv_nw) {
+        if (panel) {
+            if (drop) { KV2_SMALL(true, 256, true); Q_SMALL(true, 256, true); }
+            else { KV2_SMALL(false, 256, true); Q_SMALL(false, 256, true); }
+        } else if (kv2 && !kv_nw) {
             if (T <= 256) { if (drop) KV2_SMALL(true, 256); else KV2_SMALL(false, 256); }
             else { if (drop) KV2_SMALL(true, 512); else KV2_SMALL(false, 512); }
             if (T <= 256) { if (drop) Q_SMALL(true, 256); else Q_SMALL(false, 256); }
diff --git a/mmtg_amd/csrc/gemm.hip b/mmtg_amd/csrc/gemm.hip
--- a/mmtg_amd/csrc/gemm.hip
+++ b/mmtg_amd/csrc/gemm.hip
@@ -650,7 +650,7 @@
     return (col0 + col < ncols) ? (int)(((long)k * ld + col) * 2) : OOB;
 }
 
-template <int TBM, bool KS = false, bool X3 = false>
+template <int TBM, bool KS = false, bool X3 = false, bool CPANEL = false>
 __global__ __launch_bounds__(512, 1) void gemm_p8_kernel(GemmArgs p) {
     typedef typename std::conditional<X3, float, bf16>::type TE;
     static_assert(!(X3 && (KS || TBM == 288)), "x3: K-contiguous operands, 256- or 192-row tiles");
@@ -811,7 +811,7 @@
     if (wr == 0) asm volatile("s_barrier" ::: "memory");
     asm volatile("s_barrier" ::: "memory");
     if constexpr (KS) p.C = reinterpret_cast<char*>(p.C) + (long)split * p.split_stride;
-    gemm_epilogue<TE, false, TMW, 4, (TBM == 256 ? 2 : TBM == 288 ? -1 : -2), X3>(p, acc, m0 + wr * WTM, n0 + wc * 64, g, l15, smem + wave * epi_scratch_bytes<TMW, 4>(), lane);
+    gemm_epilogue<TE, false, TMW, 4, (TBM == 256 ? 2 : TBM == 288 ? -1 : -2), X3, CPANEL>(p, acc, m0 + wr * WTM, n0 + wc * 64, g, l15, smem + wave * epi_scratch_bytes<TMW, 4>(), lane);
 #ifdef MMTG_P8_PHASE_TRACE
     if (tr && blockIdx.x == 0 && lane == 0 && (int)(gridDim.x + 4 * wave + 4) <= p.trace_n) {
         unsigned long long* r = p.trace + 6 * (size_t)(gridDim.x + 4 * wave);
@@ -968,12 +968,12 @@
     return MMTG_OK;
 }
 
-template <int TBM, bool KS = false, bool X3 = false>
+template <int TBM, bool KS = false, bool X3 = false, bool CPANEL = false>
 int launch_p8(const GemmArgs& a, int splits, hipStream_t stream) {
     static bool attr_done = false;
     const size_t shm = 2 * (TBM + 256) * 128;
     if (!attr_done) {
-        int rc = set_lds(gemm_p8_kernel<TBM, KS, X3>, shm, 512, KS ? "eight-phase 256x256 K-strided" : TBM == 256 ? "eight-phase 256x256" : TBM == 288 ? "eight-phase 288x256" : "eight-phase 192x256");
+        int rc = set_lds(gemm_p8_kernel<TBM, KS, X3, CPANEL>, shm, 512, KS ? "eight-phase 256x256 K-strided" : TBM == 256 ? "eight-phase 256x256" : TBM == 288 ? "eight-phase 288x256" : "eight-phase 192x256");
         if (rc) return rc;
         attr_done = true;
     }
@@ -984,7 +984,7 @@
     b.tiles_m_fast = KS && b.tiles_n > cdiv(a.M, TBM) && !(a.dbg_flags & 1);
     b.cbw = 0;
     if (!KS && !(a.dbg_flags & 1)) b.cbw = column_block(a, TBM, 256, num_cus());
-    hipLaunchKernelGGL((gemm_p8_kernel<TBM, KS, X3>), dim3(b.nitems), dim3(512), shm, stream, b);
+    hipLaunchKernelGGL((gemm_p8_kernel<TBM, KS, X3, CPANEL>), dim3(b.nitems), dim3(512), shm, stream, b);
     return MMTG_OK;
 }
 
@@ -1163,6 +1163,13 @@
     } else {
         MMTG_REQUIRE(!bias, "gemm: atomic epilogue takes no bias");
     }
+    const bool cpanel = (flags & MMTG_GEMM_C_PANEL) != 0;
+    if (cpanel)
+        MMTG_REQUIRE(dtype == MMTG_BF16 && !transA && transB && K % 128 == 0 && N % 64 == 0 && epi == MMTG_EPI_NONE && !out_f32 && splits <= 1 &&
+                     !(flags & (MMTG_GEMM_REGSTAGE | MMTG_GEMM_NO_TR | MMTG_GEMM_SKINNY | MMTG_GEMM_WIDE | MMTG_GEMM_OCC4 | MMTG_GEMM_P256 |
+                                MMTG_GEMM_NO_P8 | MMTG_GEMM_PERSIST)),
+                     "gemm: the panel store (MMTG_GEMM_C_PANEL) is built into the eight-phase kernel only: bf16, transA=0, transB=1, "
+                     "K %% 128 == 0, N %% 64 == 0, plain epilogue, bf16 output, one K split");
     if (epi == MMTG_EPI_ROWDOT)
         MMTG_REQUIRE(aux2 && !bias && N % 64 == 0 && dtype == MMTG_BF16 && !transA && M > 256 && !(flags & (MMTG_GEMM_REGSTAGE | MMTG_GEMM_NO_TR | MMTG_GEMM_SKINNY)),
                      "gemm: ROWDOT epilogue needs aux2 (f32 [M, N/64]), no bias, N %% 64 == 0, the bf16 128x128 LDS-DMA configuration");
@@ -1204,9 +1211,10 @@
     a.nitems = a.ntiles * splits;
     MMTG_REQUIRE((long)cdiv(M, BM) * cdiv(N, BN) * splits < (1L << 20), "gemm: %ld work items exceed the tile-order arithmetic's 2^20", (long)cdiv(M, BM) * cdiv(N, BN) * splits);
     dim3 grid(a.nitems);
-    const int skinny = (flags & MMTG_GEMM_SKINNY) || (!transA && transB && M <= 256 && !(flags & MMTG_GEMM_NO_SKINNY));
+    const int skinny = !cpanel && ((flags & MMTG_GEMM_SKINNY) || (!transA && transB && M <= 256 && !(flags & MMTG_GEMM_NO_SKINNY)));
     int rc;
     if (dtype == MMTG_F32) rc = launch_regstage<float>(a, transA, transB, grid, s);
+    else if (cpanel && !small) MMTG_FAIL(MMTG_ERR_BAD_ARG, "gemm: the panel store needs operands below 2 GiB");
     else if ((flags & (MMTG_GEMM_REGSTAGE | MMTG_GEMM_NO_TR)) || !small) rc = launch_regstage<bf16>(a, transA, transB, grid, s);
     else {
         bool wide = (flags & MMTG_GEMM_WIDE) != 0;
@@ -1239,9 +1247,9 @@
         const bool nt_big = !transA && transB && !skinny && !wgrad && M >= 1024 && N >= 256 && splits == 1 && epi != MMTG_EPI_SPLIT &&
                             epi != MMTG_EPI_ATOMIC && !(flags & (MMTG_GEMM_WIDE | MMTG_GEMM_OCC4 | MMTG_GEMM_P256 | MMTG_GEMM_NO_P8)) &&
                             (!(flags & MMTG_GEMM_PERSIST) || (flags & MMTG_GEMM_P8));
-        if (big == 1 && nt_big && epi != MMTG_EPI_ROWDOT && !(epi == MMTG_EPI_DGELU && aux2)) {
+        if (big == 1 && nt_big && !cpanel && epi != MMTG_EPI_ROWDOT && !(epi == MMTG_EPI_DGELU && aux2)) {
             wide = false; persist = false; a.dbg_flags &= ~(2 | 32); a.dbg_flags |= 64;
-        } else if (p8 && nt_big && K % 128 == 0 && (epi != MMTG_EPI_DGELU || p8 >= 2 || (flags & MMTG_GEMM_P8))) {
+        } else if (cpanel || (p8 && nt_big && K % 128 == 0 && (epi != MMTG_EPI_DGELU || p8 >= 2 || (flags & MMTG_GEMM_P8)))) {
             const long t256 = (long)cdiv(M, 256) * cdiv(N, 256), t192 = (long)cdiv(M, 192) * cdiv(N, 256), t288 = (long)cdiv(M, 288) * cdiv(N, 256);
             const long ncu = p8_cus();
             static const int p8_288 = getenv("MMTG_GEMM_P8_288") ? atoi(getenv("MMTG_GEMM_P8_288")) : 1;
@@ -1257,7 +1265,9 @@
             const bool want_persist = p8_persist || ((flags & MMTG_GEMM_P8) && (flags & MMTG_GEMM_PERSIST));
             if (want_persist && rows == 288) rows = 256;
             const long tiles = rows == 192 ? t192 : rows == 288 ? t288 : t256;
-            if (want_persist && tiles > num_cus() && num_cus() % 8 == 0) rc = rows == 192 ? launch_p8p<192>(a, s) : launch_p8p<256>(a, s);
+            if (cpanel) rc = rows == 192 ? launch_p8<192, false, false, true>(a, 1, s) : rows == 288 ? launch_p8<288, false, false, true>(a, 1, s)
+                                                                            : launch_p8<256, false, false, true>(a, 1, s);
+            else if (want_persist && tiles > num_cus() && num_cus() % 8 == 0) rc = rows == 192 ? launch_p8p<192>(a, s) : launch_p8p<256>(a, s);
             else rc = rows == 192 ? launch_p8<192>(a, 1, s) : rows == 288 ? launch_p8<288>(a, 1, s) : launch_p8<256>(a, 1, s);
             if (rc) return rc;
             MMTG_LAUNCH_CHECK("gemm");
diff --git a/mmtg_amd/csrc/gemm_common.h b/mmtg_amd/csrc/gemm_common.h
--- a/mmtg_amd/csrc/gemm_common.h
+++ b/mmtg_amd/csrc/gemm_common.h
@@ -272,7 +272,7 @@
     bf16x8 o = {(bf16)v[0], (bf16)v[1], (bf16)v[2], (bf16)v[3], (bf16)v[4], (bf16)v[5], (bf16)v[6], (bf16)v[7]};
     *reinterpret_cast<bf16x8*>(p) = o;
 }
-template <typename T, int EPI, int TM, int TN, int PFD, bool X3 = false>
+template <typename T, int EPI, int TM, int TN, int PFD, bool X3 = false, bool CPANEL = false>
 __device__ __forceinline__ void epi_tiles(const GemmArgs& p, f32x4 (&acc)[TM][TN], int mw0, int nw0, int g, int l15,
                                           char* lds, int lane) {
     constexpr int WTN = TN * 16;
@@ -391,6 +391,8 @@
                     *reinterpret_cast<bf16x8*>(dst) = hi;
                     *reinterpret_cast<bf16x8*>(dst + p.plane_out) = lo;
                 }
+            } else if constexpr (CPANEL) {
+                store8<T>(reinterpret_cast<T*>(p.C) + ((long)(n >> 6) * p.M + m) * 64 + (n & 63), v);
             } else {
                 if (p.out_f32) store8<float>(reinterpret_cast<float*>(p.C) + (long)m * p.ldc + n, v);
                 else store8<T>(reinterpret_cast<T*>(p.C) + (long)m * p.ldc + n, v);
@@ -419,10 +421,13 @@
 
 template <int TM, int TN> constexpr int epi_scratch_bytes() { return 16 * (TN * 16) * 4; }
 
-template <typename T, bool std_orient, int TM, int TN, int PFD = TM, bool X3 = false>
+template <typename T, bool std_orient, int TM, int TN, int PFD = TM, bool X3 = false, bool CPANEL = false>
 __device__ __forceinline__ void gemm_epilogue(const GemmArgs& p, f32x4 (&acc)[TM][TN], int mw0, int nw0, int g, int l15,
                                               char* lds, int lane) {
-    if constexpr (std_orient) {
+    if constexpr (CPANEL) {
+        static_assert(!std_orient && !X3 && TN == 4, "panel stores: swapped orientation, 64-column wave tiles, bf16");
+        epi_tiles<T, MMTG_EPI_NONE, TM, TN, PFD, false, true>(p, acc, mw0, nw0, g, l15, lds, lane);
+    } else if constexpr (std_orient) {
         float* C = reinterpret_cast<float*>(p.C);
         const bool slab = p.epi == MMTG_EPI_SPLIT;
 #pragma unroll
diff --git a/mmtg_amd/engine.py b/mmtg_amd/engine.py
--- a/mmtg_amd/engine.py
+++ b/mmtg_amd/engine.py
@@ -188,6 +188,7 @@
 _ENC_STREAMS = _os.environ.get("MMTG_ENC_STREAMS", "0") != "0"
 _HYBRID_ENC_BF16 = _os.environ.get("MMTG_HYBRID_ENC_BF16", "1") != "0"
 _X3_WG_CFG = 6 if _os.environ.get("MMTG_WGRAD_X3_COMBINED", "1") != "0" else 2
+_QKV_PANEL = _os.environ.get("MMTG_QKV_PANEL", "1") != "0"
 _WGRAD_GROUP_CFG = int(_os.environ.get("MMTG_WGRAD_GROUP_CFG", "0"))
 
 
@@ -711,6 +712,9 @@
         layers = []
         x3 = self.x3 and D % 128 == 0
         a["x3"] = x3
+        panel = (_QKV_PANEL and need_logits and not x3 and self.dtype == hip.BF16 and D % 128 == 0 and hip.attn_qkv_panel(hip.BF16, T) and
+                 all(f"{pre}h.{l}.attn.c_attn.weight" in self.wt_entries for l in range(sh.L)))
+        a["qkv_panel"] = panel
         for l in range(sh.L):
             p = f"{pre}h.{l}."
             s = (mix_seed(seed, 3 * l + 1), mix_seed(seed, 3 * l + 2), mix_seed(seed, 3 * l + 3))
@@ -753,13 +757,15 @@
             a1 = self.buf(f"l{l}_a", (M, D))
             hip.layernorm_fwd(hcur, a1, self.P(p + "ln_1.weight"), self.P(p + "ln_1.bias"), mu1, rs1, M, D, sh.eps)
             qkv = self.buf(f"l{l}_qkv", (M, 3 * D))
-            self._fwd(a1, p + "attn.c_attn.weight", qkv, M, "conv1d", bias=self.P(p + "attn.c_attn.bias"))
+            self._fwd(a1, p + "attn.c_attn.weight", qkv, M, "conv1d", bias=self.P(p + "attn.c_attn.bias"),
+                      **({"flags": hip.GEMM_C_PANEL} if panel else {}))
             if not need_logits and l == sh.L - 1:
                 layers.append((hcur, mu1, rs1, a1, qkv))
                 break
             ctx = self.buf(f"l{l}_ctx", (M, D))
             lse = self.buf(f"l{l}_lse", (B, sh.nH, T), torch.float32)
-            hip.attn_fwd(qkv, keep, ctx, lse, B, T, sh.nH, D // sh.nH, drop_p=pa, drop_seed=s[0])
+            hip.attn_fwd(qkv, keep, ctx, lse, B, T, sh.nH, D // sh.nH, drop_p=pa, drop_seed=s[0],
+                         flags=hip.ATTN_QKV_PANEL if panel else 0)
             xmid = self.buf(f"l{l}_xmid", (M, D))
             self._fwd(ctx, p + "attn.c_proj.weight", xmid, M, "conv1d", bias=self.P(p + "attn.c_proj.bias"),
                       epi=hip.EPI_RESID, aux=hcur, ldaux=D, drop_p=pr, drop_seed=s[1])
@@ -977,7 +983,7 @@
             hip.cast_f32_to(a["h1"], h1b, a["h1"].numel())
             xb = self.buf("x_cond_b", tuple(a["x"].shape), torch.bfloat16)
             hip.cast_f32_to(a["x"], xb, a["x"].numel())
-        ab.update(x3=False, px3=False, gelu_grad=False, elem_mask=True, layers=layers, x_last=a["x_last_b"], hf=hi(a["hf"]), h1=h1b, x=xb, ids32=None)
+        ab.update(x3=False, px3=False, gelu_grad=False, elem_mask=True, qkv_panel=False, layers=layers, x_last=a["x_last_b"], hf=hi(a["hf"]), h1=h1b, x=xb, ids32=None)
         try:
             with self._as_bf16():
                 self.act = ab
@@ -1212,7 +1218,8 @@
                                                (hip.attn_bwd_bias_rows(B, T, self.dtype), 3 * D), torch.float32)
             hip.attn_bwd(qkv, a["keep"], ctx, dctx, lse, delta, dq32, dqkv, B, T, sh.nH, D // sh.nH,
                          drop_p=pa, drop_seed=s[0], delta_ready=fuse_delta, dbias=None if exact else self.G(p + "attn.c_attn.bias"),
-                         flags=(hip.ATTN_ELEM_MASK if a.get("elem_mask") else 0) | (hip.ATTN_DBIAS_ROWS if brows else 0), dbias_ws=bws)
+                         flags=(hip.ATTN_ELEM_MASK if a.get("elem_mask") else 0) | (hip.ATTN_DBIAS_ROWS if brows else 0) |
+                               (hip.ATTN_QKV_PANEL if a.get("qkv_panel") else 0), dbias_ws=bws)
             if brows:
                 self._defer_sum(bws, 3 * D, brows, 3 * D, self.G(p + "attn.c_attn.bias"))
             if exact:
diff --git a/mmtg_amd/hip.py b/mmtg_amd/hip.py
--- a/mmtg_amd/hip.py
+++ b/mmtg_amd/hip.py
@@ -13,6 +13,7 @@
 GEMM_GELU_GRAD = 32768
 GEMM_P8_288 = 65536
 GEMM_AUX2_BF16 = 131072
+GEMM_C_PANEL = 262144
 PROF_CATS = ["gemm_bf16", "gemm_f32", "attn_fwd", "attn_bwd", "layernorm", "embed", "loss",
              "optim", "encoder", "decode", "misc"]
 
@@ -40,6 +41,8 @@
     "mmtg_layernorm_bwd": ([_i, _vp, _vp, _vp, _vp, _vp, _vp, _vp, _vp, _vp, _i, _i, _vp, _u, _u, _vp, _vp, _l, _vp], _i),
     "mmtg_layernorm_bwd_x3": ([_vp, _vp, _vp, _vp, _vp, _vp, _vp, _vp, _vp, _i, _i, _vp, _l, _u, _u, _vp, _vp, _l, _vp], _i),
     "mmtg_attn_fwd": ([_i, _vp, _vp, _vp, _vp, _i, _i, _i, _i, _u, _u, _vp], _i),
+    "mmtg_attn_fwd_flags": ([_i, _vp, _vp, _vp, _vp, _i, _i, _i, _i, _u, _u, _i, _vp], _i),
+    "mmtg_attn_qkv_panel": ([_i, _i], _i),
     "mmtg_attn_fwd_x3": ([_vp, _l, _vp, _vp, _vp, _l, _vp, _i, _i, _i, _i, _u, _u, _vp], _i),
     "mmtg_attn_bwd_x3": ([_vp, _l, _vp, _vp, _vp, _l, _vp, _vp, _i, _vp, _l, _vp, _l, _vp, _vp, _l, _i, _i, _i, _i, _u, _u, _vp], _i),
     "mmtg_attn_trace": ([_vp], _i),
@@ -410,9 +413,13 @@
     return n.value
 
 
-def attn_fwd(qkv, keep, out, lse, B, T, nH, dh, drop_p=0.0, drop_seed=0):
-    _check(lib().mmtg_attn_fwd(dt(qkv), _p(qkv), _p(keep), _p(out), _p(lse), B, T, nH, dh,
-                               drop_thresh(drop_p), drop_seed & 0xFFFFFFFF, _stream()), "attn_fwd")
+def attn_fwd(qkv, keep, out, lse, B, T, nH, dh, drop_p=0.0, drop_seed=0, flags=0):
+    if flags:
+        _check(lib().mmtg_attn_fwd_flags(dt(qkv), _p(qkv), _p(keep), _p(out), _p(lse), B, T, nH, dh,
+                                         drop_thresh(drop_p), drop_seed & 0xFFFFFFFF, int(flags), _stream()), "attn_fwd")
+    else:
+        _check(lib().mmtg_attn_fwd(dt(qkv), _p(qkv), _p(keep), _p(out), _p(lse), B, T, nH, dh,
+                                   drop_thresh(drop_p), drop_seed & 0xFFFFFFFF, _stream()), "attn_fwd")
 
 
 def attn_fwd_x3(qkv_planes, keep, out, out_planes, lse, B, T, nH, dh, drop_p=0.0, drop_seed=0):
@@ -457,6 +464,16 @@
 
 
 ATTN_DBIAS_ROWS = 2
+ATTN_QKV_PANEL = 4
+
+
+def attn_qkv_panel(dtype_code, T):
+    return bool(lib().mmtg_attn_qkv_panel(dtype_code, T))
+
+
+def panel_layout(x, cols=64):
+    M, N = x.shape
+    return x.reshape(M, N // cols, cols).permute(1, 0, 2).contiguous()
 
 
 def attn_bwd_dbias_rows(dtype_code, B, T):
```

Measured after the change: 1.063 million tokens/s (median of 6 runs). Within noise of the previous version (+0.4%).
